# scrose/pylc

Measured on AMD Instinct MI355X. Metric: 512x512 tiles/sec fwd+bwd (DeepLabV3+/ResNet101, 9-class), higher is better.
Workload: dtype f32; 1 GPU; DeepLabV3+ ResNet101 OS16, 3-ch 512x512 tiles, 9 classes, CE+Dice+Focal, clip 0.5 + AdamW, bs=32/GPU (BASELINE.json configs[2]); global_batch=32, parallelism=dp1, conv_arithmetic=f16x3 split (fp32-grade), rccl_ranks=0, wgrad_queue=compute stream, sync_bn=True, activation_format=fp16 planes between BatchNorm and conv kernels (4 B/element)

## Files before the change

include/pylc_hip.h:

```cpp
#ifndef PYLC_HIP_H
#define PYLC_HIP_H

#include <stddef.h>
#include <stdint.h>

#ifdef __cplusplus
extern "C" {
#endif

#define PYLC_OK 0
#define PYLC_ERR_ARG 1
#define PYLC_ERR_HIP 2
#define PYLC_ERR_WORKSPACE 3
#define PYLC_ERR_UNSUPPORTED 4

const char* pylc_last_error(void);
int pylc_abi_version(void);
int pylc_experimental_build(void);
int pylc_init(void);

typedef struct PylcConvDesc {
    int B, H, W;
    int Cin, Cout;
    int R, S;
    int stride, pad, dil;
    int OH, OW;
    int x_pitch;
    int y_pitch;
    const unsigned int* x_amax;
    const unsigned int* w_amax;
    const unsigned int* dy_amax;
    const void* w_planes;
    const void* w_planes_t;
    int x_fmt;
    int dy_fmt;
    int out_fmt;
    unsigned int* out_bound;
    int w_planes_fmt;
} PylcConvDesc;

int pylc_set_conv_precision(int mode);
int pylc_get_conv_precision(void);

int pylc_amax(const float* x, long long rows, int cols, int pitch, unsigned int* out_bits, void* stream);
typedef struct PylcWPrepEntry {
    long long src_offset;
    long long fwd_offset;
    long long t_offset;
    long long tile_begin;
    int K, RS, C;
    int amax_index;
} PylcWPrepEntry;
int pylc_conv1x1_fold_input_affine(const float* w, const float* scale, const float* shift, const float* bias_in, int Cout, int Cin,
                                   float* w_out, float* bias_out, unsigned int* amax_out, void* stream);
int pylc_weight_prepare(const float* base, const PylcWPrepEntry* table, int count, long long total_tiles,
                        const unsigned int* amax, void* planes, int interleave, void* stream);
int pylc_range_product(const unsigned int* a_bits, const unsigned int* b_bits, float factor, const unsigned int* add_bits,
                       unsigned int* out_bits, void* stream);
int pylc_amax_segments(const float* base, const long long* offsets, int count, unsigned int* out_bits, void* stream);

long long pylc_planes_stride(long long M, int C, int nplanes);
int pylc_set_planes_interleave(int on);
int pylc_to_planes(const float* x, int x_pitch, void* planes, int p_pitch, long long plane_stride, long long M, int C,
                   const unsigned int* amax, int nplanes, void* stream);
int pylc_from_planes(const void* planes, int p_pitch, long long plane_stride, float* x, int x_pitch, long long M, int C,
                     const unsigned int* amax, int nplanes, void* stream);
size_t pylc_planes_colsum_workspace_floats(int C);
int pylc_upsample2_crop_concat_planes(const float* z, int z_pitch, int B, int h, int w, int C1, const float* bridge, int bridge_pitch, int HH, int WW,
                                      int C2, void* planes, long long plane_stride, int nplanes, const unsigned int* bound, void* stream);
int pylc_planes_colsum(const void* planes, int p_pitch, long long plane_stride, int nplanes, const unsigned int* amax, long long M, int C,
                       float* sums, float* workspace, void* stream);

int pylc_conv2d_fwd(const PylcConvDesc* d, const float* x, const float* w_krsc, const float* bias,
                    float* y, void* stream);
int pylc_conv2d_fwd_bnact(const PylcConvDesc* d, const float* x, const float* w_krsc, const float* bias,
                          const float* scale, const float* shift, const float* residual, int relu, float* y,
                          unsigned int* amax_out, void* stream);

typedef struct PylcFwdEp {
    const float* scale;
    const float* shift;
    const unsigned int* scale_amax;
    const unsigned int* shift_amax;
    const void* residual;
    int res_fmt;
    const unsigned int* res_scale_bound;
    const unsigned int* res_amax;
    const unsigned int* x_true_amax;
    int relu;
    unsigned int* amax_out;
} PylcFwdEp;
int pylc_conv2d_fwd_bnact_ex(const PylcConvDesc* d, const void* x, const float* w, const float* bias, const PylcFwdEp* ep, void* y, void* stream);
size_t pylc_conv2d_fwd_stats_floats(const PylcConvDesc* d);
int pylc_conv2d_fwd_stats(const PylcConvDesc* d, const float* x, const float* w_krsc, const float* bias,
                          float* y, float* stats_partial, int* stats_rows, void* stream);
int pylc_conv2d_dgrad(const PylcConvDesc* d, const float* dy, const float* w_crsk, float* dx,
                      int accumulate, void* stream);
int pylc_conv2d_dgrad_add(const PylcConvDesc* d, const float* dy, const float* w_crsk, float* dx, int accumulate,
                          const float* add_src, const void* add_mask, void* stream);
#ifdef PYLC_EXPERIMENTAL
typedef struct PylcBnBack {
    const float* y;
    const float* mean;
    const float* invstd;
    const float* scale;
    const float* shift;
    const void* relu_mask;
    int relu;
    unsigned int* g_amax;
} PylcBnBack;
size_t pylc_conv2d_dgrad_bn_floats(const PylcConvDesc* d);
int pylc_conv2d_dgrad_bn(const PylcConvDesc* d, const float* dy, const float* w_crsk, float* dx, int accumulate,
                         const float* add_src, const void* add_mask, const PylcBnBack* bn, float* sums_partial, int* sums_rows,
                         void* stream);
#endif
int pylc_relu_bwd_bits(const float* dout, const void* mask, float* g_out, long long M, int C, void* stream);
int pylc_conv2d_dgrad_needs_f32_weights(const PylcConvDesc* d);
size_t pylc_conv2d_wgrad_workspace(const PylcConvDesc* d);
int pylc_conv2d_wgrad(const PylcConvDesc* d, const float* x, const float* dy, float* dw_krsc,
                      float* dbias ,
                      void* workspace, size_t workspace_bytes, void* stream);
typedef struct PylcSlabSum {
    const float* slabs;
    float* dw;
    long long n4;
    long long slab_stride;
    int splits;
    int reserved;
} PylcSlabSum;
int pylc_conv2d_wgrad_slabs(const PylcConvDesc* d, const float* x, const float* dy, float* dw_krsc, void* workspace, size_t workspace_bytes,
                            PylcSlabSum* pending, void* stream);
int pylc_splitk_reduce_batch(const PylcSlabSum* table_dev, const long long* tile_prefix_dev, int n, long long total_tiles, void* stream);
int pylc_weight_transpose(const float* w_krsc, float* w_crsk, int K, int RS, int C, void* stream);

typedef struct PylcDwDesc {
    int B, H, W, C;
    int stride, dil;
    int OH, OW;
    int x_pitch, y_pitch;
} PylcDwDesc;
int pylc_dwconv3x3_fwd(const PylcDwDesc* d, const float* x, const float* w, float* y, void* stream);
int pylc_dwconv3x3_fwd_stats_rows(const PylcDwDesc* d);
int pylc_dwconv3x3_fwd_stats(const PylcDwDesc* d, const float* x, const float* w_c9, float* y, float* stats_partial, void* stream);
int pylc_dwconv3x3_dgrad(const PylcDwDesc* d, const float* dy, const float* w, float* dx, void* stream);
int pylc_dwconv3x3_dgrad_acc(const PylcDwDesc* d, const float* dy, const float* w_c9, float* dx, int accumulate, void* stream);
size_t pylc_dwconv3x3_wgrad_workspace(const PylcDwDesc* d);
int pylc_dwconv3x3_wgrad(const PylcDwDesc* d, const float* x, const float* dy, float* dw,
                         void* workspace, size_t workspace_bytes, void* stream);
int pylc_dwconv3x3_half_ok(const PylcDwDesc* d);
int pylc_dwconv3x3_fwd_h_stats_rows(const PylcDwDesc* d);
int pylc_dwconv3x3_fwd_h(const PylcDwDesc* d, const void* x_h, const unsigned int* x_bound, const float* w_c9, const unsigned int* w_amax,
                         void* y_h, unsigned int* y_bound_out, float* stats_partial, void* stream);
int pylc_dwconv3x3_fwd_h_eval(const PylcDwDesc* d, const void* x_h, const unsigned int* x_bound, const unsigned int* x_true_amax, const float* w,
                              const unsigned int* w_amax, void* y_h, unsigned int* y_bound_out, void* stream);
int pylc_dwconv3x3_dgrad_h(const PylcDwDesc* d, const void* dy_h, const unsigned int* dy_bound, const float* w_c9, const unsigned int* w_amax,
                           void* dx_h, unsigned int* dx_bound_out, int accumulate, const unsigned int* acc_bound, void* stream);
int pylc_dwconv3x3_dgrad_h_add_ok(const PylcDwDesc* d);
int pylc_dwconv3x3_dgrad_h_add(const PylcDwDesc* d, const void* dy_h, const unsigned int* dy_bound, const float* w_c9, const unsigned int* w_amax,
                               float* dx, const float* add_src, const unsigned char* add_mask, void* stream);
int pylc_dwconv3x3_bn_ok(const PylcDwDesc* d);
int pylc_dwconv3x3_fwd_h_bn(const PylcDwDesc* d, const void* y_in_h, const unsigned int* y_in_bound, const float* bn_scale, const float* bn_shift,
                            int relu, const unsigned int* x_bound, const float* w_c9, const unsigned int* w_amax, void* y_h,
                            unsigned int* y_bound_out, float* stats_partial, void* stream);
int pylc_dwconv3x3_wgrad_h_bn(const PylcDwDesc* d, const void* y_in_h, const unsigned int* y_in_bound, const float* bn_scale, const float* bn_shift,
                              int relu, const unsigned int* x_bound, const void* dy_h, const unsigned int* dy_bound, float* dw, void* workspace,
                              size_t workspace_bytes, void* stream);
int pylc_dwconv3x3_wgrad_h(const PylcDwDesc* d, const void* x_h, const unsigned int* x_bound, const void* dy_h, const unsigned int* dy_bound,
                           float* dw, void* workspace, size_t workspace_bytes, void* stream);

size_t pylc_bn_workspace_floats(long long M, int C);
int pylc_bn_stats(const float* y, long long M, int C, int y_pitch, float* sums ,
                  float* workspace, void* stream);
int pylc_bn_stats_from_partial(const float* partial, int n_rows, int C, float* sums , void* stream);
int pylc_bn_finalize(const float* sums, double n, int C, const float* gamma, const float* beta,
                     float eps, float momentum, int clamp_eps,
                     float* running_mean, float* running_var,
                     float* mean, float* invstd, float* scale, float* shift, void* stream);
int pylc_bn_finalize_from_partial(const float* partial, int n_rows, double n, int C, const float* gamma, const float* beta,
                                  float eps, float momentum, int clamp_eps, float* running_mean, float* running_var,
                                  float* mean, float* invstd, float* scale, float* shift, void* stream);
int pylc_bn_eval_coeffs(const float* running_mean, const float* running_var, const float* gamma,
                        const float* beta, float eps, int C, float* scale, float* shift, void* stream);
int pylc_bn_eval_coeffs_full(const float* running_mean, const float* running_var, const float* gamma, const float* beta, float eps,
                             int C, float* scale, float* shift, float* mean, float* invstd, void* stream);
int pylc_bn_apply(const float* y, int y_pitch, const float* scale, const float* shift,
                  const float* residual, int res_pitch, float* out, int out_pitch,
                  long long M, int C, int relu, unsigned int* amax_out, void* stream);
int pylc_bn_bwd_reduce(const float* dout, int dout_pitch, const float* out, int out_pitch,
                       const float* y, int y_pitch, const float* mean, const float* invstd,
                       long long M, int C, int relu, float* sums , float* workspace,
                       const float* scale, const float* shift, void* stream);
int pylc_bn_bwd_apply(const float* dout, int dout_pitch, const float* out, int out_pitch,
                      const float* y, int y_pitch, const float* mean, const float* invstd,
                      const float* gamma, const float* sums, double n,
                      long long M, int C, int relu, float* dy, int dy_pitch, float* g_out, int g_pitch,
                      unsigned int* amax_dy, const float* scale, const float* shift, void* stream);
typedef struct PylcBnExtra {
    void* out_planes;        long long out_plane_stride;  const unsigned int* out_bound;
    const void* res_planes;  long long res_plane_stride;  const unsigned int* res_amax;
    void* dy_planes;         long long dy_plane_stride;   const unsigned int* dy_bound;
    int nplanes;
    float drop_p;
    uint64_t drop_seed;
    unsigned int* g_amax;
    void* relu_mask;
    const unsigned int* y_half_bound;
    const unsigned int* dout_half_bound;
} PylcBnExtra;
int pylc_bn_finalize_ex(const float* sums, double n, int C, const float* gamma, const float* beta, float eps, float momentum,
                        int clamp_eps, float* running_mean, float* running_var, float* mean, float* invstd, float* scale,
                        float* shift, const unsigned int* bound_extra, float bound_mul, unsigned int* bound_out,
                        const float* y, int y_pitch, long long M, const float* stat_shift, void* stream);
int pylc_bn_finalize_from_partial_ex(const float* partial, int n_rows, double n, int C, const float* gamma, const float* beta,
                                     float eps, float momentum, int clamp_eps, float* running_mean, float* running_var,
                                     float* mean, float* invstd, float* scale, float* shift, const unsigned int* bound_extra,
                                     float bound_mul, unsigned int* bound_out, const float* y, int y_pitch, long long M,
                                     const float* stat_shift, void* stream);
int pylc_bn_local_moments(const float* sums, double n, int C, const float* y, int y_pitch, long long M, const float* stat_shift,
                          double* moments, void* stream);
int pylc_bn_finalize_moments(const double* moments, double n, int C, const float* gamma, const float* beta, float eps, float momentum,
                             int clamp_eps, float* running_mean, float* running_var, float* mean, float* invstd, float* scale,
                             float* shift, const unsigned int* bound_extra, float bound_mul, unsigned int* bound_out,
                             const float* stat_shift, void* stream);
int pylc_bn_apply_ex(const float* y, int y_pitch, const float* scale, const float* shift, const float* residual, int res_pitch,
                     float* out, int out_pitch, long long M, int C, int relu, unsigned int* amax_out, const PylcBnExtra* ex,
                     void* stream);
int pylc_bn_bwd_reduce_ex(const float* dout, int dout_pitch, const float* out, int out_pitch, const float* y, int y_pitch,
                          const float* mean, const float* invstd, long long M, int C, int relu, float* sums, float* workspace,
                          const float* scale, const float* shift, const float* gamma, double n, const PylcBnExtra* ex,
                          unsigned int* dy_bound_out, void* stream);
int pylc_bn_bwd_bound(const float* sums, const float* gamma, const float* invstd, double n, int C, const unsigned int* g_amax,
                      unsigned int* bound_out, void* stream);
#ifdef PYLC_EXPERIMENTAL
int pylc_bn_bwd_sums_from_partial(const float* partial, int rows, int C, float* sums, const float* gamma, const float* invstd, double n,
                                  const unsigned int* g_amax, unsigned int* dy_bound_out, void* stream);
#endif
int pylc_bn_bwd_apply_ex(const float* dout, int dout_pitch, const float* out, int out_pitch, const float* y, int y_pitch,
                         const float* mean, const float* invstd, const float* gamma, const float* sums, double n, long long M,
                         int C, int relu, float* dy, int dy_pitch, float* g_out, int g_pitch, unsigned int* amax_dy,
                         const float* scale, const float* shift, const PylcBnExtra* ex, void* stream);
int pylc_bn_frozen_bwd(const float* dout, int dout_pitch, const float* out, int out_pitch, const float* y, int y_pitch,
                       const float* mean, const float* invstd, const float* gamma, long long M, int C, int relu, float* dy,
                       int dy_pitch, float* g_out, int g_pitch, unsigned int* amax_dy, const float* scale, const float* shift,
                       float* sums , float* workspace, const PylcBnExtra* ex, void* stream);
int pylc_relu_fwd(const float* x, int x_pitch, float* out, int out_pitch, long long M, int C, void* stream);
int pylc_relu_bwd(const float* dout, int dout_pitch, const float* out, int out_pitch, float* dx, int dx_pitch,
                  long long M, int C, void* stream);

int pylc_maxpool_fwd(const float* x, float* y, unsigned char* idx, int B, int H, int W, int C, int k, int stride,
                     int pad, int OH, int OW, void* stream);
int pylc_maxpool_fwd_planes(const float* x, void* y_planes, long long plane_stride, int nplanes, const unsigned int* bound, unsigned char* idx,
                            int B, int H, int W, int C, int k, int stride, int pad, int OH, int OW, void* stream);
int pylc_maxpool_bwd(const float* dy, const unsigned char* idx, float* dx, int B, int H, int W, int C, int k,
                     int stride, int pad, int OH, int OW, void* stream);
int pylc_maxpool_bwd_add(const float* dy, const unsigned char* idx, float* dx, int B, int H, int W, int C, int k,
                         int stride, int pad, int OH, int OW, const float* add, int add_pitch, int add_h0,
                         int add_w0, int add_h, int add_w, void* stream);
int pylc_crop_copy(const float* src, int src_pitch, int H, int W, int h0, int w0, float* dst, int dst_pitch,
                   int B, int TH, int TW, int C, void* stream);
int pylc_bilinear_fwd(const float* x, int x_pitch, float* y, int y_pitch, int B, int H, int W, int C,
                      int OH, int OW, void* stream);
int pylc_bilinear_bwd(const float* dy, int dy_pitch, float* dx, int dx_pitch, int B, int H, int W, int C,
                      int OH, int OW, void* stream);
size_t pylc_bilinear_bwd_workspace(int B, int W, int C, int OH);
int pylc_bilinear_bwd_separable(const float* dy, int dy_pitch, float* dx, int dx_pitch, int B, int H, int W, int C,
                                int OH, int OW, float* workspace, unsigned int* amax_bits, void* stream);
int pylc_gap_fwd(const float* x, float* y, int B, int HW, int C, void* stream);
int pylc_gap_bwd(const float* dy, float* dx, int B, int HW, int C, void* stream);
int pylc_gap_fwd_planes(const void* planes, long long plane_stride, int nplanes, const unsigned int* amax, float* y,
                        int B, int HW, int C, void* stream);
int pylc_gap_bwd_acc(const float* dy, float* dx, int B, int HW, int C, int accumulate, void* stream);

int pylc_image_pack(const float* img_nchw, int B, int Cimg, int H, int W, const float* mean3,
                    const float* std3, float* out_nhwc4, void* stream);
int pylc_image_pack_tiles(const float* img, int Cimg, int H, int W, int tile, int stride, int first_tile, int n_tiles,
                          const float* mean3, const float* std3, float* out, void* stream);
int pylc_stitch_argmax(const float* logits, int pitch, int rows, int cols, int tile, int stride, int C,
                       unsigned char* mask, void* stream);
int pylc_colourize_resize(const unsigned char* mask, int h, int w, const unsigned char* palette_rgb,
                          unsigned char* out_rgb, int oh, int ow, void* stream);
int pylc_image_pack_tiles_reflect(const void* img, int is_u8, int Cimg, int H, int W, int tile, int out, int stride,
                                  int first_tile, int n_tiles, const float* mean3, const float* std3, float* tiles,
                                  void* stream);
int pylc_stitch_overlap_argmax(const float* logits, int pitch, int n_tiles, int H, int W, int out, int stride, int C,
                               unsigned char* mask, float* probs, void* stream);
int pylc_resize_area_u8(const unsigned char* src, int src_planar, int Cimg, int H, int W, unsigned char* dst, int oh, int ow,
                        void* stream);
int pylc_class_encode_resize(const unsigned char* rgb, int H, int W, const unsigned char* palette_rgb, int n_classes,
                             unsigned char* out, int oh, int ow, void* stream);
int pylc_class_encode_resize_ex(const unsigned char* rgb, int H, int W, const unsigned char* palette_rgb, int n_classes,
                                unsigned char* out, int oh, int ow, int unmatched_value, void* stream);
int pylc_image_pack_tiles_ex(const void* img, int is_u8, int Cimg, int H, int W, int tile, int stride, int first_tile,
                             int n_tiles, const float* mean3, const float* std3, float* out, void* stream);

int pylc_blend_accumulate(const float* logits, int pitch, int first_tile, int n_tiles, int H, int W, int out, int stride, int C,
                          int flip, float* acc, int acc_pitch, void* stream);
int pylc_blend_finalize(const float* acc, int acc_pitch, int H, int W, int out, int stride, int C, int members,
                        unsigned char* mask, float* probs, float* conf, void* stream);
int pylc_image_pack_tiles_flip(const void* img, int is_u8, int Cimg, int H, int W, int tile, int stride, int first_tile,
                               int n_tiles, const float* mean3, const float* std3, float* out, void* stream, int flip);
int pylc_image_pack_tiles_reflect_ex(const void* img, int is_u8, int Cimg, int H, int W, int tile, int out, int stride,
                                     int first_tile, int n_tiles, const float* mean3, const float* std3, float* tiles,
                                     void* stream, int flip);

int pylc_resize_bilinear_image(const void* src, int is_u8, int Cimg, int H, int W, float* dst, int oh, int ow, void* stream);
int pylc_blend_resample_accumulate(const float* acc_s, int src_pitch, int Hs, int Ws, int out, int stride, int members, float weight,
                                   int C, float* ens, int ens_pitch, int H, int W, int add, void* stream);
int pylc_ensemble_finalize(const float* ens, int pitch, int H, int W, int C, float total_weight, unsigned char* mask, float* probs,
                           float* conf, void* stream);

int pylc_extract_tiles(const unsigned char* img, int Cimg, int H, int W, const unsigned char* mask, int n_classes, int tile,
                       int stride, int first_tile, int n_tiles, int band_rows, unsigned char* img_tiles,
                       unsigned char* mask_tiles, unsigned long long* sums, unsigned long long* hist, void* stream);
int pylc_tile_stats(const unsigned char* img_tiles, long long n_tiles, int Cimg, int tile, const unsigned char* mask_tiles,
                    int n_classes, int band_rows, unsigned long long* sums, unsigned long long* hist, void* stream);
int pylc_augment_tiles(const unsigned char* img_tiles, const unsigned char* mask_tiles, long long n_src, int Cimg, int tile,
                       const int* src_index, const double* minv, const int* shift, long long m, int band_rows,
                       unsigned char* out_img, unsigned char* out_mask, int n_classes, unsigned long long* sums,
                       unsigned long long* hist, void* stream);

int pylc_confusion_matrix(const void* y_true, int true_bytes, const void* y_pred, int pred_bytes, long long n, int C,
                          int force_coverage, unsigned long long* cm, void* stream);
int pylc_confusion_matrix_ex(const void* y_true, int true_bytes, const void* y_pred, int pred_bytes, long long n, int C,
                             int force_coverage, unsigned long long* cm, int ignore_index, unsigned long long* n_skipped, void* stream);
int pylc_logits_score(const float* logits, int pitch, const void* target, int target_bytes, long long N, int C, unsigned char* mask,
                      unsigned long long* counts, void* stream);
int pylc_logits_score_ex(const float* logits, int pitch, const void* target, int target_bytes, long long N, int C, unsigned char* mask,
                         int ignore_index, unsigned long long* counts, void* stream);

int pylc_label_regions(const unsigned char* mask, int H, int W, int connectivity, int ignore_index, int* labels, void* stream);
int pylc_region_sizes(const int* labels, long long N, int* sizes, void* stream);
int pylc_sieve_regions(const unsigned char* mask, const int* labels, const int* sizes, int H, int W, int min_size, int ignore_index,
                       int fill, unsigned long long* best_ws, unsigned char* out, long long* n_changed, void* stream);

int pylc_image_pack_denom(const void* img_nchw, int is_u8, int B, int Cimg, int H, int W, const float* mean3, const float* std3,
                          float denom, float* out_nhwc4, void* stream);
int pylc_image_pack_u8(const unsigned char* img_nchw, int B, int Cimg, int H, int W, const float* mean3,
                       const float* std3, float* out_nhwc4, void* stream);

int pylc_nhwc_to_nchw(const float* x, int x_pitch, float* y, int B, int H, int W, int C, void* stream);
int pylc_nchw_to_nhwc(const float* x, float* y, int y_pitch, int B, int H, int W, int C, void* stream);

#define PYLC_MAX_CLASSES 16
size_t pylc_multiloss_workspace_floats(long long N, int C);
int pylc_multiloss_stats(const float* logits, int pitch, const int64_t* target, long long N, int C,
                         const float* class_weights, float* stats, float* workspace, void* stream);
int pylc_multiloss_finalize(const float* stats, double n_global, int C, float w_ce, float w_dice, float w_focal,
                            float* losses, void* stream);
int pylc_multiloss_bwd(const float* logits, int pitch, const int64_t* target, long long N, int C,
                       const float* class_weights, const float* stats, double n_global,
                       float w_ce, float w_dice, float w_focal, const float* grad_scale,
                       float* dlogits, int dpitch, unsigned int* amax_bits, void* stream);
int pylc_multiloss_stats_ex(const float* logits, int pitch, const void* target, int target_bytes, long long N, int C, int ignore_index,
                            const float* class_weights, float* stats, float* workspace, unsigned long long* n_bad, void* stream);
int pylc_multiloss_finalize_ex(const float* stats, int C, float w_ce, float w_dice, float w_focal, float* losses, void* stream);
int pylc_multiloss_bwd_ex(const float* logits, int pitch, const void* target, int target_bytes, long long N, int C, int ignore_index,
                          const float* class_weights, const float* stats, float w_ce, float w_dice, float w_focal,
                          const float* grad_scale, float* dlogits, int dpitch, unsigned int* amax_bits, void* stream);

size_t pylc_sqnorm_workspace_floats(long long n);
int pylc_grad_norm_clip(const float* g, long long n, float max_norm, float* out2, float* workspace, void* stream);
int pylc_adamw_step(float* p, const float* g, float* m, float* v, long long n, const float* coef,
                    float lr, float beta1, float beta2, float eps, float weight_decay, int step, void* stream);
int pylc_adamw_step_ranges(float* p, const float* g, float* m, float* v, long long n, const float* coef,
                           float lr, float beta1, float beta2, float eps, float weight_decay, int step,
                           const long long* seg_offsets, int seg_count, unsigned int* seg_amax_bits, void* stream);
int pylc_sgd_step(float* p, const float* g, float* buf, long long n, const float* coef, float lr, float momentum,
                  int step, void* stream);

int pylc_dropout(const float* x, int x_pitch, float* out, int out_pitch, long long M, int C, float p,
                 uint64_t seed, void* stream);

#ifdef PYLC_EXPERIMENTAL
int pylc_stream_create_cu_mask(int n_cus, int from_top, void** stream_out);
int pylc_stream_destroy(void* stream);
#endif

int pylc_debug_set_big_tile(int mode);
int pylc_debug_pp_flags(int flags);
int pylc_debug_stagger(int units);
int pylc_debug_dw_tiles(int on);
int pylc_debug_wgrad_m16(int on);
int pylc_debug_wgrad_dma(int on);
int pylc_debug_wgrad_acc1(int on);
int pylc_debug_wgrad_sets(int mode);
int pylc_debug_wgrad_flags(int flags);
int pylc_debug_wgrad_max_steps(int steps);
int pylc_debug_pp_stamps(unsigned long long* buf);

#define PYLC_COMM_ID_BYTES 128
int pylc_comm_available(void);
int pylc_comm_unique_id(void* id_out);
int pylc_comm_init(const void* id, int rank, int world, void** comm_out);
int pylc_comm_allreduce(void* comm, void* buf, long long count, int dtype, void* stream);
int pylc_comm_syncbn_reduce(void* comm, double* moments, int channels, void* stream);
int pylc_comm_destroy(void* comm);

#ifdef __cplusplus
}
#endif
#endif
```

pylc_amd/csrc/common.h:

```cpp
#pragma once
#include <hip/hip_runtime.h>
#include <cstdarg>
#include <cstdio>
#include <cstring>
#include "../../include/pylc_hip.h"

namespace pylc {

extern thread_local char g_err[512];

inline int fail(int code, const char* fmt, ...) {
    va_list ap;
    va_start(ap, fmt);
    vsnprintf(g_err, sizeof(g_err), fmt, ap);
    va_end(ap);
    return code;
}

#define PYLC_REQUIRE(cond, ...)                                     \
    do {                                                            \
        if (!(cond)) return ::pylc::fail(PYLC_ERR_ARG, __VA_ARGS__); \
    } while (0)

#define PYLC_HIP(expr)                                                                          \
    do {                                                                                        \
        hipError_t e__ = (expr);                                                                \
        if (e__ != hipSuccess)                                                                  \
            return ::pylc::fail(PYLC_ERR_HIP, "%s failed: %s", #expr, hipGetErrorString(e__));  \
    } while (0)

#define PYLC_LAUNCH_CHECK() PYLC_HIP(hipGetLastError())

inline hipStream_t as_stream(void* s) { return reinterpret_cast<hipStream_t>(s); }

template <typename T>
__host__ __device__ inline T cdiv(T a, T b) { return (a + b - 1) / b; }

constexpr long long kPlanesIL = 32;
__host__ __device__ inline bool planes_il(long long plane_stride) { return plane_stride == kPlanesIL; }
__host__ __device__ inline long long planes_phys(long long e, bool il) { return il ? ((e >> 5) << 6) + (e & 31) : e; }
__host__ __device__ inline long long planes_p1(long long plane_stride) { return plane_stride; }

extern int g_planes_interleave;
inline long long planes_stride_rule(long long M, int C, int pitch, int nplanes) {
    const bool il = nplanes == 2 && g_planes_interleave && pitch == C && C % 32 == 0 && M * C * 4 < (1ll << 31);
    return il ? kPlanesIL : M * pitch;
}

constexpr int kWave = 64;
constexpr int kNumCU = 256;

__device__ inline float block_sum_256(float v, float* red) {
#pragma unroll
    for (int o = 32; o > 0; o >>= 1) v += __shfl_down(v, o, 64);
    const int lane = threadIdx.x & 63, wv = threadIdx.x >> 6;
    __syncthreads();
    if (lane == 0) red[wv] = v;
    __syncthreads();
    return red[0] + red[1] + red[2] + red[3];
}

__device__ inline void amax_commit(float m, unsigned* out) {
#pragma unroll
    for (int o = 32; o > 0; o >>= 1) m = fmaxf(m, __shfl_xor(m, o, 64));
    if ((threadIdx.x & 63) == 0) {
        const unsigned bits = __float_as_uint(m);
        if (bits > __atomic_load_n(out, __ATOMIC_RELAXED)) atomicMax(out, bits);
    }
}

__global__ __launch_bounds__(256) static void column_sum_kernel(const float* __restrict__ partial, int nrows, int ncols,
                                                                 float* __restrict__ out) {
    __shared__ double red[32][9];
    const int tx = threadIdx.x & 7, ty = threadIdx.x >> 3;
    const int c = blockIdx.x * 8 + tx;
    double acc = 0.0;
    if (c < ncols) {
        for (int r = ty; r < nrows; r += 16 * 32) {
            float v[16];
#pragma unroll
            for (int u = 0; u < 16; ++u) v[u] = partial[(size_t)(r + u * 32 < nrows ? r + u * 32 : 0) * ncols + c];
#pragma unroll
            for (int u = 0; u < 16; ++u) acc += r + u * 32 < nrows ? (double)v[u] : 0.0;
        }
    }
    red[ty][tx] = acc;
    __syncthreads();
    if (ty == 0 && c < ncols) {
        double s = 0.0;
#pragma unroll
        for (int k = 0; k < 32; ++k) s += red[k][tx];
        out[c] = (float)s;
    }
}

}
```

pylc_amd/csrc/loss.hip:

```cpp
#include "common.h"

namespace pylc {

constexpr int MAXC = PYLC_MAX_CLASSES;
constexpr float kFlAlpha = 0.25f;
constexpr float kFlEps = 1e-8f;
constexpr float kDiceSmooth = 1.f;
constexpr int kLossBlocks = 1024;

template <int C>
__device__ __forceinline__ void softmax_px(const float* __restrict__ z, float (&p)[C], float& lse) {
    float zmax = z[0];
#pragma unroll
    for (int c = 1; c < C; ++c) zmax = fmaxf(zmax, z[c]);
    float sum = 0.f;
#pragma unroll
    for (int c = 0; c < C; ++c) { p[c] = expf(z[c] - zmax); sum += p[c]; }
    const float inv = 1.f / sum;
#pragma unroll
    for (int c = 0; c < C; ++c) p[c] *= inv;
    lse = zmax + logf(sum);
}

template <int C, typename TT, bool IGN>
__global__ __launch_bounds__(256) void multiloss_stats_kernel(const float* __restrict__ logits, int pitch, const TT* __restrict__ target,
                                                              long long N, const float* __restrict__ cw, float* __restrict__ partial,
                                                              long long ignore, unsigned long long* __restrict__ n_bad) {
    __shared__ float red[4];
    float acc[3 + 3 * C];
#pragma unroll
    for (int k = 0; k < 3 + 3 * C; ++k) acc[k] = 0.f;
    unsigned int bad = 0;
    for (long long n = (long long)blockIdx.x * blockDim.x + threadIdx.x; n < N; n += (long long)gridDim.x * blockDim.x) {
        const long long tl = (long long)target[n];
        if constexpr (IGN) {
            if (tl == ignore) continue;
            if ((unsigned long long)tl >= (unsigned long long)C) { ++bad; continue; }
        }
        float z[C], p[C], lse;
        const float* src = logits + n * pitch;
#pragma unroll
        for (int c = 0; c < C; ++c) z[c] = src[c];
        softmax_px<C>(z, p, lse);
        const int t = (int)tl;
        float zt = 0.f, pt = 0.f;
#pragma unroll
        for (int c = 0; c < C; ++c) {
            const bool is = (c == t);
            zt = is ? z[c] : zt;
            pt = is ? p[c] : pt;
            acc[3 + c] += is ? p[c] : 0.f;
            acc[3 + C + c] += p[c];
            acc[3 + 2 * C + c] += is ? 1.f : 0.f;
        }
        const float w = cw != nullptr ? cw[t] : 1.f;
        acc[0] += w * (lse - zt);
        acc[1] += w;
        const float q = pt + kFlEps;
        const float omq = 1.f - q;
        acc[2] += -kFlAlpha * omq * omq * logf(q);
    }
    float* dst = partial + (size_t)blockIdx.x * (3 + 3 * C);
#pragma unroll
    for (int k = 0; k < 3 + 3 * C; ++k) {
        const float s = block_sum_256(acc[k], red);
        if (threadIdx.x == 0) dst[k] = s;
    }
    if constexpr (IGN) {
        if (n_bad != nullptr) {
            unsigned long long wave_bad = 0;
            for (int l = 0; l < 64; ++l) wave_bad += (unsigned)__shfl((int)bad, l, 64);
            if ((threadIdx.x & 63) == 0 && wave_bad != 0) atomicAdd(n_bad, wave_bad);
        }
    }
}

__device__ __forceinline__ double stats_n_valid(const float* __restrict__ stats, int C) {
    double n = 0.0;
    for (int c = 0; c < C; ++c) n += (double)stats[3 + 2 * C + c];
    return n;
}

template <bool FROM_STATS>
__global__ void multiloss_finalize_kernel(const float* __restrict__ stats, double n, int C, float w_ce, float w_d, float w_f,
                                          float* __restrict__ losses) {
    if (threadIdx.x != 0 || blockIdx.x != 0) return;
    double ce, fl;
    if constexpr (FROM_STATS) {
        n = stats_n_valid(stats, C);
        ce = stats[1] > 0.f ? (double)stats[0] / (double)stats[1] : 0.0;
        fl = n > 0.0 ? (double)stats[2] / n : 0.0;
    } else {
        ce = (double)stats[0] / (double)stats[1];
        fl = (double)stats[2] / n;
    }
    double dsc = 0.0;
    for (int c = 0; c < C; ++c) {
        const double I = stats[3 + c], K = (double)stats[3 + C + c] + (double)stats[3 + 2 * C + c];
        dsc += 1.0 - (2.0 * I + kDiceSmooth) / (K + kDiceSmooth);
    }
    dsc /= C;
    losses[0] = (float)(w_ce * ce + w_d * dsc + w_f * fl);
    losses[1] = (float)ce;
    losses[2] = (float)dsc;
    losses[3] = (float)fl;
}

typedef float loss_f4 __attribute__((ext_vector_type(4)));

template <int C, typename TT, bool IGN>
__global__ __launch_bounds__(256) void multiloss_bwd_kernel(const float* __restrict__ logits, int pitch, const TT* __restrict__ target,
                                                            long long N, const float* __restrict__ cw, const float* __restrict__ stats,
                                                            float inv_n, float w_ce, float w_d, float w_f,
                                                            const float* __restrict__ grad_scale, float* __restrict__ dlogits, int dpitch,
                                                            int Cstore, unsigned* __restrict__ amax_out, long long ignore, int zero16) {
    float dA[C], dB[C];
#pragma unroll
    for (int c = 0; c < C; ++c) {
        const float I = stats[3 + c], K = stats[3 + C + c] + stats[3 + 2 * C + c];
        const float den = K + kDiceSmooth;
        dA[c] = -2.f / den / (float)C;
        dB[c] = (2.f * I + kDiceSmooth) / (den * den) / (float)C;
    }
    const float gs = grad_scale != nullptr ? grad_scale[0] : 1.f;
    float ce_norm;
    if constexpr (IGN) {
        const double nv = stats_n_valid(stats, C);
        inv_n = nv > 0.0 ? (float)(1.0 / nv) : 0.f;
        ce_norm = stats[1] > 0.f ? w_ce / stats[1] : 0.f;
    } else {
        ce_norm = w_ce / stats[1];
    }
    float gmax = 0.f;
    for (long long n = (long long)blockIdx.x * blockDim.x + threadIdx.x; n < N; n += (long long)gridDim.x * blockDim.x) {
        const long long tl = (long long)target[n];
        if constexpr (IGN) {
            if (tl == ignore || (unsigned long long)tl >= (unsigned long long)C) {
                float* zrow = dlogits + n * dpitch;
                if (zero16) {
                    for (int c = 0; c < Cstore; c += 4) *reinterpret_cast<loss_f4*>(zrow + c) = loss_f4{0.f, 0.f, 0.f, 0.f};
                } else {
                    for (int c = 0; c < Cstore; ++c) zrow[c] = 0.f;
                }
                continue;
            }
        }
        float z[C], p[C], lse;
        const float* src = logits + n * pitch;
#pragma unroll
        for (int c = 0; c < C; ++c) z[c] = src[c];
        softmax_px<C>(z, p, lse);
        const int t = (int)tl;
        float pt = 0.f;
#pragma unroll
        for (int c = 0; c < C; ++c) pt = (c == t) ? p[c] : pt;
        const float w = cw != nullptr ? cw[t] : 1.f;
        const float q = pt + kFlEps, omq = 1.f - q;
        const float fprime = kFlAlpha * 2.f * omq * logf(q) - kFlAlpha * omq * omq / q;
        const float fcoef = w_f * inv_n * fprime * pt;
        float gdot = 0.f;
#pragma unroll
        for (int c = 0; c < C; ++c) gdot += ((c == t ? dA[c] : 0.f) + dB[c]) * p[c];
        float* dst = dlogits + n * dpitch;
#pragma unroll
        for (int c = 0; c < C; ++c) {
            const float o = (c == t) ? 1.f : 0.f;
            const float gc = (c == t ? dA[c] : 0.f) + dB[c];
            const float d = ce_norm * w * (p[c] - o) + w_d * p[c] * (gc - gdot) + fcoef * (o - p[c]);
            dst[c] = gs * d;
            gmax = fmaxf(gmax, fabsf(gs * d));
        }
        for (int c = C; c < Cstore; ++c) dst[c] = 0.f;
    }
    if (amax_out != nullptr) amax_commit(gmax, amax_out);
}

#define PYLC_FOR_C(MACRO)                                                                                              \
    switch (C) {                                                                                                       \
        case 2: MACRO(2); break; case 3: MACRO(3); break; case 4: MACRO(4); break; case 5: MACRO(5); break;           \
        case 6: MACRO(6); break; case 7: MACRO(7); break; case 8: MACRO(8); break; case 9: MACRO(9); break;           \
        case 10: MACRO(10); break; case 11: MACRO(11); break; case 12: MACRO(12); break; case 13: MACRO(13); break;   \
        case 14: MACRO(14); break; case 15: MACRO(15); break; case 16: MACRO(16); break;                              \
        default: return fail(PYLC_ERR_ARG, "multiloss: n_classes=%d unsupported (2..%d)", C, MAXC);                   \
    }

}

using namespace pylc;

extern "C" size_t pylc_multiloss_workspace_floats(long long N, int C) {
    (void)N;
    return (size_t)kLossBlocks * (3 + 3 * (size_t)C);
}

static int multiloss_stats_impl(const float* logits, int pitch, const void* target, int target_bytes, bool ign, long long N, int C, long long ignore,
                                const float* cw, float* stats, float* workspace, unsigned long long* n_bad, void* stream) {
    hipStream_t st = as_stream(stream);
    const int blocks = (int)(cdiv<long long>(N, 256) < kLossBlocks ? cdiv<long long>(N, 256) : kLossBlocks);
#define LAUNCH_STATS_T(CC, TT, IGN)                                                                                                          \
    hipLaunchKernelGGL((multiloss_stats_kernel<CC, TT, IGN>), dim3(blocks), dim3(256), 0, st, logits, pitch, static_cast<const TT*>(target), N, cw, \
                       workspace, ignore, n_bad)
    if (!ign) {
#define LAUNCH_STATS(CC) LAUNCH_STATS_T(CC, long long, false)
        PYLC_FOR_C(LAUNCH_STATS)
#undef LAUNCH_STATS
    } else if (target_bytes == 8) {
#define LAUNCH_STATS(CC) LAUNCH_STATS_T(CC, long long, true)
        PYLC_FOR_C(LAUNCH_STATS)
#undef LAUNCH_STATS
    } else {
#define LAUNCH_STATS(CC) LAUNCH_STATS_T(CC, unsigned char, true)
        PYLC_FOR_C(LAUNCH_STATS)
#undef LAUNCH_STATS
    }
#undef LAUNCH_STATS_T
    PYLC_LAUNCH_CHECK();
    const int K = 3 + 3 * C;
    hipLaunchKernelGGL(column_sum_kernel, dim3(cdiv(K, 8)), dim3(256), 0, st, workspace, blocks, K, stats);
    PYLC_LAUNCH_CHECK();
    return PYLC_OK;
}

extern "C" int pylc_multiloss_stats(const float* logits, int pitch, const int64_t* target, long long N, int C, const float* cw, float* stats,
                                    float* workspace, void* stream) {
    PYLC_REQUIRE(C >= 2 && C <= MAXC, "multiloss_stats: n_classes=%d unsupported (2..%d)", C, MAXC);
    PYLC_REQUIRE(logits && target && stats && workspace && N > 0 && pitch >= C, "multiloss_stats: bad arguments");
    return multiloss_stats_impl(logits, pitch, target, 8, false, N, C, 0, cw, stats, workspace, nullptr, stream);
}

extern "C" int pylc_multiloss_stats_ex(const float* logits, int pitch, const void* target, int target_bytes, long long N, int C, int ignore_index,
                                       const float* cw, float* stats, float* workspace, unsigned long long* n_bad, void* stream) {
    PYLC_REQUIRE(C >= 2 && C <= MAXC, "multiloss_stats_ex: n_classes=%d unsupported (2..%d)", C, MAXC);
    PYLC_REQUIRE(target_bytes == 1 || target_bytes == 8, "multiloss_stats_ex: target_bytes=%d (1: uint8, 8: int64)", target_bytes);
    PYLC_REQUIRE(target, "multiloss_stats_ex: target is NULL");
    PYLC_REQUIRE(pitch >= C, "multiloss_stats_ex: pitch=%d below n_classes=%d", pitch, C);
    PYLC_REQUIRE(N > 0, "multiloss_stats_ex: N=%lld is not positive", N);
    PYLC_REQUIRE(logits && stats && workspace, "multiloss_stats_ex: logits, stats or workspace is NULL");
    PYLC_REQUIRE((target_bytes != 8 || (reinterpret_cast<uintptr_t>(target) & 7) == 0) && (reinterpret_cast<uintptr_t>(n_bad) & 7) == 0,
                 "multiloss_stats_ex: a buffer is not aligned to its element");
    return multiloss_stats_impl(logits, pitch, target, target_bytes, true, N, C, (long long)ignore_index, cw, stats, workspace, n_bad, stream);
}

extern "C" int pylc_multiloss_finalize(const float* stats, double n_global, int C, float w_ce, float w_dice, float w_focal, float* losses,
                                       void* stream) {
    PYLC_REQUIRE(stats && losses && n_global > 0 && C >= 2 && C <= MAXC, "multiloss_finalize: bad arguments");
    hipLaunchKernelGGL(multiloss_finalize_kernel<false>, dim3(1), dim3(64), 0, as_stream(stream), stats, n_global, C, w_ce, w_dice, w_focal, losses);
    PYLC_LAUNCH_CHECK();
    return PYLC_OK;
}

extern "C" int pylc_multiloss_finalize_ex(const float* stats, int C, float w_ce, float w_dice, float w_focal, float* losses, void* stream) {
    PYLC_REQUIRE(C >= 2 && C <= MAXC, "multiloss_finalize_ex: n_classes=%d unsupported (2..%d)", C, MAXC);
    PYLC_REQUIRE(stats && losses, "multiloss_finalize_ex: stats or losses is NULL");
    hipLaunchKernelGGL(multiloss_finalize_kernel<true>, dim3(1), dim3(64), 0, as_stream(stream), stats, 0.0, C, w_ce, w_dice, w_focal, losses);
    PYLC_LAUNCH_CHECK();
    return PYLC_OK;
}

static int multiloss_bwd_impl(const float* logits, int pitch, const void* target, int target_bytes, bool ign, long long N, int C, long long ignore,
                              const float* cw, const float* stats, double n_global, float w_ce, float w_dice, float w_focal,
                              const float* grad_scale, float* dlogits, int dpitch, unsigned int* amax_bits, void* stream) {
    hipStream_t st = as_stream(stream);
    if (amax_bits != nullptr) PYLC_HIP(hipMemsetAsync(amax_bits, 0, sizeof(unsigned), st));
    const int blocks = (int)(cdiv<long long>(N, 256) < 4096 ? cdiv<long long>(N, 256) : 4096);
    const int Cstore = ((C + 3) & ~3) <= dpitch ? ((C + 3) & ~3) : C;
    const float inv_n = ign ? 0.f : (float)(1.0 / n_global);
    const int zero16 = dpitch % 4 == 0 && (reinterpret_cast<uintptr_t>(dlogits) & 15) == 0;
#define LAUNCH_BWD_T(CC, TT, IGN)                                                                                                              \
    hipLaunchKernelGGL((multiloss_bwd_kernel<CC, TT, IGN>), dim3(blocks), dim3(256), 0, st, logits, pitch, static_cast<const TT*>(target), N, cw, \
                       stats, inv_n, w_ce, w_dice, w_focal, grad_scale, dlogits, dpitch, Cstore, amax_bits, ignore, zero16)
    if (!ign) {
#define LAUNCH_BWD(CC) LAUNCH_BWD_T(CC, long long, false)
        PYLC_FOR_C(LAUNCH_BWD)
#undef LAUNCH_BWD
    } else if (target_bytes == 8) {
#define LAUNCH_BWD(CC) LAUNCH_BWD_T(CC, long long, true)
        PYLC_FOR_C(LAUNCH_BWD)
#undef LAUNCH_BWD
    } else {
#define LAUNCH_BWD(CC) LAUNCH_BWD_T(CC, unsigned char, true)
        PYLC_FOR_C(LAUNCH_BWD)
#undef LAUNCH_BWD
    }
#undef LAUNCH_BWD_T
    PYLC_LAUNCH_CHECK();
    return PYLC_OK;
}

extern "C" int pylc_multiloss_bwd(const float* logits, int pitch, const int64_t* target, long long N, int C, const float* cw,
                                  const float* stats, double n_global, float w_ce, float w_dice, float w_focal, const float* grad_scale,
                                  float* dlogits, int dpitch, unsigned int* amax_bits, void* stream) {
    PYLC_REQUIRE(C >= 2 && C <= MAXC, "multiloss_bwd: n_classes=%d unsupported (2..%d)", C, MAXC);
    PYLC_REQUIRE(logits && target && stats && dlogits && N > 0 && pitch >= C && dpitch >= C && n_global > 0, "multiloss_bwd: bad arguments");
    return multiloss_bwd_impl(logits, pitch, target, 8, false, N, C, 0, cw, stats, n_global, w_ce, w_dice, w_focal, grad_scale, dlogits, dpitch,
                              amax_bits, stream);
}

extern "C" int pylc_multiloss_bwd_ex(const float* logits, int pitch, const void* target, int target_bytes, long long N, int C, int ignore_index,
                                     const float* cw, const float* stats, float w_ce, float w_dice, float w_focal, const float* grad_scale,
                                     float* dlogits, int dpitch, unsigned int* amax_bits, void* stream) {
    PYLC_REQUIRE(C >= 2 && C <= MAXC, "multiloss_bwd_ex: n_classes=%d unsupported (2..%d)", C, MAXC);
    PYLC_REQUIRE(target_bytes == 1 || target_bytes == 8, "multiloss_bwd_ex: target_bytes=%d (1: uint8, 8: int64)", target_bytes);
    PYLC_REQUIRE(target, "multiloss_bwd_ex: target is NULL");
    PYLC_REQUIRE(pitch >= C && dpitch >= C, "multiloss_bwd_ex: pitch=%d or dpitch=%d below n_classes=%d", pitch, dpitch, C);
    PYLC_REQUIRE(N > 0, "multiloss_bwd_ex: N=%lld is not positive", N);
    PYLC_REQUIRE(logits && stats && dlogits, "multiloss_bwd_ex: logits, stats or dlogits is NULL");
    PYLC_REQUIRE(target_bytes != 8 || (reinterpret_cast<uintptr_t>(target) & 7) == 0, "multiloss_bwd_ex: an int64 target is not 8-byte aligned");
    return multiloss_bwd_impl(logits, pitch, target, target_bytes, true, N, C, (long long)ignore_index, cw, stats, 1.0, w_ce, w_dice, w_focal,
                              grad_scale, dlogits, dpitch, amax_bits, stream);
}
```

pylc_amd/csrc/planes.hip:

```cpp
#include "conv_common.h"

namespace pylc {

typedef _Float16 f16;

__device__ __forceinline__ void psplit(float x, float s, f16& h0, f16& h1) {
    const float xs = x * s;
    h0 = (f16)xs;
    h1 = (f16)((xs - (float)h0) * 2048.f);
}

template <int NPL>
__global__ __launch_bounds__(256) void to_planes_kernel(const float* __restrict__ x, int x_pitch, f16* __restrict__ planes, int p_pitch,
                                                        long long plane_stride, long long M, int C8, const unsigned* __restrict__ amax) {
    const float s = pow2_scale_for(*amax);
    const long long total = M * C8;
    for (long long i = (long long)blockIdx.x * 256 + threadIdx.x; i < total; i += (long long)gridDim.x * 256) {
        const long long r = i / C8;
        const int c = (int)(i - r * C8) * 8;
        const f32x4 lo = *reinterpret_cast<const f32x4*>(x + r * x_pitch + c);
        const f32x4 hi = *reinterpret_cast<const f32x4*>(x + r * x_pitch + c + 4);
        f16x8 h0, h1;
#pragma unroll
        for (int e = 0; e < 4; ++e) {
            f16 a0, a1, b0, b1;
            psplit(lo[e], s, a0, a1);
            psplit(hi[e], s, b0, b1);
            h0[e] = a0; h1[e] = a1; h0[4 + e] = b0; h1[4 + e] = b1;
        }
        const long long e = planes_phys(r * p_pitch + c, NPL == 2 && planes_il(plane_stride));
        *reinterpret_cast<f16x8*>(planes + e) = h0;
        if constexpr (NPL == 2) *reinterpret_cast<f16x8*>(planes + plane_stride + e) = h1;
    }
}

template <int NPL>
__global__ __launch_bounds__(256) void from_planes_kernel(const f16* __restrict__ planes, int p_pitch, long long plane_stride,
                                                          float* __restrict__ x, int x_pitch, long long M, int C8,
                                                          const unsigned* __restrict__ amax) {
    const float inv = 1.f / pow2_scale_for(*amax);
    const long long total = M * C8;
    for (long long i = (long long)blockIdx.x * 256 + threadIdx.x; i < total; i += (long long)gridDim.x * 256) {
        const long long r = i / C8;
        const int c = (int)(i - r * C8) * 8;
        const long long e = planes_phys(r * p_pitch + c, NPL == 2 && planes_il(plane_stride));
        const f16x8 h0 = *reinterpret_cast<const f16x8*>(planes + e);
        f16x8 h1 = {};
        if constexpr (NPL == 2) h1 = *reinterpret_cast<const f16x8*>(planes + plane_stride + e);
        f32x4 lo, hi;
#pragma unroll
        for (int e = 0; e < 4; ++e) {
            lo[e] = ((float)h0[e] + (float)h1[e] * (1.f / 2048.f)) * inv;
            hi[e] = ((float)h0[4 + e] + (float)h1[4 + e] * (1.f / 2048.f)) * inv;
        }
        *reinterpret_cast<f32x4*>(x + r * x_pitch + c) = lo;
        *reinterpret_cast<f32x4*>(x + r * x_pitch + c + 4) = hi;
    }
}

struct UpLerp { int i0, i1; float w0, w1; };
__device__ __forceinline__ UpLerp up_lerp(int dst, float scale, int in_size) {
    const float src = scale * (float)dst;
    UpLerp l;
    l.i0 = (int)src;
    if (l.i0 > in_size - 1) l.i0 = in_size - 1;
    l.i1 = l.i0 + (l.i0 < in_size - 1 ? 1 : 0);
    l.w1 = src - (float)l.i0;
    l.w0 = 1.f - l.w1;
    return l;
}

template <int NPL>
__global__ __launch_bounds__(256) void upcat_planes_kernel(const float* __restrict__ z, int z_pitch, int h, int w, const float* __restrict__ bridge,
                                                           int b_pitch, int HH, int WW, int h0, int w0, f16* __restrict__ planes,
                                                           long long plane_stride, int OH, int OW, int C1, int C2, float sh, float sw,
                                                           const unsigned* __restrict__ bound) {
    const int C8 = (C1 + C2) / 8;
    const unsigned i = blockIdx.x * 256u + threadIdx.x;
    if (i >= (unsigned)(OW * C8)) return;
    const int c = (int)(i % (unsigned)C8) * 8, ow = (int)(i / (unsigned)C8);
    const int oh = blockIdx.y, b = blockIdx.z;
    const float s = pow2_scale_for(*bound);
    f32x4 lo, hi;
    if (c < C1) {
        const UpLerp lh = up_lerp(oh, sh, h), lw = up_lerp(ow, sw, w);
        const float* base = z + (size_t)b * h * w * z_pitch + c;
        const float* p00 = base + ((size_t)lh.i0 * w + lw.i0) * z_pitch;
        const float* p01 = base + ((size_t)lh.i0 * w + lw.i1) * z_pitch;
        const float* p10 = base + ((size_t)lh.i1 * w + lw.i0) * z_pitch;
        const float* p11 = base + ((size_t)lh.i1 * w + lw.i1) * z_pitch;
        lo = lh.w0 * (lw.w0 * *reinterpret_cast<const f32x4*>(p00) + lw.w1 * *reinterpret_cast<const f32x4*>(p01)) +
             lh.w1 * (lw.w0 * *reinterpret_cast<const f32x4*>(p10) + lw.w1 * *reinterpret_cast<const f32x4*>(p11));
        hi = lh.w0 * (lw.w0 * *reinterpret_cast<const f32x4*>(p00 + 4) + lw.w1 * *reinterpret_cast<const f32x4*>(p01 + 4)) +
             lh.w1 * (lw.w0 * *reinterpret_cast<const f32x4*>(p10 + 4) + lw.w1 * *reinterpret_cast<const f32x4*>(p11 + 4));
    } else {
        const float* src = bridge + ((size_t)(b * HH + h0 + oh) * WW + w0 + ow) * b_pitch + (c - C1);
        lo = *reinterpret_cast<const f32x4*>(src);
        hi = *reinterpret_cast<const f32x4*>(src + 4);
    }
    f16x8 q0, q1;
#pragma unroll
    for (int e = 0; e < 4; ++e) {
        f16 a0, a1, b0, b1;
        psplit(lo[e], s, a0, a1);
        psplit(hi[e], s, b0, b1);
        q0[e] = a0; q1[e] = a1; q0[4 + e] = b0; q1[4 + e] = b1;
    }
    f16* dst = planes + planes_phys((long long)((size_t)(b * OH + oh) * OW + ow) * (C1 + C2) + c, NPL == 2 && planes_il(plane_stride));
    *reinterpret_cast<f16x8*>(dst) = q0;
    if constexpr (NPL == 2) *reinterpret_cast<f16x8*>(dst + plane_stride) = q1;
}

constexpr int kColsumSlabs = 768;
template <int NPL>
__global__ __launch_bounds__(256) void planes_colsum_kernel(const f16* __restrict__ planes, int p_pitch, long long plane_stride, long long M, int C8,
                                                            int cols, int RL, long long rows_per_slab, const unsigned* __restrict__ amax,
                                                            float* __restrict__ partial) {
    __shared__ float red[256][9];
    const float inv = 1.f / pow2_scale_for(*amax);
    const int tx = threadIdx.x % cols, ty = threadIdx.x / cols;
    const long long r_begin = (long long)blockIdx.x * rows_per_slab;
    long long r_end = r_begin + rows_per_slab;
    if (r_end > M) r_end = M;
    for (int cb = 0; cb < C8; cb += cols) {
        const int c8 = cb + tx;
        const bool active = ty < RL && c8 < C8;
        float acc[8] = {0.f, 0.f, 0.f, 0.f, 0.f, 0.f, 0.f, 0.f};
        if (active) {
            for (long long r = r_begin + ty; r < r_end; r += RL) {
                const long long e = planes_phys(r * p_pitch + 8 * c8, NPL == 2 && planes_il(plane_stride));
                const f16x8 h0 = *reinterpret_cast<const f16x8*>(planes + e);
                f16x8 h1 = {};
                if constexpr (NPL == 2) h1 = *reinterpret_cast<const f16x8*>(planes + plane_stride + e);
#pragma unroll
                for (int e = 0; e < 8; ++e) acc[e] += ((float)h0[e] + (float)h1[e] * (1.f / 2048.f)) * inv;
            }
        }
#pragma unroll
        for (int e = 0; e < 8; ++e) red[threadIdx.x][e] = acc[e];
        __syncthreads();
        if (ty == 0 && c8 < C8) {
#pragma unroll
            for (int e = 0; e < 8; ++e) {
                float sum = acc[e];
                for (int q = 1; q < RL; ++q) sum += red[q * cols + tx][e];
                partial[(size_t)blockIdx.x * (8 * C8) + 8 * c8 + e] = sum;
            }
        }
        __syncthreads();
    }
}

static int check_planes(const void* planes, int p_pitch, long long plane_stride, long long M, int C, int nplanes, const char* what) {
    PYLC_REQUIRE(planes && M > 0 && C > 0 && C % 8 == 0, "%s: need M > 0 and C %% 8 == 0 (M=%lld C=%d)", what, M, C);
    PYLC_REQUIRE(p_pitch >= C && p_pitch % 8 == 0, "%s: plane pitch %d invalid for C=%d (multiple of 8)", what, p_pitch, C);
    PYLC_REQUIRE(nplanes == 1 || nplanes == 2, "%s: nplanes must be 1 or 2", what);
    PYLC_REQUIRE(nplanes == 1 || (plane_stride >= M * p_pitch - (p_pitch - C) && plane_stride % 8 == 0) ||
                     (planes_il(plane_stride) && p_pitch == C && C % 32 == 0),
                 "%s: bad plane stride (32 = chunk-interleaved needs a dense pitch and C %% 32 == 0)", what);
    PYLC_REQUIRE((reinterpret_cast<uintptr_t>(planes) & 15) == 0, "%s: planes must be 16-byte aligned", what);
    return PYLC_OK;
}

}

using namespace pylc;

int pylc::g_planes_interleave = 1;
extern "C" int pylc_set_planes_interleave(int on) { pylc::g_planes_interleave = on ? 1 : 0; return PYLC_OK; }
extern "C" long long pylc_planes_stride(long long M, int C, int nplanes) { return pylc::planes_stride_rule(M, C, C, nplanes); }

extern "C" int pylc_to_planes(const float* x, int x_pitch, void* planes, int p_pitch, long long plane_stride, long long M, int C,
                              const unsigned int* amax, int nplanes, void* stream) {
    if (int rc = check_planes(planes, p_pitch, plane_stride, M, C, nplanes, "to_planes")) return rc;
    PYLC_REQUIRE(x && amax && x_pitch >= C && x_pitch % 4 == 0 && (reinterpret_cast<uintptr_t>(x) & 15) == 0, "to_planes: bad fp32 source");
    const long long total = M * (C / 8);
    const int blocks = (int)(cdiv<long long>(total, 256 * 4) < 4096 ? cdiv<long long>(total, 256 * 4) : 4096);
    const dim3 g(blocks > 0 ? blocks : 1), b(256);
    if (nplanes == 2) hipLaunchKernelGGL((to_planes_kernel<2>), g, b, 0, as_stream(stream), x, x_pitch, static_cast<f16*>(planes), p_pitch, plane_stride, M, C / 8, amax);
    else hipLaunchKernelGGL((to_planes_kernel<1>), g, b, 0, as_stream(stream), x, x_pitch, static_cast<f16*>(planes), p_pitch, plane_stride, M, C / 8, amax);
    PYLC_LAUNCH_CHECK();
    return PYLC_OK;
}

extern "C" int pylc_from_planes(const void* planes, int p_pitch, long long plane_stride, float* x, int x_pitch, long long M, int C,
                                const unsigned int* amax, int nplanes, void* stream) {
    if (int rc = check_planes(planes, p_pitch, plane_stride, M, C, nplanes, "from_planes")) return rc;
    PYLC_REQUIRE(x && amax && x_pitch >= C && x_pitch % 4 == 0 && (reinterpret_cast<uintptr_t>(x) & 15) == 0, "from_planes: bad fp32 destination");
    const long long total = M * (C / 8);
    const int blocks = (int)(cdiv<long long>(total, 256 * 4) < 4096 ? cdiv<long long>(total, 256 * 4) : 4096);
    const dim3 g(blocks > 0 ? blocks : 1), b(256);
    if (nplanes == 2) hipLaunchKernelGGL((from_planes_kernel<2>), g, b, 0, as_stream(stream), static_cast<const f16*>(planes), p_pitch, plane_stride, x, x_pitch, M, C / 8, amax);
    else hipLaunchKernelGGL((from_planes_kernel<1>), g, b, 0, as_stream(stream), static_cast<const f16*>(planes), p_pitch, plane_stride, x, x_pitch, M, C / 8, amax);
    PYLC_LAUNCH_CHECK();
    return PYLC_OK;
}

extern "C" size_t pylc_planes_colsum_workspace_floats(int C) { return (size_t)kColsumSlabs * (size_t)C; }

extern "C" int pylc_planes_colsum(const void* planes, int p_pitch, long long plane_stride, int nplanes, const unsigned int* amax, long long M, int C,
                                  float* sums, float* workspace, void* stream) {
    if (int rc = check_planes(planes, p_pitch, plane_stride, M, C, nplanes, "planes_colsum")) return rc;
    PYLC_REQUIRE(amax && sums && workspace, "planes_colsum: null pointer");
    const int C8 = C / 8;
    const int cols = C8 < 256 ? C8 : 256;
    const int RL = 256 / cols;
    long long rps = cdiv<long long>(M, kColsumSlabs);
    if (rps < (long long)RL * 8) rps = (long long)RL * 8;
    rps = cdiv<long long>(rps, RL) * RL;
    const int nslab = (int)cdiv<long long>(M, rps);
    hipStream_t st = as_stream(stream);
    const f16* p = static_cast<const f16*>(planes);
    if (nplanes == 2)
        hipLaunchKernelGGL(planes_colsum_kernel<2>, dim3(nslab), dim3(256), 0, st, p, p_pitch, plane_stride, M, C8, cols, RL, rps, amax, workspace);
    else
        hipLaunchKernelGGL(planes_colsum_kernel<1>, dim3(nslab), dim3(256), 0, st, p, p_pitch, plane_stride, M, C8, cols, RL, rps, amax, workspace);
    PYLC_LAUNCH_CHECK();
    hipLaunchKernelGGL(column_sum_kernel, dim3(cdiv(C, 8)), dim3(256), 0, st, workspace, nslab, C, sums);
    PYLC_LAUNCH_CHECK();
    return PYLC_OK;
}

extern "C" int pylc_upsample2_crop_concat_planes(const float* z, int z_pitch, int B, int h, int w, int C1, const float* bridge, int bridge_pitch, int HH,
                                                 int WW, int C2, void* planes, long long plane_stride, int nplanes, const unsigned int* bound,
                                                 void* stream) {
    const int OH = 2 * h, OW = 2 * w;
    PYLC_REQUIRE(z && bridge && planes && bound && B > 0 && h > 0 && w > 0 && C1 > 0 && C2 > 0 && C1 % 8 == 0 && C2 % 8 == 0 && (nplanes == 1 || nplanes == 2),
                 "upsample2_crop_concat_planes: bad arguments (channel counts must be multiples of 8)");
    PYLC_REQUIRE(z_pitch >= C1 && bridge_pitch >= C2 && z_pitch % 4 == 0 && bridge_pitch % 4 == 0 && HH >= OH && WW >= OW && B <= 65535 && OH <= 65535 &&
                     (reinterpret_cast<uintptr_t>(planes) & 15) == 0 && plane_stride % 8 == 0,
                 "upsample2_crop_concat_planes: bad pitch / the bridge is smaller than the up-sampled tensor / unaligned planes");
    const int h0 = (HH - OH) / 2, w0 = (WW - OW) / 2;
    const float sh = OH > 1 ? (float)(h - 1) / (float)(OH - 1) : 0.f, sw = OW > 1 ? (float)(w - 1) / (float)(OW - 1) : 0.f;
    const dim3 grid(cdiv(OW * ((C1 + C2) / 8), 256), OH, B);
    if (nplanes == 2)
        hipLaunchKernelGGL(upcat_planes_kernel<2>, grid, dim3(256), 0, as_stream(stream), z, z_pitch, h, w, bridge, bridge_pitch, HH, WW, h0, w0,
                           static_cast<f16*>(planes), plane_stride, OH, OW, C1, C2, sh, sw, bound);
    else
        hipLaunchKernelGGL(upcat_planes_kernel<1>, grid, dim3(256), 0, as_stream(stream), z, z_pitch, h, w, bridge, bridge_pitch, HH, WW, h0, w0,
                           static_cast<f16*>(planes), plane_stride, OH, OW, C1, C2, sh, sw, bound);
    PYLC_LAUNCH_CHECK();
    return PYLC_OK;
}
```

pylc_amd/csrc/pool_resize.hip:

```cpp
#include "common.h"

namespace pylc {

typedef float f32x4 __attribute__((ext_vector_type(4)));
__device__ __forceinline__ f32x4 ld4(const float* p) { return *reinterpret_cast<const f32x4*>(p); }
__device__ __forceinline__ void st4(float* p, f32x4 v) { *reinterpret_cast<f32x4*>(p) = v; }

static inline int grid_for(long long n, int cap = 8192) {
    long long b = cdiv<long long>(n, 256);
    return (int)(b < cap ? (b < 1 ? 1 : b) : cap);
}

struct PoolPlanes { _Float16* planes; long long plane_stride; const unsigned* bound; int nplanes; };
__device__ __forceinline__ float pool_pow2_scale(unsigned bits) {
    int e = (int)((bits >> 23) & 0xFFu);
    int se = 127 + 14 - (e - 127);
    se = se < 1 ? 1 : (se > 242 ? 242 : se);
    return __uint_as_float((unsigned)se << 23);
}

__global__ void maxpool_fwd_kernel(const float* __restrict__ x, float* __restrict__ y, unsigned char* __restrict__ idx, int B, int H, int W,
                                   int C, int k, int s, int pad, int OH, int OW, PoolPlanes pp) {
    const int CV = C / 4;
    const long long total = (long long)B * OH * OW * CV;
    for (long long i = (long long)blockIdx.x * blockDim.x + threadIdx.x; i < total; i += (long long)gridDim.x * blockDim.x) {
        const int cv = (int)(i % CV);
        long long t = i / CV;
        const int ow = (int)(t % OW); t /= OW;
        const int oh = (int)(t % OH);
        const int b = (int)(t / OH);
        f32x4 best = {-INFINITY, -INFINITY, -INFINITY, -INFINITY};
        int bi[4] = {0, 0, 0, 0};
        bool first = true;
        for (int kh = 0; kh < k; ++kh) {
            const int h = oh * s - pad + kh;
            if ((unsigned)h >= (unsigned)H) continue;
            for (int kw = 0; kw < k; ++kw) {
                const int w = ow * s - pad + kw;
                if ((unsigned)w >= (unsigned)W) continue;
                const f32x4 v = ld4(x + ((size_t)(b * H + h) * W + w) * C + 4 * cv);
                const int code = kh * k + kw;
                if (first || v.x > best.x) { best.x = v.x; bi[0] = code; }
                if (first || v.y > best.y) { best.y = v.y; bi[1] = code; }
                if (first || v.z > best.z) { best.z = v.z; bi[2] = code; }
                if (first || v.w > best.w) { best.w = v.w; bi[3] = code; }
                first = false;
            }
        }
        if (pp.planes != nullptr) {
            typedef _Float16 f16x4_ __attribute__((ext_vector_type(4)));
            const float sc = pool_pow2_scale(*pp.bound);
            const f32x4 xs = best * sc;
            const f16x4_ h0 = {(_Float16)xs.x, (_Float16)xs.y, (_Float16)xs.z, (_Float16)xs.w};
            const long long pe = planes_phys(4 * i, pp.nplanes == 2 && planes_il(pp.plane_stride));
            *reinterpret_cast<uint2*>(pp.planes + pe) = __builtin_bit_cast(uint2, h0);
            if (pp.nplanes == 2) {
                const f32x4 r = {(xs.x - (float)h0.x) * 2048.f, (xs.y - (float)h0.y) * 2048.f, (xs.z - (float)h0.z) * 2048.f, (xs.w - (float)h0.w) * 2048.f};
                const f16x4_ h1 = {(_Float16)r.x, (_Float16)r.y, (_Float16)r.z, (_Float16)r.w};
                *reinterpret_cast<uint2*>(pp.planes + pp.plane_stride + pe) = __builtin_bit_cast(uint2, h1);
            }
        } else {
            st4(y + 4 * i, best);
        }
        if (idx != nullptr) {
            uchar4 c4 = make_uchar4((unsigned char)bi[0], (unsigned char)bi[1], (unsigned char)bi[2], (unsigned char)bi[3]);
            *reinterpret_cast<uchar4*>(idx + 4 * i) = c4;
        }
    }
}

struct PoolAdd { const float* p; int pitch, h0, w0, AH, AW; };

__global__ void maxpool_bwd_kernel(const float* __restrict__ dy, const unsigned char* __restrict__ idx, float* __restrict__ dx, int B, int H,
                                   int W, int C, int k, int s, int pad, int OH, int OW, PoolAdd add) {
    const int CV = C / 4;
    const long long total = (long long)B * H * W * CV;
    for (long long i = (long long)blockIdx.x * blockDim.x + threadIdx.x; i < total; i += (long long)gridDim.x * blockDim.x) {
        const int cv = (int)(i % CV);
        long long t = i / CV;
        const int w = (int)(t % W); t /= W;
        const int h = (int)(t % H);
        const int b = (int)(t / H);
        f32x4 acc = {0.f, 0.f, 0.f, 0.f};
        int oh_lo = (h + pad - k + 1 + s - 1); oh_lo = oh_lo < 0 ? 0 : oh_lo / s;
        int oh_hi = (h + pad) / s; if (oh_hi > OH - 1) oh_hi = OH - 1;
        int ow_lo = (w + pad - k + 1 + s - 1); ow_lo = ow_lo < 0 ? 0 : ow_lo / s;
        int ow_hi = (w + pad) / s; if (ow_hi > OW - 1) ow_hi = OW - 1;
        for (int oh = oh_lo; oh <= oh_hi; ++oh) {
            const int kh = h - (oh * s - pad);
            for (int ow = ow_lo; ow <= ow_hi; ++ow) {
                const int code = kh * k + (w - (ow * s - pad));
                const size_t o = ((size_t)(b * OH + oh) * OW + ow) * C + 4 * cv;
                const uchar4 c4 = *reinterpret_cast<const uchar4*>(idx + o);
                const f32x4 g = ld4(dy + o);
                if (c4.x == code) acc.x += g.x;
                if (c4.y == code) acc.y += g.y;
                if (c4.z == code) acc.z += g.z;
                if (c4.w == code) acc.w += g.w;
            }
        }
        if (add.p != nullptr && (unsigned)(h - add.h0) < (unsigned)add.AH && (unsigned)(w - add.w0) < (unsigned)add.AW)
            acc += ld4(add.p + ((size_t)(b * add.AH + (h - add.h0)) * add.AW + (w - add.w0)) * add.pitch + 4 * cv);
        st4(dx + 4 * i, acc);
    }
}

__global__ __launch_bounds__(256) void maxpool2_bwd_kernel(const float* __restrict__ dy, const unsigned char* __restrict__ idx, float* __restrict__ dx,
                                                          int H, int W, int C, int OH, int OW, int PW, PoolAdd add) {
    const int CV = C / 4;
    const unsigned i = blockIdx.x * 256u + threadIdx.x;
    if (i >= (unsigned)(PW * CV)) return;
    const int cv = (int)(i % (unsigned)CV), pw = (int)(i / (unsigned)CV);
    const int ph = blockIdx.y, b = blockIdx.z;
    f32x4 g = {0.f, 0.f, 0.f, 0.f};
    uchar4 c4 = make_uchar4(255, 255, 255, 255);
    if (ph < OH && pw < OW) {
        const size_t o = ((size_t)(b * OH + ph) * OW + pw) * C + 4 * cv;
        g = ld4(dy + o);
        c4 = *reinterpret_cast<const uchar4*>(idx + o);
    }
#pragma unroll
    for (int kh = 0; kh < 2; ++kh)
#pragma unroll
        for (int kw = 0; kw < 2; ++kw) {
            const int h = 2 * ph + kh, w = 2 * pw + kw;
            if (h >= H || w >= W) continue;
            const int code = kh * 2 + kw;
            f32x4 acc = {c4.x == code ? g.x : 0.f, c4.y == code ? g.y : 0.f, c4.z == code ? g.z : 0.f, c4.w == code ? g.w : 0.f};
            if (add.p != nullptr && (unsigned)(h - add.h0) < (unsigned)add.AH && (unsigned)(w - add.w0) < (unsigned)add.AW)
                acc += ld4(add.p + ((size_t)(b * add.AH + (h - add.h0)) * add.AW + (w - add.w0)) * add.pitch + 4 * cv);
            st4(dx + ((size_t)(b * H + h) * W + w) * C + 4 * cv, acc);
        }
}

static bool launch_maxpool2_bwd(const float* dy, const unsigned char* idx, float* dx, int B, int H, int W, int C, int k, int stride, int pad, int OH,
                                int OW, PoolAdd add, hipStream_t st) {
    if (!(k == 2 && stride == 2 && pad == 0 && OH == (H - 2) / 2 + 1 && OW == (W - 2) / 2 + 1 && B <= 65535 && (H + 1) / 2 <= 65535)) return false;
    const int PH = (H + 1) / 2, PW = (W + 1) / 2;
    hipLaunchKernelGGL(maxpool2_bwd_kernel, dim3(cdiv(PW * (C / 4), 256), PH, B), dim3(256), 0, st, dy, idx, dx, H, W, C, OH, OW, PW, add);
    return true;
}

__global__ void crop_copy_kernel(const float* __restrict__ src, int src_pitch, int H, int W, int h0, int w0, float* __restrict__ dst,
                                 int dst_pitch, int B, int TH, int TW, int C) {
    const int CV = C / 4;
    const long long total = (long long)B * TH * TW * CV;
    for (long long i = (long long)blockIdx.x * blockDim.x + threadIdx.x; i < total; i += (long long)gridDim.x * blockDim.x) {
        const int cv = (int)(i % CV);
        long long t = i / CV;
        const int x = (int)(t % TW); t /= TW;
        const int y = (int)(t % TH);
        const int b = (int)(t / TH);
        st4(dst + ((size_t)(b * TH + y) * TW + x) * dst_pitch + 4 * cv,
            ld4(src + ((size_t)(b * H + h0 + y) * W + w0 + x) * src_pitch + 4 * cv));
    }
}

struct Lerp { int i0, i1; float w0, w1; };
__device__ __forceinline__ Lerp lerp_of(int dst, float scale, int in_size) {
    const float src = scale * (float)dst;
    Lerp l;
    l.i0 = (int)src;
    if (l.i0 > in_size - 1) l.i0 = in_size - 1;
    l.i1 = l.i0 + (l.i0 < in_size - 1 ? 1 : 0);
    l.w1 = src - (float)l.i0;
    l.w0 = 1.f - l.w1;
    return l;
}

__global__ void bilinear_fwd_kernel(const float* __restrict__ x, int x_pitch, float* __restrict__ y, int y_pitch, int B, int H, int W, int C,
                                    int OH, int OW, float sh, float sw) {
    const int CV = C / 4;
    const long long total = (long long)B * OH * OW * CV;
    for (long long i = (long long)blockIdx.x * blockDim.x + threadIdx.x; i < total; i += (long long)gridDim.x * blockDim.x) {
        const int cv = (int)(i % CV);
        long long t = i / CV;
        const int ow = (int)(t % OW); t /= OW;
        const int oh = (int)(t % OH);
        const int b = (int)(t / OH);
        const Lerp lh = lerp_of(oh, sh, H), lw = lerp_of(ow, sw, W);
        const float* base = x + (size_t)b * H * W * x_pitch + 4 * cv;
        const f32x4 v00 = ld4(base + ((size_t)lh.i0 * W + lw.i0) * x_pitch), v01 = ld4(base + ((size_t)lh.i0 * W + lw.i1) * x_pitch);
        const f32x4 v10 = ld4(base + ((size_t)lh.i1 * W + lw.i0) * x_pitch), v11 = ld4(base + ((size_t)lh.i1 * W + lw.i1) * x_pitch);
        const f32x4 r = lh.w0 * (lw.w0 * v00 + lw.w1 * v01) + lh.w1 * (lw.w0 * v10 + lw.w1 * v11);
        st4(y + ((size_t)(b * OH + oh) * OW + ow) * y_pitch + 4 * cv, r);
    }
}

__global__ __launch_bounds__(256) void bilinear_fwd_rows_kernel(const float* __restrict__ x, int x_pitch, float* __restrict__ y, int y_pitch, int H, int W,
                                                                  int C, int OH, int OW, float sh, float sw) {
    const unsigned CV = (unsigned)C / 4;
    const unsigned idx = blockIdx.x * 256u + threadIdx.x;
    if (idx >= (unsigned)OW * CV) return;
    const unsigned ow = idx / CV, cv = idx - ow * CV;
    const int oh = blockIdx.y, b = blockIdx.z;
    const Lerp lh = lerp_of(oh, sh, H), lw = lerp_of((int)ow, sw, W);
    const float* base = x + (size_t)b * H * W * x_pitch + 4 * cv;
    const f32x4 v00 = ld4(base + ((size_t)lh.i0 * W + lw.i0) * x_pitch), v01 = ld4(base + ((size_t)lh.i0 * W + lw.i1) * x_pitch);
    const f32x4 v10 = ld4(base + ((size_t)lh.i1 * W + lw.i0) * x_pitch), v11 = ld4(base + ((size_t)lh.i1 * W + lw.i1) * x_pitch);
    const f32x4 r = lh.w0 * (lw.w0 * v00 + lw.w1 * v01) + lh.w1 * (lw.w0 * v10 + lw.w1 * v11);
    st4(y + ((size_t)(b * OH + oh) * OW + ow) * y_pitch + 4 * cv, r);
}

__device__ __forceinline__ void cand_range(int i, float scale, int out_size, int& lo, int& hi) {
    if (scale <= 0.f) { lo = 0; hi = out_size - 1; return; }
    lo = (int)floorf((float)(i - 1) / scale) - 1;
    hi = (int)ceilf((float)(i + 1) / scale) + 1;
    if (lo < 0) lo = 0;
    if (hi > out_size - 1) hi = out_size - 1;
}

__global__ void bilinear_bwd_kernel(const float* __restrict__ dy, int dy_pitch, float* __restrict__ dx, int dx_pitch, int B, int H, int W,
                                    int C, int OH, int OW, float sh, float sw) {
    const int CV = C / 4;
    const long long total = (long long)B * H * W * CV;
    for (long long i = (long long)blockIdx.x * blockDim.x + threadIdx.x; i < total; i += (long long)gridDim.x * blockDim.x) {
        const int cv = (int)(i % CV);
        long long t = i / CV;
        const int w = (int)(t % W); t /= W;
        const int h = (int)(t % H);
        const int b = (int)(t / H);
        int oh_lo, oh_hi, ow_lo, ow_hi;
        cand_range(h, sh, OH, oh_lo, oh_hi);
        cand_range(w, sw, OW, ow_lo, ow_hi);
        f32x4 acc = {0.f, 0.f, 0.f, 0.f};
        for (int oh = oh_lo; oh <= oh_hi; ++oh) {
            const Lerp lh = lerp_of(oh, sh, H);
            float wh = 0.f;
            if (lh.i0 == h) wh += lh.w0;
            if (lh.i1 == h) wh += lh.w1;
            if (lh.i0 != h && lh.i1 != h) continue;
            const float* row = dy + (size_t)(b * OH + oh) * OW * dy_pitch + 4 * cv;
            for (int ow = ow_lo; ow <= ow_hi; ++ow) {
                const Lerp lw = lerp_of(ow, sw, W);
                if (lw.i0 != w && lw.i1 != w) continue;
                float ww = 0.f;
                if (lw.i0 == w) ww += lw.w0;
                if (lw.i1 == w) ww += lw.w1;
                acc += (wh * ww) * ld4(row + (size_t)ow * dy_pitch);
            }
        }
        st4(dx + ((size_t)(b * H + h) * W + w) * dx_pitch + 4 * cv, acc);
    }
}

template <int AXIS>
__global__ void bilinear_bwd_axis_kernel(const float* __restrict__ src, int src_pitch, float* __restrict__ dst, int dst_pitch, int rows, int n_in,
                                         int n_out, int inner, int C, float scale, unsigned* __restrict__ amax_out) {
    const int CV = C / 4;
    const long long total = (long long)rows * n_in * inner * CV;
    float m = 0.f;
    for (long long idx = (long long)blockIdx.x * blockDim.x + threadIdx.x; idx < total; idx += (long long)gridDim.x * blockDim.x) {
        const int cv = (int)(idx % CV);
        long long t = idx / CV;
        const int w = (int)(t % inner); t /= inner;
        const int i = (int)(t % n_in);
        const int row = (int)(t / n_in);
        int lo, hi;
        cand_range(i, scale, n_out, lo, hi);
        f32x4 acc = {0.f, 0.f, 0.f, 0.f};
        const float* base = src + ((size_t)row * n_out * inner + w) * src_pitch + 4 * cv;
        for (int o = lo; o <= hi; ++o) {
            const Lerp l = lerp_of(o, scale, n_in);
            if (l.i0 != i && l.i1 != i) continue;
            float wt = 0.f;
            if (l.i0 == i) wt += l.w0;
            if (l.i1 == i) wt += l.w1;
            acc += wt * ld4(base + (size_t)o * inner * src_pitch);
        }
        st4(dst + (((size_t)row * n_in + i) * inner + w) * dst_pitch + 4 * cv, acc);
        m = fmaxf(fmaxf(m, fmaxf(fabsf(acc.x), fabsf(acc.y))), fmaxf(fabsf(acc.z), fabsf(acc.w)));
    }
    if (amax_out != nullptr) amax_commit(m, amax_out);
}

__global__ __launch_bounds__(256) void gap_fwd_kernel(const float* __restrict__ x, float* __restrict__ y, int HW, int C) {
    __shared__ f32x4 red[256];
    const int CV = C / 4;
    const int b = blockIdx.y;
    const int tx = threadIdx.x & 15, ty = threadIdx.x >> 4;
    const int cv = blockIdx.x * 16 + tx;
    f32x4 s = {0.f, 0.f, 0.f, 0.f};
    if (cv < CV) {
        const float* base = x + (size_t)b * HW * C + 4 * cv;
        for (int r = ty; r < HW; r += 16 * 8) {
            f32x4 v[8];
#pragma unroll
            for (int u = 0; u < 8; ++u) {
                const int rr = r + 16 * u;
                v[u] = ld4(base + (size_t)(rr < HW ? rr : r) * C);
            }
#pragma unroll
            for (int u = 0; u < 8; ++u)
                if (r + 16 * u < HW) s += v[u];
        }
    }
    red[threadIdx.x] = s;
    __syncthreads();
    if (ty == 0 && cv < CV) {
        for (int k = 1; k < 16; ++k) s += red[16 * k + tx];
        st4(y + (size_t)b * C + 4 * cv, s * (1.f / (float)HW));
    }
}

typedef _Float16 f16x4p __attribute__((ext_vector_type(4)));
template <int NPL>
__global__ __launch_bounds__(256) void gap_fwd_planes_kernel(const _Float16* __restrict__ planes, long long plane_stride, const unsigned* __restrict__ amax,
                                                             float* __restrict__ y, int HW, int C) {
    __shared__ f32x4 red[256];
    const int CV = C / 4;
    const int b = blockIdx.y;
    const int tx = threadIdx.x & 15, ty = threadIdx.x >> 4;
    const int cv = blockIdx.x * 16 + tx;
    int e = (int)((*amax >> 23) & 0xFFu);
    int se = 127 + 14 - (e - 127);
    se = se < 1 ? 1 : (se > 242 ? 242 : se);
    const float inv = 1.f / __uint_as_float((unsigned)se << 23);
    f32x4 s = {0.f, 0.f, 0.f, 0.f};
    if (cv < CV) {
        const bool il = NPL == 2 && planes_il(plane_stride);
        const long long e0 = (long long)b * HW * C + 4 * cv;
        for (int r = ty; r < HW; r += 16 * 8) {
            f16x4p h0[8], h1[8];
#pragma unroll
            for (int u = 0; u < 8; ++u) {
                const int rr = r + 16 * u;
                const long long off = planes_phys(e0 + (long long)(rr < HW ? rr : r) * C, il);
                h0[u] = *reinterpret_cast<const f16x4p*>(planes + off);
                if constexpr (NPL == 2) h1[u] = *reinterpret_cast<const f16x4p*>(planes + plane_stride + off);
            }
#pragma unroll
            for (int u = 0; u < 8; ++u)
                if (r + 16 * u < HW) {
                    f32x4 v;
#pragma unroll
                    for (int k = 0; k < 4; ++k) v[k] = ((float)h0[u][k] + (NPL == 2 ? (float)h1[u][k] : 0.f) * (1.f / 2048.f)) * inv;
                    s += v;
                }
        }
    }
    red[threadIdx.x] = s;
    __syncthreads();
    if (ty == 0 && cv < CV) {
        for (int k = 1; k < 16; ++k) s += red[16 * k + tx];
        st4(y + (size_t)b * C + 4 * cv, s * (1.f / (float)HW));
    }
}

template <bool ACC>
__global__ void gap_bwd_kernel(const float* __restrict__ dy, float* __restrict__ dx, int B, int HW, int C) {
    const int CV = C / 4;
    const long long total = (long long)B * HW * CV;
    const float inv = 1.f / (float)HW;
    for (long long i = (long long)blockIdx.x * blockDim.x + threadIdx.x; i < total; i += (long long)gridDim.x * blockDim.x) {
        const int cv = (int)(i % CV);
        const int b = (int)(i / ((long long)HW * CV));
        f32x4 v = ld4(dy + (size_t)b * C + 4 * cv) * inv;
        if (ACC) v = v + ld4(dx + 4 * i);
        st4(dx + 4 * i, v);
    }
}

__global__ void image_pack_kernel(const float* __restrict__ img, int B, int Cimg, int HW, f32x4 mean, f32x4 istd, float* __restrict__ out,
                                  float denom) {
    const long long total = (long long)B * HW;
    for (long long i = (long long)blockIdx.x * blockDim.x + threadIdx.x; i < total; i += (long long)gridDim.x * blockDim.x) {
        const long long b = i / HW, p = i % HW;
        const float* src = img + b * Cimg * HW + p;
        f32x4 v;
        v.x = src[0];
        v.y = Cimg == 3 ? src[HW] : v.x;
        v.z = Cimg == 3 ? src[2 * (long long)HW] : v.x;
        v.w = 0.f;
        f32x4 r;
        r.x = ((v.x - mean.x) / istd.x) / denom;
        r.y = ((v.y - mean.y) / istd.y) / denom;
        r.z = ((v.z - mean.z) / istd.z) / denom;
        r.w = 0.f;
        st4(out + 4 * i, r);
    }
}

__global__ void image_pack_u8_kernel(const unsigned char* __restrict__ img, int B, int Cimg, int HW, f32x4 mean, f32x4 sd,
                                     float* __restrict__ out, float denom) {
    const long long total = (long long)B * HW;
    for (long long i = (long long)blockIdx.x * blockDim.x + threadIdx.x; i < total; i += (long long)gridDim.x * blockDim.x) {
        const long long b = i / HW, p = i % HW;
        const unsigned char* src = img + b * Cimg * HW + p;
        const float x = (float)src[0];
        const float y = Cimg == 3 ? (float)src[HW] : x;
        const float z = Cimg == 3 ? (float)src[2 * (long long)HW] : x;
        f32x4 r;
        r.x = ((x - mean.x) / sd.x) / denom;
        r.y = ((y - mean.y) / sd.y) / denom;
        r.z = ((z - mean.z) / sd.z) / denom;
        r.w = 0.f;
        st4(out + 4 * i, r);
    }
}

__global__ void nhwc_to_nchw_kernel(const float* __restrict__ x, int x_pitch, float* __restrict__ y, int B, int HW, int C) {
    const long long total = (long long)B * C * HW;
    for (long long i = (long long)blockIdx.x * blockDim.x + threadIdx.x; i < total; i += (long long)gridDim.x * blockDim.x) {
        const long long p = i % HW;
        const long long t = i / HW;
        const int c = (int)(t % C);
        const long long b = t / C;
        y[i] = x[(b * HW + p) * x_pitch + c];
    }
}

__global__ void nchw_to_nhwc_kernel(const float* __restrict__ x, float* __restrict__ y, int y_pitch, int B, int HW, int C) {
    const long long total = (long long)B * HW * C;
    for (long long i = (long long)blockIdx.x * blockDim.x + threadIdx.x; i < total; i += (long long)gridDim.x * blockDim.x) {
        const int c = (int)(i % C);
        const long long t = i / C;
        const long long p = t % HW, b = t / HW;
        y[(b * HW + p) * y_pitch + c] = x[(b * C + c) * HW + p];
    }
}

}

using namespace pylc;

extern "C" int pylc_maxpool_fwd(const float* x, float* y, unsigned char* idx, int B, int H, int W, int C, int k, int stride, int pad, int OH,
                                int OW, void* stream) {
    PYLC_REQUIRE(x && y && B > 0 && C > 0 && C % 4 == 0 && k >= 1 && k <= 15 && stride >= 1 && pad >= 0 && pad <= k / 2, "maxpool_fwd: bad arguments");
    PYLC_REQUIRE(OH == (H + 2 * pad - k) / stride + 1 && OW == (W + 2 * pad - k) / stride + 1 && OH > 0 && OW > 0, "maxpool_fwd: bad output size");
    const long long total = (long long)B * OH * OW * (C / 4);
    hipLaunchKernelGGL(maxpool_fwd_kernel, dim3(grid_for(total)), dim3(256), 0, as_stream(stream), x, y, idx, B, H, W, C, k, stride, pad, OH, OW,
                       PoolPlanes{nullptr, 0, nullptr, 0});
    PYLC_LAUNCH_CHECK();
    return PYLC_OK;
}

extern "C" int pylc_maxpool_fwd_planes(const float* x, void* y_planes, long long plane_stride, int nplanes, const unsigned int* bound, unsigned char* idx,
                                       int B, int H, int W, int C, int k, int stride, int pad, int OH, int OW, void* stream) {
    PYLC_REQUIRE(x && y_planes && bound && B > 0 && C > 0 && C % 8 == 0 && k >= 1 && k <= 15 && stride >= 1 && pad >= 0 && pad <= k / 2 &&
                     (nplanes == 1 || nplanes == 2) && plane_stride % 4 == 0, "maxpool_fwd_planes: bad arguments (C must be a multiple of 8)");
    PYLC_REQUIRE(OH == (H + 2 * pad - k) / stride + 1 && OW == (W + 2 * pad - k) / stride + 1 && OH > 0 && OW > 0, "maxpool_fwd_planes: bad output size");
    const long long total = (long long)B * OH * OW * (C / 4);
    hipLaunchKernelGGL(maxpool_fwd_kernel, dim3(grid_for(total)), dim3(256), 0, as_stream(stream), x, nullptr, idx, B, H, W, C, k, stride, pad, OH, OW,
                       PoolPlanes{static_cast<_Float16*>(y_planes), plane_stride, bound, nplanes});
    PYLC_LAUNCH_CHECK();
    return PYLC_OK;
}

extern "C" int pylc_maxpool_bwd(const float* dy, const unsigned char* idx, float* dx, int B, int H, int W, int C, int k, int stride, int pad,
                                int OH, int OW, void* stream) {
    PYLC_REQUIRE(dy && idx && dx && B > 0 && C > 0 && C % 4 == 0 && k >= 1 && k <= 15 && stride >= 1, "maxpool_bwd: bad arguments");
    const long long total = (long long)B * H * W * (C / 4);
    if (!launch_maxpool2_bwd(dy, idx, dx, B, H, W, C, k, stride, pad, OH, OW, PoolAdd{nullptr, 0, 0, 0, 0, 0}, as_stream(stream)))
        hipLaunchKernelGGL(maxpool_bwd_kernel, dim3(grid_for(total)), dim3(256), 0, as_stream(stream), dy, idx, dx, B, H, W, C, k, stride, pad, OH, OW,
                           PoolAdd{nullptr, 0, 0, 0, 0, 0});
    PYLC_LAUNCH_CHECK();
    return PYLC_OK;
}

extern "C" int pylc_maxpool_bwd_add(const float* dy, const unsigned char* idx, float* dx, int B, int H, int W, int C, int k, int stride, int pad,
                                    int OH, int OW, const float* add, int add_pitch, int add_h0, int add_w0, int add_h, int add_w, void* stream) {
    PYLC_REQUIRE(dy && idx && dx && add && B > 0 && C > 0 && C % 4 == 0 && k >= 1 && k <= 15 && stride >= 1, "maxpool_bwd_add: bad arguments");
    PYLC_REQUIRE(add_pitch >= C && add_pitch % 4 == 0 && add_h0 >= 0 && add_w0 >= 0 && add_h > 0 && add_w > 0 && add_h0 + add_h <= H &&
                     add_w0 + add_w <= W, "maxpool_bwd_add: the added window must lie inside the %dx%d input", H, W);
    const long long total = (long long)B * H * W * (C / 4);
    if (!launch_maxpool2_bwd(dy, idx, dx, B, H, W, C, k, stride, pad, OH, OW, PoolAdd{add, add_pitch, add_h0, add_w0, add_h, add_w}, as_stream(stream)))
        hipLaunchKernelGGL(maxpool_bwd_kernel, dim3(grid_for(total)), dim3(256), 0, as_stream(stream), dy, idx, dx, B, H, W, C, k, stride, pad, OH, OW,
                           PoolAdd{add, add_pitch, add_h0, add_w0, add_h, add_w});
    PYLC_LAUNCH_CHECK();
    return PYLC_OK;
}

extern "C" int pylc_crop_copy(const float* src, int src_pitch, int H, int W, int h0, int w0, float* dst, int dst_pitch, int B, int TH, int TW,
                              int C, void* stream) {
    PYLC_REQUIRE(src && dst && B > 0 && C > 0 && C % 4 == 0 && TH > 0 && TW > 0, "crop_copy: bad arguments");
    PYLC_REQUIRE(src_pitch >= C && dst_pitch >= C && src_pitch % 4 == 0 && dst_pitch % 4 == 0, "crop_copy: bad pitch");
    PYLC_REQUIRE(h0 >= 0 && w0 >= 0 && h0 + TH <= H && w0 + TW <= W, "crop_copy: window outside the %dx%d source", H, W);
    const long long total = (long long)B * TH * TW * (C / 4);
    hipLaunchKernelGGL(crop_copy_kernel, dim3(grid_for(total)), dim3(256), 0, as_stream(stream), src, src_pitch, H, W, h0, w0, dst, dst_pitch, B, TH,
                       TW, C);
    PYLC_LAUNCH_CHECK();
    return PYLC_OK;
}

static inline float ac_scale(int in, int out) { return out > 1 ? (float)(in - 1) / (float)(out - 1) : 0.f; }

extern "C" int pylc_bilinear_fwd(const float* x, int x_pitch, float* y, int y_pitch, int B, int H, int W, int C, int OH, int OW, void* stream) {
    PYLC_REQUIRE(x && y && B > 0 && H > 0 && W > 0 && OH > 0 && OW > 0 && C > 0 && C % 4 == 0, "bilinear_fwd: bad arguments");
    PYLC_REQUIRE(x_pitch >= C && y_pitch >= C && x_pitch % 4 == 0 && y_pitch % 4 == 0, "bilinear_fwd: bad pitch");
    const long long total = (long long)B * OH * OW * (C / 4);
    if (B <= 65535 && OH <= 65535 && (long long)OW * (C / 4) < (1ll << 31))
        hipLaunchKernelGGL(bilinear_fwd_rows_kernel, dim3(cdiv(OW * (C / 4), 256), OH, B), dim3(256), 0, as_stream(stream), x, x_pitch, y, y_pitch, H, W, C, OH, OW,
                           ac_scale(H, OH), ac_scale(W, OW));
    else
    hipLaunchKernelGGL(bilinear_fwd_kernel, dim3(grid_for(total)), dim3(256), 0, as_stream(stream), x, x_pitch, y, y_pitch, B, H, W, C, OH, OW,
                       ac_scale(H, OH), ac_scale(W, OW));
    PYLC_LAUNCH_CHECK();
    return PYLC_OK;
}

extern "C" int pylc_bilinear_bwd(const float* dy, int dy_pitch, float* dx, int dx_pitch, int B, int H, int W, int C, int OH, int OW, void* stream) {
    PYLC_REQUIRE(dy && dx && B > 0 && H > 0 && W > 0 && OH > 0 && OW > 0 && C > 0 && C % 4 == 0, "bilinear_bwd: bad arguments");
    PYLC_REQUIRE(dy_pitch >= C && dx_pitch >= C && dy_pitch % 4 == 0 && dx_pitch % 4 == 0, "bilinear_bwd: bad pitch");
    const long long total = (long long)B * H * W * (C / 4);
    hipLaunchKernelGGL(bilinear_bwd_kernel, dim3(grid_for(total)), dim3(256), 0, as_stream(stream), dy, dy_pitch, dx, dx_pitch, B, H, W, C, OH, OW,
                       ac_scale(H, OH), ac_scale(W, OW));
    PYLC_LAUNCH_CHECK();
    return PYLC_OK;
}

extern "C" size_t pylc_bilinear_bwd_workspace(int B, int W, int C, int OH) { return (size_t)B * OH * W * C * sizeof(float); }

extern "C" int pylc_bilinear_bwd_separable(const float* dy, int dy_pitch, float* dx, int dx_pitch, int B, int H, int W, int C, int OH, int OW,
                                           float* workspace, unsigned int* amax_bits, void* stream) {
    PYLC_REQUIRE(dy && dx && workspace && B > 0 && H > 0 && W > 0 && OH > 0 && OW > 0 && C > 0 && C % 4 == 0, "bilinear_bwd_separable: bad arguments");
    PYLC_REQUIRE(dy_pitch >= C && dx_pitch >= C && dy_pitch % 4 == 0 && dx_pitch % 4 == 0, "bilinear_bwd_separable: bad pitch");
    const long long t0 = (long long)B * OH * W * (C / 4), t1 = (long long)B * H * W * (C / 4);
    if (amax_bits != nullptr) PYLC_HIP(hipMemsetAsync(amax_bits, 0, sizeof(unsigned), as_stream(stream)));
    hipLaunchKernelGGL(bilinear_bwd_axis_kernel<0>, dim3(grid_for(t0)), dim3(256), 0, as_stream(stream), dy, dy_pitch, workspace, C, B * OH, W, OW, 1, C,
                       ac_scale(W, OW), static_cast<unsigned*>(nullptr));
    PYLC_LAUNCH_CHECK();
    hipLaunchKernelGGL(bilinear_bwd_axis_kernel<1>, dim3(grid_for(t1)), dim3(256), 0, as_stream(stream), workspace, C, dx, dx_pitch, B, H, OH, W, C,
                       ac_scale(H, OH), amax_bits);
    PYLC_LAUNCH_CHECK();
    return PYLC_OK;
}

extern "C" int pylc_gap_fwd(const float* x, float* y, int B, int HW, int C, void* stream) {
    PYLC_REQUIRE(x && y && B > 0 && HW > 0 && C > 0 && C % 4 == 0, "gap_fwd: bad arguments");
    hipLaunchKernelGGL(gap_fwd_kernel, dim3(cdiv(C / 4, 16), B), dim3(256), 0, as_stream(stream), x, y, HW, C);
    PYLC_LAUNCH_CHECK();
    return PYLC_OK;
}

extern "C" int pylc_gap_fwd_planes(const void* planes, long long plane_stride, int nplanes, const unsigned int* amax, float* y, int B, int HW, int C,
                                   void* stream) {
    PYLC_REQUIRE(planes && amax && y && B > 0 && HW > 0 && C > 0 && C % 8 == 0 && (nplanes == 1 || nplanes == 2) &&
                 (nplanes == 1 || plane_stride >= (long long)B * HW * C || (planes_il(plane_stride) && C % 32 == 0)), "gap_fwd_planes: bad arguments");
    const _Float16* p = static_cast<const _Float16*>(planes);
    if (nplanes == 2)
        hipLaunchKernelGGL(gap_fwd_planes_kernel<2>, dim3(cdiv(C / 4, 16), B), dim3(256), 0, as_stream(stream), p, plane_stride, amax, y, HW, C);
    else
        hipLaunchKernelGGL(gap_fwd_planes_kernel<1>, dim3(cdiv(C / 4, 16), B), dim3(256), 0, as_stream(stream), p, plane_stride, amax, y, HW, C);
    PYLC_LAUNCH_CHECK();
    return PYLC_OK;
}

extern "C" int pylc_gap_bwd_acc(const float* dy, float* dx, int B, int HW, int C, int accumulate, void* stream) {
    PYLC_REQUIRE(dy && dx && B > 0 && HW > 0 && C > 0 && C % 4 == 0, "gap_bwd: bad arguments");
    const dim3 grid(grid_for((long long)B * HW * (C / 4)));
    if (accumulate)
        hipLaunchKernelGGL(gap_bwd_kernel<true>, grid, dim3(256), 0, as_stream(stream), dy, dx, B, HW, C);
    else
        hipLaunchKernelGGL(gap_bwd_kernel<false>, grid, dim3(256), 0, as_stream(stream), dy, dx, B, HW, C);
    PYLC_LAUNCH_CHECK();
    return PYLC_OK;
}

extern "C" int pylc_gap_bwd(const float* dy, float* dx, int B, int HW, int C, void* stream) {
    return pylc_gap_bwd_acc(dy, dx, B, HW, C, 0, stream);
}

extern "C" int pylc_image_pack_denom(const void* img, int is_u8, int B, int Cimg, int H, int W, const float* mean3, const float* std3,
                                     float denom, float* out, void* stream) {
    PYLC_REQUIRE(img && out && mean3 && std3 && B > 0 && H > 0 && W > 0 && (Cimg == 1 || Cimg == 3) && denom > 0.f, "image_pack: bad arguments");
    f32x4 mean = {mean3[0], mean3[1], mean3[2], 0.f}, sd = {std3[0], std3[1], std3[2], 1.f};
    if (is_u8)
        hipLaunchKernelGGL(image_pack_u8_kernel, dim3(grid_for((long long)B * H * W)), dim3(256), 0, as_stream(stream),
                           static_cast<const unsigned char*>(img), B, Cimg, H * W, mean, sd, out, denom);
    else
        hipLaunchKernelGGL(image_pack_kernel, dim3(grid_for((long long)B * H * W)), dim3(256), 0, as_stream(stream),
                           static_cast<const float*>(img), B, Cimg, H * W, mean, sd, out, denom);
    PYLC_LAUNCH_CHECK();
    return PYLC_OK;
}

extern "C" int pylc_image_pack(const float* img, int B, int Cimg, int H, int W, const float* mean3, const float* std3, float* out, void* stream) {
    return pylc_image_pack_denom(img, 0, B, Cimg, H, W, mean3, std3, 255.f, out, stream);
}

extern "C" int pylc_image_pack_u8(const unsigned char* img, int B, int Cimg, int H, int W, const float* mean3, const float* std3, float* out,
                                  void* stream) {
    return pylc_image_pack_denom(img, 1, B, Cimg, H, W, mean3, std3, 255.f, out, stream);
}

extern "C" int pylc_nhwc_to_nchw(const float* x, int x_pitch, float* y, int B, int H, int W, int C, void* stream) {
    PYLC_REQUIRE(x && y && B > 0 && H > 0 && W > 0 && C > 0 && x_pitch >= C, "nhwc_to_nchw: bad arguments");
    hipLaunchKernelGGL(nhwc_to_nchw_kernel, dim3(grid_for((long long)B * H * W * C)), dim3(256), 0, as_stream(stream), x, x_pitch, y, B, H * W, C);
    PYLC_LAUNCH_CHECK();
    return PYLC_OK;
}

extern "C" int pylc_nchw_to_nhwc(const float* x, float* y, int y_pitch, int B, int H, int W, int C, void* stream) {
    PYLC_REQUIRE(x && y && B > 0 && H > 0 && W > 0 && C > 0 && y_pitch >= C, "nchw_to_nhwc: bad arguments");
    hipLaunchKernelGGL(nchw_to_nhwc_kernel, dim3(grid_for((long long)B * H * W * C)), dim3(256), 0, as_stream(stream), x, y, y_pitch, B, H * W, C);
    PYLC_LAUNCH_CHECK();
    return PYLC_OK;
}
```

pylc_amd/lib.py:

```python
import ctypes as C
import os

import torch

_HERE = os.path.dirname(os.path.abspath(__file__))
LIB_PATH = os.environ.get('PYLC_LIB') or os.path.join(_HERE, 'libpylc_hip.so')

ABI_VERSION = 15


class PylcError(RuntimeError):
    pass


class ConvDesc(C.Structure):
    _fields_ = [(n, C.c_int) for n in ('B', 'H', 'W', 'Cin', 'Cout', 'R', 'S', 'stride', 'pad', 'dil',
                                       'OH', 'OW', 'x_pitch', 'y_pitch')] + \
               [(n, C.c_void_p) for n in ('x_amax', 'w_amax', 'dy_amax',
                                          'w_planes', 'w_planes_t')] + \
               [(n, C.c_int) for n in ('x_fmt', 'dy_fmt', 'out_fmt')] + [('out_bound', C.c_void_p)] + \
               [('w_planes_fmt', C.c_int)]


class WPrepEntry(C.Structure):
    _fields_ = [('src_offset', C.c_longlong), ('fwd_offset', C.c_longlong), ('t_offset', C.c_longlong),
                ('tile_begin', C.c_longlong), ('K', C.c_int), ('RS', C.c_int), ('C', C.c_int), ('amax_index', C.c_int)]


class SlabSum(C.Structure):
    _fields_ = [('slabs', C.c_void_p), ('dw', C.c_void_p), ('n4', C.c_longlong), ('slab_stride', C.c_longlong), ('splits', C.c_int), ('reserved', C.c_int)]


class BnExtra(C.Structure):
    _fields_ = [('out_planes', C.c_void_p), ('out_plane_stride', C.c_longlong), ('out_bound', C.c_void_p),
                ('res_planes', C.c_void_p), ('res_plane_stride', C.c_longlong), ('res_amax', C.c_void_p),
                ('dy_planes', C.c_void_p), ('dy_plane_stride', C.c_longlong), ('dy_bound', C.c_void_p),
                ('nplanes', C.c_int), ('drop_p', C.c_float), ('drop_seed', C.c_uint64), ('g_amax', C.c_void_p), ('relu_mask', C.c_void_p), ('y_half_bound', C.c_void_p), ('dout_half_bound', C.c_void_p)]


class BnBack(C.Structure):
    _fields_ = [('y', C.c_void_p), ('mean', C.c_void_p), ('invstd', C.c_void_p), ('scale', C.c_void_p), ('shift', C.c_void_p),
                ('relu_mask', C.c_void_p), ('relu', C.c_int), ('g_amax', C.c_void_p)]


class FwdEp(C.Structure):
    _fields_ = [('scale', C.c_void_p), ('shift', C.c_void_p), ('scale_amax', C.c_void_p), ('shift_amax', C.c_void_p), ('residual', C.c_void_p),
                ('res_fmt', C.c_int), ('res_scale_bound', C.c_void_p), ('res_amax', C.c_void_p), ('x_true_amax', C.c_void_p), ('relu', C.c_int),
                ('amax_out', C.c_void_p)]


class DwDesc(C.Structure):
    _fields_ = [(n, C.c_int) for n in ('B', 'H', 'W', 'C', 'stride', 'dil', 'OH', 'OW', 'x_pitch', 'y_pitch')]


_P = C.c_void_p
_I = C.c_int
_LL = C.c_longlong
_F = C.c_float
_D = C.c_double
_SZ = C.c_size_t

SIGNATURES = {
    'pylc_last_error': (C.c_char_p, []),
    'pylc_abi_version': (_I, []),
    'pylc_planes_stride': (_LL, [_LL, _I, _I]),
    'pylc_set_planes_interleave': (_I, [_I]),
    'pylc_experimental_build': (_I, []),
    'pylc_init': (_I, []),
    'pylc_set_conv_precision': (_I, [_I]),
    'pylc_get_conv_precision': (_I, []),
    'pylc_debug_set_big_tile': (_I, [_I]),
    'pylc_debug_pp_flags': (_I, [_I]),
    'pylc_debug_stagger': (_I, [_I]),
    'pylc_debug_wgrad_flags': (_I, [_I]),
    'pylc_debug_wgrad_max_steps': (_I, [_I]),
    'pylc_comm_available': (_I, []),
    'pylc_comm_unique_id': (_I, [_P]),
    'pylc_comm_init': (_I, [_P, _I, _I, C.POINTER(C.c_void_p)]),
    'pylc_comm_allreduce': (_I, [_P, _P, _LL, _I, _P]),
    'pylc_comm_syncbn_reduce': (_I, [_P, _P, _I, _P]),
    'pylc_comm_destroy': (_I, [_P]),
    'pylc_debug_dw_tiles': (_I, [_I]),
    'pylc_range_product': (_I, [_P, _P, _F, _P, _P, _P]),
    'pylc_maxpool_fwd_planes': (_I, [_P, _P, _LL, _I, _P, _P, _I, _I, _I, _I, _I, _I, _I, _I, _I, _P]),
    'pylc_upsample2_crop_concat_planes': (_I, [_P, _I, _I, _I, _I, _I, _P, _I, _I, _I, _I, _P, _LL, _I, _P, _P]),
    'pylc_conv1x1_fold_input_affine': (_I, [_P, _P, _P, _P, _I, _I, _P, _P, _P, _P]),
    'pylc_debug_wgrad_acc1': (_I, [_I]),
    'pylc_debug_wgrad_sets': (_I, [_I]),
    'pylc_debug_wgrad_m16': (_I, [_I]),
    'pylc_debug_wgrad_dma': (_I, [_I]),
    'pylc_debug_pp_stamps': (_I, [_P]),
    'pylc_amax': (_I, [_P, _LL, _I, _I, _P, _P]),
    'pylc_amax_segments': (_I, [_P, _P, _I, _P, _P]),
    'pylc_to_planes': (_I, [_P, _I, _P, _I, _LL, _LL, _I, _P, _I, _P]),
    'pylc_from_planes': (_I, [_P, _I, _LL, _P, _I, _LL, _I, _P, _I, _P]),
    'pylc_planes_colsum_workspace_floats': (C.c_size_t, [_I]),
    'pylc_planes_colsum': (_I, [_P, _I, _LL, _I, _P, _LL, _I, _P, _P, _P]),
    'pylc_weight_prepare': (_I, [_P, _P, _I, _LL, _P, _P, _I, _P]),
    'pylc_conv2d_dgrad_needs_f32_weights': (_I, [C.POINTER(ConvDesc)]),
    'pylc_conv2d_fwd': (_I, [C.POINTER(ConvDesc), _P, _P, _P, _P, _P]),
    'pylc_conv2d_fwd_bnact': (_I, [C.POINTER(ConvDesc), _P, _P, _P, _P, _P, _P, _I, _P, _P, _P]),
    'pylc_conv2d_fwd_bnact_ex': (_I, [C.POINTER(ConvDesc), _P, _P, _P, C.POINTER(FwdEp), _P, _P]),
    'pylc_conv2d_fwd_stats_floats': (_SZ, [C.POINTER(ConvDesc)]),
    'pylc_conv2d_fwd_stats': (_I, [C.POINTER(ConvDesc), _P, _P, _P, _P, _P, C.POINTER(_I), _P]),
    'pylc_conv2d_dgrad': (_I, [C.POINTER(ConvDesc), _P, _P, _P, _I, _P]),
    'pylc_conv2d_dgrad_add': (_I, [C.POINTER(ConvDesc), _P, _P, _P, _I, _P, _P, _P]),
    'pylc_relu_bwd_bits': (_I, [_P, _P, _P, _LL, _I, _P]),
    'pylc_conv2d_dgrad_bn_floats': (_SZ, [C.POINTER(ConvDesc)]),
    'pylc_conv2d_dgrad_bn': (_I, [C.POINTER(ConvDesc), _P, _P, _P, _I, _P, _P, C.POINTER(BnBack), _P, C.POINTER(_I), _P]),
    'pylc_bn_bwd_sums_from_partial': (_I, [_P, _I, _I, _P, _P, _P, _D, _P, _P, _P]),
    'pylc_conv2d_wgrad_workspace': (_SZ, [C.POINTER(ConvDesc)]),
    'pylc_conv2d_wgrad': (_I, [C.POINTER(ConvDesc), _P, _P, _P, _P, _P, _SZ, _P]),
    'pylc_conv2d_wgrad_slabs': (_I, [C.POINTER(ConvDesc), _P, _P, _P, _P, _SZ, C.POINTER(SlabSum), _P]),
    'pylc_splitk_reduce_batch': (_I, [_P, _P, _I, C.c_longlong, _P]),
    'pylc_weight_transpose': (_I, [_P, _P, _I, _I, _I, _P]),
    'pylc_dwconv3x3_fwd': (_I, [C.POINTER(DwDesc), _P, _P, _P, _P]),
    'pylc_dwconv3x3_fwd_stats_rows': (_I, [C.POINTER(DwDesc)]),
    'pylc_dwconv3x3_fwd_stats': (_I, [C.POINTER(DwDesc), _P, _P, _P, _P, _P]),
    'pylc_dwconv3x3_dgrad': (_I, [C.POINTER(DwDesc), _P, _P, _P, _P]),
    'pylc_dwconv3x3_dgrad_acc': (_I, [C.POINTER(DwDesc), _P, _P, _P, _I, _P]),
    'pylc_dwconv3x3_wgrad_workspace': (_SZ, [C.POINTER(DwDesc)]),
    'pylc_dwconv3x3_wgrad': (_I, [C.POINTER(DwDesc), _P, _P, _P, _P, _SZ, _P]),
    'pylc_dwconv3x3_half_ok': (_I, [C.POINTER(DwDesc)]),
    'pylc_dwconv3x3_fwd_h_stats_rows': (_I, [C.POINTER(DwDesc)]),
    'pylc_dwconv3x3_bn_ok': (_I, [C.POINTER(DwDesc)]),
    'pylc_dwconv3x3_fwd_h_bn': (_I, [C.POINTER(DwDesc), _P, _P, _P, _P, _I, _P, _P, _P, _P, _P, _P, _P]),
    'pylc_dwconv3x3_wgrad_h_bn': (_I, [C.POINTER(DwDesc), _P, _P, _P, _P, _I, _P, _P, _P, _P, _P, _SZ, _P]),
    'pylc_dwconv3x3_dgrad_h_add_ok': (_I, [C.POINTER(DwDesc)]),
    'pylc_dwconv3x3_dgrad_h_add': (_I, [C.POINTER(DwDesc), _P, _P, _P, _P, _P, _P, _P, _P]),
    'pylc_dwconv3x3_fwd_h': (_I, [C.POINTER(DwDesc), _P, _P, _P, _P, _P, _P, _P, _P]),
    'pylc_dwconv3x3_fwd_h_eval': (_I, [C.POINTER(DwDesc), _P, _P, _P, _P, _P, _P, _P, _P]),
    'pylc_dwconv3x3_dgrad_h': (_I, [C.POINTER(DwDesc), _P, _P, _P, _P, _P, _P, _I, _P, _P]),
    'pylc_dwconv3x3_wgrad_h': (_I, [C.POINTER(DwDesc), _P, _P, _P, _P, _P, _P, _SZ, _P]),
    'pylc_bn_workspace_floats': (_SZ, [_LL, _I]),
    'pylc_bn_stats': (_I, [_P, _LL, _I, _I, _P, _P, _P]),
    'pylc_bn_stats_from_partial': (_I, [_P, _I, _I, _P, _P]),
    'pylc_bn_finalize': (_I, [_P, _D, _I, _P, _P, _F, _F, _I, _P, _P, _P, _P, _P, _P, _P]),
    'pylc_bn_eval_coeffs': (_I, [_P, _P, _P, _P, _F, _I, _P, _P, _P]),
    'pylc_bn_eval_coeffs_full': (_I, [_P, _P, _P, _P, _F, _I, _P, _P, _P, _P, _P]),
    'pylc_bn_finalize_from_partial': (_I, [_P, _I, _D, _I, _P, _P, _F, _F, _I, _P, _P, _P, _P, _P, _P, _P]),
    'pylc_bn_finalize_ex': (_I, [_P, _D, _I, _P, _P, _F, _F, _I, _P, _P, _P, _P, _P, _P, _P, _F, _P, _P, _I, _LL, _P, _P]),
    'pylc_bn_local_moments': (_I, [_P, _D, _I, _P, _I, _LL, _P, _P, _P]),
    'pylc_bn_finalize_moments': (_I, [_P, _D, _I, _P, _P, _F, _F, _I, _P, _P, _P, _P, _P, _P, _P, _F, _P, _P, _P]),
    'pylc_bn_finalize_from_partial_ex': (_I, [_P, _I, _D, _I, _P, _P, _F, _F, _I, _P, _P, _P, _P, _P, _P, _P, _F, _P, _P, _I, _LL, _P, _P]),
    'pylc_bn_apply_ex': (_I, [_P, _I, _P, _P, _P, _I, _P, _I, _LL, _I, _I, _P, C.POINTER(BnExtra), _P]),
    'pylc_bn_bwd_reduce_ex': (_I, [_P, _I, _P, _I, _P, _I, _P, _P, _LL, _I, _I, _P, _P, _P, _P, _P, _D, C.POINTER(BnExtra), _P, _P]),
    'pylc_bn_bwd_bound': (_I, [_P, _P, _P, _D, _I, _P, _P, _P]),
    'pylc_bn_bwd_apply_ex': (_I, [_P, _I, _P, _I, _P, _I, _P, _P, _P, _P, _D, _LL, _I, _I, _P, _I, _P, _I, _P, _P, _P,
                                  C.POINTER(BnExtra), _P]),
    'pylc_bn_apply': (_I, [_P, _I, _P, _P, _P, _I, _P, _I, _LL, _I, _I, _P, _P]),
    'pylc_bn_bwd_reduce': (_I, [_P, _I, _P, _I, _P, _I, _P, _P, _LL, _I, _I, _P, _P, _P, _P, _P]),
    'pylc_bn_bwd_apply': (_I, [_P, _I, _P, _I, _P, _I, _P, _P, _P, _P, _D, _LL, _I, _I, _P, _I, _P, _I, _P, _P, _P, _P]),
    'pylc_bn_frozen_bwd': (_I, [_P, _I, _P, _I, _P, _I, _P, _P, _P, _LL, _I, _I, _P, _I, _P, _I, _P, _P, _P, _P, _P, C.POINTER(BnExtra), _P]),
    'pylc_relu_fwd': (_I, [_P, _I, _P, _I, _LL, _I, _P]),
    'pylc_relu_bwd': (_I, [_P, _I, _P, _I, _P, _I, _LL, _I, _P]),
    'pylc_maxpool_fwd': (_I, [_P, _P, _P, _I, _I, _I, _I, _I, _I, _I, _I, _I, _P]),
    'pylc_maxpool_bwd': (_I, [_P, _P, _P, _I, _I, _I, _I, _I, _I, _I, _I, _I, _P]),
    'pylc_maxpool_bwd_add': (_I, [_P, _P, _P, _I, _I, _I, _I, _I, _I, _I, _I, _I, _P, _I, _I, _I, _I, _I, _P]),
    'pylc_crop_copy': (_I, [_P, _I, _I, _I, _I, _I, _P, _I, _I, _I, _I, _I, _P]),
    'pylc_bilinear_fwd': (_I, [_P, _I, _P, _I, _I, _I, _I, _I, _I, _I, _P]),
    'pylc_bilinear_bwd': (_I, [_P, _I, _P, _I, _I, _I, _I, _I, _I, _I, _P]),
    'pylc_bilinear_bwd_workspace': (C.c_size_t, [_I, _I, _I, _I]),
    'pylc_bilinear_bwd_separable': (_I, [_P, _I, _P, _I, _I, _I, _I, _I, _I, _I, _P, _P, _P]),
    'pylc_gap_fwd': (_I, [_P, _P, _I, _I, _I, _P]),
    'pylc_gap_fwd_planes': (_I, [_P, _LL, _I, _P, _P, _I, _I, _I, _P]),
    'pylc_gap_bwd': (_I, [_P, _P, _I, _I, _I, _P]),
    'pylc_gap_bwd_acc': (_I, [_P, _P, _I, _I, _I, _I, _P]),
    'pylc_image_pack': (_I, [_P, _I, _I, _I, _I, C.POINTER(_F), C.POINTER(_F), _P, _P]),
    'pylc_image_pack_tiles': (_I, [_P, _I, _I, _I, _I, _I, _I, _I, C.POINTER(_F), C.POINTER(_F), _P, _P]),
    'pylc_stitch_argmax': (_I, [_P, _I, _I, _I, _I, _I, _I, _P, _P]),
    'pylc_colourize_resize': (_I, [_P, _I, _I, _P, _P, _I, _I, _P]),
    'pylc_image_pack_tiles_reflect': (_I, [_P, _I, _I, _I, _I, _I, _I, _I, _I, _I, C.POINTER(_F), C.POINTER(_F), _P, _P]),
    'pylc_stitch_overlap_argmax': (_I, [_P, _I, _I, _I, _I, _I, _I, _I, _P, _P, _P]),
    'pylc_resize_area_u8': (_I, [_P, _I, _I, _I, _I, _P, _I, _I, _P]),
    'pylc_class_encode_resize': (_I, [_P, _I, _I, _P, _I, _P, _I, _I, _P]),
    'pylc_class_encode_resize_ex': (_I, [_P, _I, _I, _P, _I, _P, _I, _I, _I, _P]),
    'pylc_image_pack_tiles_ex': (_I, [_P, _I, _I, _I, _I, _I, _I, _I, _I, C.POINTER(_F), C.POINTER(_F), _P, _P]),
    'pylc_image_pack_tiles_flip': (_I, [_P, _I, _I, _I, _I, _I, _I, _I, _I, C.POINTER(_F), C.POINTER(_F), _P, _P, _I]),
    'pylc_image_pack_tiles_reflect_ex': (_I, [_P, _I, _I, _I, _I, _I, _I, _I, _I, _I, C.POINTER(_F), C.POINTER(_F), _P, _P, _I]),
    'pylc_blend_accumulate': (_I, [_P, _I, _I, _I, _I, _I, _I, _I, _I, _I, _P, _I, _P]),
    'pylc_blend_finalize': (_I, [_P, _I, _I, _I, _I, _I, _I, _I, _P, _P, _P, _P]),
    'pylc_resize_bilinear_image': (_I, [_P, _I, _I, _I, _I, _P, _I, _I, _P]),
    'pylc_blend_resample_accumulate': (_I, [_P, _I, _I, _I, _I, _I, _I, _F, _I, _P, _I, _I, _I, _I, _P]),
    'pylc_ensemble_finalize': (_I, [_P, _I, _I, _I, _I, _F, _P, _P, _P, _P]),
    'pylc_image_pack_denom': (_I, [_P, _I, _I, _I, _I, _I, C.POINTER(_F), C.POINTER(_F), _F, _P, _P]),
    'pylc_image_pack_u8': (_I, [_P, _I, _I, _I, _I, C.POINTER(_F), C.POINTER(_F), _P, _P]),
    'pylc_extract_tiles': (_I, [_P, _I, _I, _I, _P, _I, _I, _I, _I, _I, _I, _P, _P, _P, _P, _P]),
    'pylc_tile_stats': (_I, [_P, _LL, _I, _I, _P, _I, _I, _P, _P, _P]),
    'pylc_augment_tiles': (_I, [_P, _P, _LL, _I, _I, _P, _P, _P, _LL, _I, _P, _P, _I, _P, _P, _P]),
    'pylc_confusion_matrix': (_I, [_P, _I, _P, _I, _LL, _I, _I, _P, _P]),
    'pylc_confusion_matrix_ex': (_I, [_P, _I, _P, _I, _LL, _I, _I, _P, _I, _P, _P]),
    'pylc_logits_score': (_I, [_P, _I, _P, _I, _LL, _I, _P, _P, _P]),
    'pylc_logits_score_ex': (_I, [_P, _I, _P, _I, _LL, _I, _P, _I, _P, _P]),
    'pylc_label_regions': (_I, [_P, _I, _I, _I, _I, _P, _P]),
    'pylc_region_sizes': (_I, [_P, _LL, _P, _P]),
    'pylc_sieve_regions': (_I, [_P, _P, _P, _I, _I, _I, _I, _I, _P, _P, _P, _P]),
    'pylc_nhwc_to_nchw': (_I, [_P, _I, _P, _I, _I, _I, _I, _P]),
    'pylc_nchw_to_nhwc': (_I, [_P, _P, _I, _I, _I, _I, _I, _P]),
    'pylc_multiloss_workspace_floats': (_SZ, [_LL, _I]),
    'pylc_multiloss_stats': (_I, [_P, _I, _P, _LL, _I, _P, _P, _P, _P]),
    'pylc_multiloss_finalize': (_I, [_P, _D, _I, _F, _F, _F, _P, _P]),
    'pylc_multiloss_bwd': (_I, [_P, _I, _P, _LL, _I, _P, _P, _D, _F, _F, _F, _P, _P, _I, _P, _P]),
    'pylc_multiloss_stats_ex': (_I, [_P, _I, _P, _I, _LL, _I, _I, _P, _P, _P, _P, _P]),
    'pylc_multiloss_finalize_ex': (_I, [_P, _I, _F, _F, _F, _P, _P]),
    'pylc_multiloss_bwd_ex': (_I, [_P, _I, _P, _I, _LL, _I, _I, _P, _P, _F, _F, _F, _P, _P, _I, _P, _P]),
    'pylc_sqnorm_workspace_floats': (_SZ, [_LL]),
    'pylc_grad_norm_clip': (_I, [_P, _LL, _F, _P, _P, _P]),
    'pylc_adamw_step': (_I, [_P, _P, _P, _P, _LL, _P, _F, _F, _F, _F, _F, _I, _P]),
    'pylc_adamw_step_ranges': (_I, [_P, _P, _P, _P, _LL, _P, _F, _F, _F, _F, _F, _I, _P, _I, _P, _P]),
    'pylc_sgd_step': (_I, [_P, _P, _P, _LL, _P, _F, _F, _I, _P]),
    'pylc_dropout': (_I, [_P, _I, _P, _I, _LL, _I, _F, C.c_uint64, _P]),
    'pylc_stream_create_cu_mask': (_I, [_I, _I, C.POINTER(_P)]),
    'pylc_stream_destroy': (_I, [_P]),
}


EXPERIMENTAL = ('pylc_conv2d_dgrad_bn_floats', 'pylc_conv2d_dgrad_bn', 'pylc_bn_bwd_sums_from_partial',
                'pylc_stream_create_cu_mask', 'pylc_stream_destroy')
HAS_EXPERIMENTAL = False


def _load():
    global HAS_EXPERIMENTAL
    if not os.path.exists(LIB_PATH):
        raise PylcError(
            'libpylc_hip.so is not built (%s). Build it with `python __graft_entry__.py` or '
            '`make -C pylc_amd/csrc`; there is no CPU fallback.' % LIB_PATH)
    lib = C.CDLL(LIB_PATH)
    HAS_EXPERIMENTAL = hasattr(lib, 'pylc_experimental_build') and lib.pylc_experimental_build() == 1
    for name, (res, args) in SIGNATURES.items():
        if name in EXPERIMENTAL and not HAS_EXPERIMENTAL:
            continue
        fn = getattr(lib, name)
        fn.restype = res
        fn.argtypes = args
    if lib.pylc_abi_version() != ABI_VERSION:
        raise PylcError('libpylc_hip.so ABI %d != binding ABI %d' % (lib.pylc_abi_version(), ABI_VERSION))
    return lib


lib = _load()
_initialised = False


def check(rc):
    if rc != 0:
        raise PylcError('libpylc_hip: %s (code %d)' % (lib.pylc_last_error().decode(), rc))


def _need_experimental(what):
    if not HAS_EXPERIMENTAL:
        raise PylcError('%s needs a library built with `make -C pylc_amd/csrc EXPERIMENTAL=1` (this one holds the product kernels only)' % what)


def init():
    global _initialised
    if not _initialised:
        check(lib.pylc_init())
        mode = os.environ.get('PYLC_CONV_PRECISION')
        if mode is not None:
            check(lib.pylc_set_conv_precision(int(mode)))
        flags = os.environ.get('PYLC_DEBUG_FLAGS')
        if flags is not None:
            lib.pylc_debug_pp_flags(int(flags))
        if os.environ.get('PYLC_NO_PLANE_INTERLEAVE'):
            lib.pylc_set_planes_interleave(0)
        for item in filter(None, (t.strip() for t in os.environ.get('PYLC_DEBUG_KNOBS', '').split(','))):
            name, _, val = item.partition('=')
            fn = getattr(lib, 'pylc_debug_' + name, None)
            if fn is None or name in ('pp_stamps',):
                raise PylcError('PYLC_DEBUG_KNOBS: no knob %r' % name)
            fn(int(val))
        _initialised = True


def stream():
    return torch.cuda.current_stream().cuda_stream


def ptr(t):
    if t is None:
        return None
    if not t.is_cuda:
        raise PylcError('pylc_amd ops need HIP device tensors (got %s); there is no CPU fallback' % t.device)
    return t.data_ptr()
```

pylc_amd/loss.py:

```python
import numpy as np
import torch
from torch import nn

from . import ops
from .runtime import runtime


class MultiLoss(nn.Module):

    def __init__(self, loss_weights, schema, ignore_index=None):
        super().__init__()
        self.ignore_index = None if ignore_index is None else int(ignore_index)
        self.bad_targets = None
        self.n_classes = schema['n_classes']
        self.codes = schema.get('class_codes')
        self.categories = schema.get('class_labels')
        self.weighted = bool(loss_weights['weighted'])
        w = loss_weights.get('weights')
        w = np.ones(self.n_classes, np.float32) if w is None else np.asarray(w, np.float32)
        if w.shape != (self.n_classes,):
            raise ValueError('class weights must have length n_classes=%d' % self.n_classes)
        self.register_buffer('weights', torch.from_numpy(w.copy()))
        self.dsc_weight = float(loss_weights['dice'])
        self.ce_weight = float(loss_weights['ce'])
        self.fl_weight = float(loss_weights['focal'])
        self.eps = 1e-8
        self.ce = self.dsc = self.fl = 0.

    def _check(self, pred, target):
        if not torch.is_tensor(pred):
            raise TypeError('Input type is not a torch.Tensor. Got {}'.format(type(pred)))
        if pred.dim() != 4 or pred.size(1) != self.n_classes:
            raise ValueError('Invalid input shape, we expect Bx{}xHxW. Got: {}'.format(self.n_classes, tuple(pred.shape)))
        if pred.size(0) != target.size(0) or pred.size(2) != target.size(1) or pred.size(3) != target.size(2):
            raise ValueError('Expected prediction {} to match target {}.'.format(tuple(pred.shape), tuple(target.shape)))
        if pred.device != target.device:
            raise ValueError('input and target must be in the same device. Got: {} and {}'.format(pred.device, target.device))

    def _all(self, pred, target, w_ce, w_d, w_f):
        self._check(pred, target)
        cw = self.weights if self.weighted else None
        if self.ignore_index is None:
            return ops.multiloss(pred, target, cw, w_ce, w_d, w_f, runtime.sync_group)
        if self.bad_targets is None or self.bad_targets.device != pred.device:
            self.bad_targets = torch.zeros(1, dtype=torch.int64, device=pred.device)
        return ops.multiloss(pred, target, cw, w_ce, w_d, w_f, runtime.sync_group, self.ignore_index, self.bad_targets)

    def forward(self, pred, target):
        losses = self._all(pred, target, self.ce_weight, self.dsc_weight, self.fl_weight)
        self.ce, self.dsc, self.fl = losses[1].detach(), losses[2].detach(), losses[3].detach()
        return losses[0]

    def ce_loss(self, pred, target):
        return self._all(pred, target, 1.0, 0.0, 0.0)[0]

    def dice_loss(self, pred, target):
        return self._all(pred, target, 0.0, 1.0, 0.0)[0]

    def focal_loss(self, pred, target):
        return self._all(pred, target, 0.0, 0.0, 1.0)[0]

    def all_losses(self, pred, target):
        return self._all(pred, target, self.ce_weight, self.dsc_weight, self.fl_weight)

    def print_settings(self):
        hline = '_' * 40
        print('{:30s}{:<10s}'.format('Loss', 'Weight'))
        print(hline)
        print('{:30s}{:<10f}'.format('Cross-entropy', self.ce_weight))
        print('\tCE losses {}weighted by class.'.format('' if self.weighted else 'not '))
        print('{:30s}{:<10f}'.format('Dice Coefficient', self.dsc_weight))
        print('{:30s}{:<10f}'.format('Focal Loss', self.fl_weight))
        if self.codes and self.categories:
            print('\n{:8s}{:22s}{:<10s}'.format('Class', 'Label', 'Weight'))
            print(hline)
            for i, w in enumerate(self.weights.tolist()):
                print('{:8s}{:22s}{:<10f}'.format(str(self.codes[i]), str(self.categories[i]), w))
```

pylc_amd/model.py:

```python
import numpy as np
import torch

from . import ops
from .loss import MultiLoss
from .nets import DeepLab, UNet
from .optim import FlatArena, FlatAdamW, FlatSGD, StepLR
from .runtime import runtime


class Meta:

    def __init__(self, **kw):
        self.arch = 'deeplab'
        self.backbone = 'resnet'
        self.ch = 3
        self.n_classes = 9
        self.class_codes = None
        self.class_labels = None
        self.px_mean = [132.47, 144.47, 149.45]
        self.px_std = [24.85, 22.04, 18.77]
        self.px_grayscale_mean = 142.01
        self.px_grayscale_std = 23.66
        self.normalize_default = False
        self.weights = None
        self.weighted = False
        self.dice_weight = 0.5
        self.ce_weight = 0.5
        self.focal_weight = 0.5
        self.lr = 1e-4
        self.weight_decay = 5e-5
        self.momentum = 0.9
        self.gamma = 0.9
        self.optim_type = 'adam'
        self.clip_norm = 0.5
        self.dropout = 0.5
        self.up_mode = 'upsample'
        self.pad_size = 94
        self.report = 20
        self.pretrained = False
        self.freeze_bn = False
        self.ignore_index = None
        for k, v in kw.items():
            if not hasattr(self, k):
                raise AttributeError('unknown Meta field %r' % k)
            setattr(self, k, v)

    def update(self, other):
        src = other if isinstance(other, dict) else vars(other)
        for k, v in src.items():
            if hasattr(self, k):
                setattr(self, k, v)
        return self


class LossLog:

    def __init__(self):
        self._pending = []
        self.intv = []
        self.train, self.valid, self.test, self.lr = [], [], [], []
        self.avg_dice, self.best_dice, self.is_best = 1.0, 1.0, False

    def save(self, path):
        self.flush()
        tmp = path + '.tmp'
        torch.save({'train': list(self.train), 'valid': list(self.valid), 'test': list(self.test), 'best_dice': float(self.best_dice),
                    'lr': list(self.lr)}, tmp)
        import os
        os.replace(tmp, path)

    def load(self, path, resume=True):
        import os
        import pickle
        if not os.path.exists(path):
            return False
        if not resume:
            os.remove(path)
            return False
        from .checkpoint import load_losses_file
        try:
            res = load_losses_file(path)
            rows = {k: [(int(row[0]),) + tuple(float(v) for v in row[1:]) for row in res.get(k, [])] for k in ('train', 'valid', 'test')}
            best = float(res['best_dice'])
        except (pickle.UnpicklingError, EOFError, ValueError, KeyError, TypeError, IndexError, RuntimeError) as e:
            if os.environ.get('PYLC_RESTART_LOSS_LOG') != '1':
                raise RuntimeError('losses.pth at %s is unreadable (%s: %s); fix or remove it, or set PYLC_RESTART_LOSS_LOG=1 to restart the '
                                   'loss log (best-Dice tracking restarts with it)' % (path, type(e).__name__, e)) from e
            import warnings
            warnings.warn('losses.pth at %s is unreadable (%s: %s); the loss log restarts (PYLC_RESTART_LOSS_LOG=1)' % (path, type(e).__name__, e))
            return False
        self.train, self.valid, self.test = rows['train'], rows['valid'], rows['test']
        self.best_dice = best
        return True

    def push(self, triple):
        self._pending.append(triple)

    def flush(self):
        if self._pending:
            vals = torch.stack(self._pending).cpu().tolist()
            self.intv += [tuple(v) for v in vals]
            self._pending = []
        return self.intv

    def log(self, it, training):
        self.flush()
        if self.intv:
            avg = tuple(np.mean(np.asarray(self.intv, np.float64), axis=0).tolist())
            if training:
                self.train.append((it,) + avg)
            else:
                self.valid.append((it,) + avg)
                self.avg_dice = avg[1]
                self.is_best = self.avg_dice < self.best_dice
                if self.is_best:
                    self.best_dice = self.avg_dice
        self.intv = []


class Model:
    def __init__(self, meta=None, device=None):
        self.meta = meta if meta is not None else Meta()
        self.device = torch.device(device if device is not None else 'cuda:0')
        self.net = self.crit = self.optim = self.sched = self.arena = None
        self.loss = LossLog()
        self.iter = 0
        self.epoch = 0
        self._bucketer = None
        self.scores = None
        self._best_by = 'dice'
        self._ranges_checked = False

    @property
    def best_by(self):
        return self._best_by

    @best_by.setter
    def best_by(self, rule):
        if rule not in ('dice', 'iou'):
            raise ValueError("best_by is 'dice' or 'iou', got %r" % (rule,))
        if rule == 'iou' and self.scores is None:
            raise ValueError("best_by='iou' needs Model.scores (a metrics.ScoreLog)")
        self._best_by = rule

    def update_meta(self, params):
        self.meta.update(params)
        return self

    def build(self):
        m = self.meta
        if m.arch == 'unet':
            if m.freeze_bn:
                raise ValueError('freeze_bn is not available for arch=unet: frozen BatchNorm is implemented for the DeepLab networks only '
                                 '(the U-Net keeps batch statistics in its training kernels)')
            self.net = UNet(in_channels=m.ch, n_classes=m.n_classes, up_mode=m.up_mode, dropout=m.dropout)
        elif m.arch == 'deeplab':
            self.net = DeepLab(backbone=m.backbone, n_classes=m.n_classes, in_channels=m.ch, freeze_bn=bool(m.freeze_bn), pretrained=False)
        else:
            raise ValueError('Model {} not available.'.format(m.arch))
        self.net = self.net.to(self.device)
        self.crit = MultiLoss(
            loss_weights={'weighted': m.weighted, 'weights': m.weights, 'ce': m.ce_weight, 'dice': m.dice_weight,
                          'focal': m.focal_weight},
            schema={'n_classes': m.n_classes, 'class_codes': m.class_codes, 'class_labels': m.class_labels},
            ignore_index=m.ignore_index).to(self.device)
        ign = None if m.ignore_index is None else int(m.ignore_index)
        if self.scores is not None and self.scores.ignore_index != ign:
            self.scores.ignore_index, self.scores.counts = ign, None
        self.init_optim()
        return self

    def init_optim(self):
        m = self.meta
        self.arena = FlatArena(self.net)
        if m.optim_type == 'adam':
            self.optim = FlatAdamW(self.arena, lr=m.lr, weight_decay=m.weight_decay, clip=m.clip_norm)
        elif m.optim_type == 'sgd':
            self.optim = FlatSGD(self.arena, lr=m.lr, momentum=m.momentum, clip=m.clip_norm)
        else:
            raise ValueError('Optimizer is not defined.')
        self.sched = StepLR(self.optim, m.gamma)

    def _stats(self, default=False):
        m = self.meta
        if m.ch == 1:
            if default:
                return [float(m.px_grayscale_mean)] * 3, [float(m.px_grayscale_std)] * 3, 1.0
            mean = float(np.mean(np.asarray(m.px_mean, np.float32)))
            std = float(np.mean(np.asarray(m.px_std, np.float32)))
            return [mean] * 3, [std] * 3, 255.0
        if default:
            return [132.47, 144.47, 149.45], [24.85, 22.04, 18.77], 255.0
        return list(m.px_mean), list(m.px_std), 255.0

    def pack_input(self, x, default=False):
        if x.dim() != 4 or x.shape[1] != self.meta.ch:
            raise ValueError('expected [B,%d,H,W] tiles, got %s' % (self.meta.ch, tuple(x.shape)))
        if x.dtype != torch.uint8:
            x = x.to(dtype=torch.float32)
        x = x.to(self.device, non_blocking=True)
        mean, std, denom = self._stats(default)
        return ops.image_pack(x, mean, std, denom)

    def _target(self, y):
        y = y.to(self.device, non_blocking=True)
        if self.meta.ignore_index is None or y.dtype != torch.uint8:
            y = y.long()
        return self.crop_target(y)

    def crop_target(self, y):
        if self.meta.arch == 'unet':
            p = self.meta.pad_size
            y = y[:, p:y.shape[1] - p, p:y.shape[2] - p]
        return y.contiguous()

    def train(self, x, y):
        self.net.train()
        if getattr(self.net, 'freeze_bn', False) and ops.nplanes() == 1:
            raise ValueError('freeze_bn is not available in conv precision mode 3: its half activations are scaled with range bounds '
                             'taken from batch statistics, which a frozen BatchNorm does not compute')
        self._ranges_checked = False
        x4 = self.pack_input(x)
        y = self._target(y)
        y_hat = self.net(x4)
        loss = self.crit(y_hat, y)
        self.loss.push(torch.stack((self.crit.ce, self.crit.dsc, self.crit.fl)))
        self.optim.zero_grad()
        if runtime.sync_group is not None:
            from .parallel import GradBucketer, assert_equal_shards
            if getattr(self, '_dp_batch', None) is None:
                assert_equal_shards(x.shape[0], runtime.sync_group)
                self._dp_batch = x.shape[0]
            if self._bucketer is None:
                self._bucketer = GradBucketer(self.arena, runtime.grad_group)
            self._bucketer.reset()
            runtime.grad_ready = self._bucketer.ready
        ops.reset_slab_sums()
        loss.backward()
        ops.sync_side_streams()
        self.arena.clear_undelivered()
        if runtime.sync_group is not None:
            runtime.grad_ready = None
            self._bucketer.finish()
        self.optim.step()
        if self.iter % self.meta.report == 0:
            self.log()
        self.loss.lr += [(self.iter, self.optim.lr)]
        self.iter += 1
        return loss.detach()

    def eval(self, x, y):
        self.net.eval()
        self._refresh_for_inference()
        x4 = self.pack_input(x)
        y = self._target(y)
        with torch.no_grad():
            y_hat = self.net(x4)
            self.loss.push(self.crit.all_losses(y_hat, y)[1:4])
            if self.scores is not None:
                if self.scores.ignore_index != self.meta.ignore_index:
                    raise ValueError('Model.scores has ignore_index=%r, Meta has %r' % (self.scores.ignore_index, self.meta.ignore_index))
                self.scores.add(y_hat, y)
        return [y_hat]

    def test(self, x):
        self._refresh_for_inference()
        x4 = self.pack_input(x, default=self.meta.normalize_default)
        with torch.no_grad():
            return [self.net(x4)]

    def predict(self, x):
        from . import metrics
        return metrics.logits_confusion(self.test(x)[0], return_mask=True)[1]

    def _refresh_for_inference(self):
        self.arena.refresh_if_changed(force=not self._ranges_checked)
        self._ranges_checked = True

    def log(self):
        if runtime.sync_group is not None:
            ops.check_equal_shards()
        training = self.net.training
        self.loss.log(self.iter, training)
        bad = getattr(self.crit, 'bad_targets', None)
        if bad is not None:
            n_bad = int(bad.item())
            if n_bad:
                bad.zero_()
                raise ValueError('%d targets since the last report lie outside 0..%d and are not ignore_index=%d'
                                 % (n_bad, self.meta.n_classes - 1, self.meta.ignore_index))
        if self._best_by == 'iou' and self.scores is None:
            raise ValueError("best_by='iou' needs Model.scores (a metrics.ScoreLog)")
        if not training and self.scores is not None:
            self.scores.close(self.iter, self.epoch, runtime.sync_group)
            if self._best_by == 'iou':
                self.loss.is_best = self.scores.is_best

    def get_lr(self):
        return self.optim.lr

    def model_id(self):
        return 'pylc_%s_ch%d_schema_%s' % (self.meta.arch, self.meta.ch, 'a' if self.meta.n_classes == 9 else 'b')

    def save(self, save_dir):
        import os
        from . import checkpoint, parallel
        rank0 = runtime.sync_group is None or parallel.rank() == 0
        if rank0:
            d = os.path.join(save_dir, self.model_id())
            os.makedirs(d, exist_ok=True)
            targets = [(os.path.join(d, 'checkpoint.pth'), False)]
            if self.loss.is_best:
                targets.append((os.path.join(d, self.model_id() + '.pth'), True))
            for path, best in targets:
                tmp = path + '.tmp.%d' % os.getpid()
                checkpoint.save(self, tmp, best=best)
                os.replace(tmp, path)
            self.loss.save(os.path.join(d, 'losses.pth'))
            if self.scores is not None:
                self.scores.save(os.path.join(d, 'scores.json'))
        if runtime.sync_group is not None:
            parallel.barrier(runtime.sync_group)
```

pylc_amd/nets/deeplabv3p.py:

```python
import torch
from torch import nn

from .. import ops
from ..layers import Conv2d, BatchNorm2d, Dropout, Named, conv_bn, bn_group
from ..runtime import runtime
from .encoder_resnet import ResNet101
from .encoder_xception import AlignedXception


class _ASPPBranch(nn.Module):
    def __init__(self, cin, cout, k, dilation):
        super().__init__()
        self.atrous_conv = Conv2d(cin, cout, k, 1, 0 if k == 1 else dilation, dilation, init='kaiming', bn=True)
        self.bn = BatchNorm2d(cout)

    def forward(self, x, link=None, into=None):
        return conv_bn(self.atrous_conv, self.bn, x, relu=True, conv_link=link, into=into)


class ASPP(nn.Module):
    def __init__(self, output_stride=16, inplanes=2048):
        super().__init__()
        dil = (1, 6, 12, 18) if output_stride == 16 else (1, 12, 24, 36)
        self.aspp1 = _ASPPBranch(inplanes, 256, 1, dil[0])
        self.aspp2 = _ASPPBranch(inplanes, 256, 3, dil[1])
        self.aspp3 = _ASPPBranch(inplanes, 256, 3, dil[2])
        self.aspp4 = _ASPPBranch(inplanes, 256, 3, dil[3])
        self.global_avg_pool = Named(_1=Conv2d(inplanes, 256, 1, init='kaiming', bn=True), _2=BatchNorm2d(256))
        self.conv1 = Conv2d(1280, 256, 1, init='kaiming', bn=True)
        self.bn1 = BatchNorm2d(256)
        self.dropout = Dropout(0.5)

    def forward(self, x):
        h, w = x.shape[2:]
        link = ops.grad_link(x)
        g = ops.global_avg_pool(x, link)
        buf = [ops.empty_nhwc(x.shape[0], 1280, h, w, x.device)]
        if (self.training and torch.is_grad_enabled() and runtime.sync_group is not None and runtime.sync_bn and runtime.coalesce_sync_bn
                and not self.bn1.frozen):
            pool_conv, pool_bn = self.global_avg_pool.child(1), self.global_avg_pool.child(2)
            brs = (self.aspp1, self.aspp2, self.aspp3, self.aspp4)
            ys = [br.atrous_conv(x, res_link=link) for br in brs]
            outs = bn_group([(br.bn, y, dict(relu=True, into=(buf, 256 * i))) for i, (br, y) in enumerate(zip(brs, ys))] +
                            [(pool_bn, pool_conv(g), dict(relu=True))])
            branches = outs[:4] + [ops.bilinear(outs[4], h, w, into=(buf, 1024))]
        else:
            g = conv_bn(self.global_avg_pool.child(1), self.global_avg_pool.child(2), g, relu=True)
            branches = [self.aspp1(x, link, (buf, 0)), self.aspp2(x, link, (buf, 256)), self.aspp3(x, link, (buf, 512)),
                        self.aspp4(x, link, (buf, 768)), ops.bilinear(g, h, w, into=(buf, 1024))]
        y = ops.concat_slices(buf, branches)
        return conv_bn(self.conv1, self.bn1, y, relu=True, drop=self.dropout)


class Decoder(nn.Module):
    def __init__(self, n_classes, low_level_inplanes):
        super().__init__()
        self.conv1 = Conv2d(low_level_inplanes, 48, 1, init='kaiming', bn=True)
        self.bn1 = BatchNorm2d(48)
        self.last_conv = Named(_0=Conv2d(304, 256, 3, 1, 1, init='kaiming', bn=True), _1=BatchNorm2d(256),
                               _4=Conv2d(256, 256, 3, 1, 1, init='kaiming', bn=True), _5=BatchNorm2d(256),
                               _8=Conv2d(256, n_classes, 1, bias=True, init='kaiming'))
        self.drop3, self.drop7 = Dropout(0.5), Dropout(0.1)
        import os
        self.last_conv.child(0).weight._pylc_wgrad_hold = int(runtime.decoder_hold[0])
        self.last_conv.child(4).weight._pylc_wgrad_hold = int(runtime.decoder_hold[1])

    def forward(self, x, low):
        b, _, lh, lw = low.shape
        cx, cl = x.shape[1], self.conv1.cout
        buf = [ops.empty_nhwc(b, cx + cl, lh, lw, x.device)]
        up = ops.bilinear(x, lh, lw, into=(buf, 0))
        low = conv_bn(self.conv1, self.bn1, low, relu=True, conv_link=ops.grad_link(low), into=(buf, cx))
        x = ops.concat_slices(buf, (up, low))
        lc = self.last_conv
        x = conv_bn(lc.child(0), lc.child(1), x, relu=True, out_planes=lc.child(4).takes_planes(), drop=self.drop3, sole=True)
        x = conv_bn(lc.child(4), lc.child(5), x, relu=True, drop=self.drop7)
        return lc.child(8)(x)


class DeepLab(nn.Module):

    def __init__(self, activ_func=None, normalizer=None, backbone='resnet', output_stride=16, n_classes=9, in_channels=3,
                 freeze_bn=False, pretrained=False):
        super().__init__()
        if backbone == 'resnet':
            self.backbone = ResNet101(output_stride)
            low_c = 256
        elif backbone == 'xception':
            self.backbone = AlignedXception(output_stride)
            low_c = 128
        else:
            raise ValueError('backbone %r not available (resnet | xception)' % backbone)
        self.aspp = ASPP(output_stride)
        self.decoder = Decoder(n_classes, low_c)
        self.in_channels = in_channels
        self.n_classes = n_classes
        self.freeze_bn = False
        if freeze_bn:
            self.set_bn_frozen(True)
        if pretrained:
            self.load_pretrained_backbone()

    def set_bn_frozen(self, on=True):
        from ..layers import DepthwiseConv3x3
        on = bool(on)
        for m in self.modules():
            if isinstance(m, BatchNorm2d):
                m.frozen = on
            elif isinstance(m, (Conv2d, DepthwiseConv3x3)):
                m.bn_frozen = on
        self.freeze_bn = on
        return self

    PRETRAINED_PATH = './data/models/resnet101-5d3b4d8f.pth'

    def load_pretrained_backbone(self, path=None):
        import torch
        if not isinstance(self.backbone, ResNet101):
            raise ValueError('pretrained weights exist for the resnet backbone only')
        path = path or self.PRETRAINED_PATH
        pretrain = torch.load(path, map_location='cpu', weights_only=True)
        own = self.backbone.state_dict()
        picked = {k: v for k, v in pretrain.items() if k in own}
        own.update(picked)
        self.backbone.load_state_dict(own)
        return sorted(picked)

    def forward(self, x):
        h, w = x.shape[2:]
        x4 = x if x.shape[1] == 4 else ops.pack_nchw(x, 4)
        f, low = self.backbone(x4, keep_planes=True)
        y = self.decoder(self.aspp(f), low)
        return ops.bilinear(y, h, w)
```

pylc_amd/ops/misc.py:

```python
from . import _core
from ._core import *


class ReluFn(torch.autograd.Function):
    @staticmethod
    def forward(ctx, x):
        L.init()
        x = as_nhwc(x)
        b, c, h, w = x.shape
        out = empty_nhwc(b, c, h, w, x.device)
        check(lib.pylc_relu_fwd(ptr(x), pitch_of(x), ptr(out), c, b * h * w, c, stream()))
        ctx.save_for_backward(out)
        return out

    @staticmethod
    def backward(ctx, dout):
        (out,) = ctx.saved_tensors
        dout = as_nhwc(dout)
        b, c, h, w = out.shape
        dx = empty_nhwc(b, c, h, w, out.device)
        check(lib.pylc_relu_bwd(ptr(dout), pitch_of(dout), ptr(out), c, ptr(dx), c, b * h * w, c, stream()))
        return dx


def relu(x):
    return ReluFn.apply(x)


class DropoutFn(torch.autograd.Function):
    @staticmethod
    def forward(ctx, x, p, seed):
        L.init()
        x = as_nhwc(x)
        b, c, h, w = x.shape
        out = empty_nhwc(b, c, h, w, x.device)
        check(lib.pylc_dropout(ptr(x), pitch_of(x), ptr(out), c, b * h * w, c, p, seed, stream()))
        ctx.cfg = (p, seed)
        return out

    @staticmethod
    def backward(ctx, dout):
        p, seed = ctx.cfg
        dout = as_nhwc(dout)
        b, c, h, w = dout.shape
        dx = empty_nhwc(b, c, h, w, dout.device)
        check(lib.pylc_dropout(ptr(dout), pitch_of(dout), ptr(dx), c, b * h * w, c, p, seed, stream()))
        return dx, None, None


def dropout(x, p, seed):
    out = DropoutFn.apply(x, p, seed)
    if ranges_needed() and 0.0 <= p < 1.0:
        binades = 0
        while (1 << binades) * (1.0 - p) < 1.0:
            binades += 1
        inherit_amax(out, x, binades)
    return out


class MaxPoolFn(torch.autograd.Function):
    @staticmethod
    def forward(ctx, x, k, stride, pad, link=None, planes_bound=None):
        L.init()
        x = as_nhwc(x)
        if pitch_of(x) != x.shape[1]:
            x = x.contiguous(memory_format=torch.channels_last)
        b, c, h, w = x.shape
        oh, ow = (h + 2 * pad - k) // stride + 1, (w + 2 * pad - k) // stride + 1
        y = empty_nhwc(b, c, oh, ow, x.device)
        need_idx = ctx.needs_input_grad[0]
        idx = torch.empty((b, oh, ow, c), device=x.device, dtype=torch.uint8) if need_idx else None
        if planes_bound is not None:
            check(lib.pylc_maxpool_fwd_planes(ptr(x), ptr(y), pstride(b * oh * ow, c), nplanes(), ptr(planes_bound), ptr(idx), b, h, w, c, k, stride, pad,
                                              oh, ow, stream()))
        else:
            check(lib.pylc_maxpool_fwd(ptr(x), ptr(y), ptr(idx), b, h, w, c, k, stride, pad, oh, ow, stream()))
        ctx.save_for_backward(idx)
        ctx.cfg = (b, c, h, w, k, stride, pad, oh, ow)
        ctx.link = link if need_idx else None
        if ctx.link is not None:
            link.pool_armed = True
        return y

    @staticmethod
    def backward(ctx, dy):
        (idx,) = ctx.saved_tensors
        b, c, h, w, k, stride, pad, oh, ow = ctx.cfg
        dy = as_nhwc(dy)
        if pitch_of(dy) != c:
            dy = dy.contiguous(memory_format=torch.channels_last)
        dx = empty_nhwc(b, c, h, w, dy.device)
        link = ctx.link
        crop = None
        if link is not None:
            link.pool_armed = False
            crop, link.crop = link.crop, None
        if crop is not None:
            g, c0, h0, w0 = crop
            check(lib.pylc_maxpool_bwd_add(ptr(dy), ptr(idx), ptr(dx), b, h, w, c, k, stride, pad, oh, ow, g.data_ptr() + 4 * c0, pitch_of(g),
                                           h0, w0, g.shape[2], g.shape[3], stream()))
        else:
            check(lib.pylc_maxpool_bwd(ptr(dy), ptr(idx), ptr(dx), b, h, w, c, k, stride, pad, oh, ow, stream()))
        return dx, None, None, None, None, None


def maxpool(x, k, stride, pad=0, link=None, out_planes=False):
    b, c, h, w = x.shape
    oh, ow = (h + 2 * pad - k) // stride + 1, (w + 2 * pad - k) // stride + 1
    if (out_planes and (torch.is_grad_enabled() or _runtime.eval_planes) and ranges_needed() and not _runtime.no_planes and not is_planes(x) and c % 8 == 0
            and planes_ok(c, b * oh * ow) and b * oh * ow >= _core.PLANES_MIN_PIXELS and _runtime.pool_planes):
        bound = amax_of(x)
        return mark_planes(MaxPoolFn.apply(x, k, stride, pad, link, bound), bound)
    y = MaxPoolFn.apply(x, k, stride, pad, link)
    return inherit_amax(y, x) if ranges_needed() else y


class CropConcatFn(torch.autograd.Function):

    @staticmethod
    def forward(ctx, up, bridge, holder, link):
        L.init()
        buf = holder[0]
        bridge = as_nhwc(bridge)
        b, cu, th, tw = up.shape
        cb, hh, ww = bridge.shape[1:]
        if (tuple(buf.shape) != (b, cu + cb, th, tw) or pitch_of(buf) != cu + cb or up.data_ptr() != buf.data_ptr() or cu % 4 or cb % 4
                or th > hh or tw > ww):
            raise L.PylcError('crop_concat: `up` must be the leading channels of the [B, C_up + C_bridge, h, w] buffer')
        h0, w0 = (hh - th) // 2, (ww - tw) // 2
        check(lib.pylc_crop_copy(ptr(bridge), pitch_of(bridge), hh, ww, h0, w0, buf.data_ptr() + 4 * cu, cu + cb, b, th, tw, cb, stream()))
        ctx.geom = (cu, cb, hh, ww, h0, w0)
        ctx.link = link if ctx.needs_input_grad[1] else None
        return buf

    @staticmethod
    def backward(ctx, dy):
        cu, cb, hh, ww, h0, w0 = ctx.geom
        dy = as_nhwc(dy)
        d_up = dy[:, :cu] if ctx.needs_input_grad[0] else None
        d_bridge = None
        if ctx.needs_input_grad[1]:
            link = ctx.link
            if link is not None and link.pool_armed and link.crop is None:
                link.crop = (dy, cu, h0, w0)
            else:
                d_bridge = zeros_nhwc(dy.shape[0], cb, hh, ww, dy.device)
                d_bridge[:, :, h0:h0 + dy.shape[2], w0:w0 + dy.shape[3]] = dy[:, cu:]
        return d_up, d_bridge, None, None


def crop_concat(up, bridge, holder, link=None):
    return CropConcatFn.apply(up, bridge, holder, link)


class UpCatPlanesFn(torch.autograd.Function):

    @staticmethod
    def forward(ctx, z, bridge, bound, link):
        L.init()
        z, bridge = as_nhwc(z), as_nhwc(bridge)
        b, c1, h, w = z.shape
        c2, hh, ww = bridge.shape[1:]
        oh, ow = 2 * h, 2 * w
        out = empty_nhwc(b, c1 + c2, oh, ow, z.device)
        check(lib.pylc_upsample2_crop_concat_planes(ptr(z), pitch_of(z), b, h, w, c1, ptr(bridge), pitch_of(bridge), hh, ww, c2, ptr(out),
                                                    pstride(b * oh * ow, c1 + c2), nplanes(), ptr(bound), stream()))
        ctx.geom = (b, c1, h, w, c2, hh, ww, (hh - oh) // 2, (ww - ow) // 2)
        ctx.link = link if ctx.needs_input_grad[1] else None
        return out

    @staticmethod
    def backward(ctx, dy):
        b, c1, h, w, c2, hh, ww, h0, w0 = ctx.geom
        dy = as_nhwc(dy)
        oh, ow = 2 * h, 2 * w
        dz = d_bridge = None
        if ctx.needs_input_grad[0]:
            dz = empty_nhwc(b, c1, h, w, dy.device)
            tmp = torch.empty(lib.pylc_bilinear_bwd_workspace(b, w, c1, oh) // 4, device=dy.device, dtype=torch.float32)
            amax = torch.empty(1, dtype=torch.int32, device=dy.device) if ranges_needed() and _runtime.fused_grad_ranges else None
            check(lib.pylc_bilinear_bwd_separable(ptr(dy), pitch_of(dy), ptr(dz), c1, b, h, w, c1, oh, ow, ptr(tmp), ptr(amax), stream()))
            if amax is not None:
                tag_amax(dz, amax)
        if ctx.needs_input_grad[1]:
            link = ctx.link
            if link is not None and link.pool_armed and link.crop is None:
                link.crop = (dy, c1, h0, w0)
            else:
                d_bridge = zeros_nhwc(b, c2, hh, ww, dy.device)
                d_bridge[:, :, h0:h0 + oh, w0:w0 + ow] = dy[:, c1:]
        return dz, d_bridge, None, None


def upsample2_crop_concat(z, bridge, link=None):
    c1, c2 = z.shape[1], bridge.shape[1]
    pixels = z.shape[0] * 4 * z.shape[2] * z.shape[3]
    if not ((torch.is_grad_enabled() or _runtime.eval_planes) and ranges_needed() and not _runtime.no_planes and c1 % 8 == 0 and c2 % 8 == 0 and planes_ok(c1 + c2, pixels)
            and pixels >= _core.PLANES_MIN_PIXELS and not is_planes(z) and _runtime.upcat_planes):
        return None
    bound = torch.maximum(amax_of(z), amax_of(bridge))
    out = UpCatPlanesFn.apply(z, bridge, bound, link)
    return mark_planes(out, bound)


class ConcatSlicesFn(torch.autograd.Function):

    @staticmethod
    def forward(ctx, holder, *parts):
        buf = holder[0]
        c0 = 0
        offs = []
        for p in parts:
            if p.data_ptr() != buf.data_ptr() + 4 * c0 or tuple(p.shape[2:]) != tuple(buf.shape[2:]) or pitch_of(p) != pitch_of(buf):
                raise L.PylcError('concat_slices: part at channel %d is not that slice of the buffer' % c0)
            offs.append((c0, p.shape[1]))
            c0 += p.shape[1]
        if c0 != buf.shape[1]:
            raise L.PylcError('concat_slices: the parts cover %d of %d channels' % (c0, buf.shape[1]))
        ctx.offs = offs
        return buf

    @staticmethod
    def backward(ctx, dy):
        dy = as_nhwc(dy)
        return (None,) + tuple(dy[:, c0:c0 + c] for c0, c in ctx.offs)


def concat_slices(holder, parts):
    out = ConcatSlicesFn.apply(holder, *parts)
    if ranges_needed():
        tags = [getattr(t, '_pylc_amax', None) for t in parts]
        if all(tg is not None and tg[1] == t._version for tg, t in zip(tags, parts)):
            a = tags[0][0]
            for tg in tags[1:]:
                a = torch.maximum(a, tg[0])
            tag_amax(out, a)
    return out


class BilinearFn(torch.autograd.Function):

    @staticmethod
    def forward(ctx, x, oh, ow, into=None):
        L.init()
        x = as_nhwc(x)
        b, c, h, w = x.shape
        cp = pitch_of(x)
        cc = _r4(c)
        if cc > cp:
            raise L.PylcError('bilinear: channel count %d needs a pitch >= %d' % (c, cc))
        if into is not None:
            buf, c0 = into[0][0], into[1]
            if tuple(buf.shape[2:]) != (oh, ow) or buf.shape[0] != b or c0 % 4 or c % 4 or c0 + c > buf.shape[1]:
                raise L.PylcError('bilinear into=: slice [%d, %d) does not fit the %s buffer' % (c0, c0 + c, tuple(buf.shape)))
            y, yp = buf[:, c0:c0 + c], pitch_of(buf)
        else:
            y, yp = empty_nhwc(b, c, oh, ow, x.device, cc), cc
        check(lib.pylc_bilinear_fwd(ptr(x), cp, ptr(y), yp, b, h, w, cc, oh, ow, stream()))
        ctx.cfg = (b, c, h, w, oh, ow)
        return y

    @staticmethod
    def backward(ctx, dy):
        b, c, h, w, oh, ow = ctx.cfg
        dy = as_nhwc(dy)
        cc = _r4(c)
        if pitch_of(dy) < cc:
            t = zeros_nhwc(b, c, oh, ow, dy.device, cc)
            t.copy_(dy)
            dy = t
        dx = empty_nhwc(b, c, h, w, dy.device, cc)
        if oh >= 2 * h and ow >= 2 * w:
            tmp = torch.empty(lib.pylc_bilinear_bwd_workspace(b, w, cc, oh) // 4, device=dy.device, dtype=torch.float32)
            amax = torch.empty(1, dtype=torch.int32, device=dy.device) if ranges_needed() and _runtime.fused_grad_ranges else None
            check(lib.pylc_bilinear_bwd_separable(ptr(dy), pitch_of(dy), ptr(dx), cc, b, h, w, cc, oh, ow, ptr(tmp), ptr(amax), stream()))
            if amax is not None:
                tag_amax(dx, amax)
        else:
            check(lib.pylc_bilinear_bwd(ptr(dy), pitch_of(dy), ptr(dx), cc, b, h, w, cc, oh, ow, stream()))
        return dx, None, None, None


def bilinear(x, oh, ow, into=None):
    y = BilinearFn.apply(x, oh, ow, into)
    return inherit_amax(y, x) if ranges_needed() else y


class GapFn(torch.autograd.Function):
    @staticmethod
    def forward(ctx, x, res_link=None):
        L.init()
        b, c, h, w = x.shape
        y = empty_nhwc(b, c, 1, 1, x.device)
        if is_planes(x) and c % 8 == 0 and _runtime.gap_planes:
            check(lib.pylc_gap_fwd_planes(ptr(x), pstride(b * h * w, c), nplanes(), ptr(planes_amax(x)), ptr(y), b, h * w, c, stream()))
        else:
            x = as_nhwc(x)
            if pitch_of(x) != x.shape[1]:
                x = x.contiguous(memory_format=torch.channels_last)
            check(lib.pylc_gap_fwd(ptr(x), ptr(y), b, h * w, c, stream()))
        ctx.cfg = (b, c, h, w)
        ctx.res_link = res_link if (res_link is not None and ctx.needs_input_grad[0]) else None
        if ctx.res_link is not None:
            res_link.pending += 1
        return y

    @staticmethod
    def backward(ctx, dy):
        b, c, h, w = ctx.cfg
        dy = dy.reshape(b, c).contiguous()
        link = ctx.res_link
        sink = _link_sink(link)
        dx = sink if sink is not None else empty_nhwc(b, c, h, w, dy.device)
        check(lib.pylc_gap_bwd_acc(ptr(dy), ptr(dx), b, h * w, c, 1 if sink is not None else 0, stream()))
        if link is not None:
            link.pending -= 1
            if link.pending > 0:
                link.buf, dx = dx, None
            else:
                link.buf = None
        return dx, None


def global_avg_pool(x, res_link=None):
    return GapFn.apply(x, res_link)


def image_pack(img, mean3, std3, denom=255.0):
    L.init()
    b, c, h, w = img.shape
    img = img.contiguous()
    out = empty_nhwc(b, 4, h, w, img.device)
    m = (C.c_float * 3)(*[float(v) for v in mean3])
    s = (C.c_float * 3)(*[float(v) for v in std3])
    u8 = img.dtype == torch.uint8
    src = img if u8 else img.float()
    check(lib.pylc_image_pack_denom(ptr(src), int(u8), b, c, h, w, m, s, float(denom), ptr(out), stream()))
    return out


def pack_nchw(x, pitch):
    L.init()
    b, c, h, w = x.shape
    x = x.contiguous()
    out = zeros_nhwc(b, pitch, h, w, x.device)
    check(lib.pylc_nchw_to_nhwc(ptr(x), ptr(out), pitch, b, h, w, c, stream()))
    return out


_shard_pairs = {}


def _shard_pair(b, dev):
    key = (int(b), str(dev))
    if key not in _shard_pairs:
        _shard_pairs[key] = torch.tensor([float(b), float(b) * float(b)], device=dev)
    return _shard_pairs[key]


SHARD_PAIRS_MAX = 64


def note_shard_pair(pair, world):
    pend = _runtime.shard_check
    if pend is None:
        pend = _runtime.shard_check = {'pairs': [], 'world': world, 'worst': None}
    pend['pairs'].append(pair)
    pend['world'] = world
    if len(pend['pairs']) >= SHARD_PAIRS_MAX:
        _fold_shard_pairs(pend)


def _shard_violation(pairs, world):
    p = torch.stack([q.double() for q in pairs])
    viol = (p[:, 1] * world - p[:, 0] * p[:, 0]).abs()
    k = torch.argmax(viol)
    return torch.stack([viol[k], p[k, 0], p[k, 1]])


def _fold_shard_pairs(pend):
    v = _shard_violation(pend['pairs'], pend['world'])
    pend['pairs'] = []
    pend['worst'] = v if pend['worst'] is None else torch.where(v[0] > pend['worst'][0], v, pend['worst'])


def check_equal_shards():
    pend, _runtime.shard_check = _runtime.shard_check, None
    if pend is None:
        return
    if isinstance(pend, tuple):
        pend = {'pairs': [pend[0]], 'world': pend[1], 'worst': None}
    world = pend['world']
    cands = [] if pend['worst'] is None else [pend['worst']]
    if pend['pairs']:
        cands.append(_shard_violation(pend['pairs'], world))
    if not cands:
        return
    viol, sb, sb2 = max((tuple(float(x) for x in c.cpu().tolist()) for c in cands), key=lambda t: t[0])
    if viol > 0.5:
        raise RuntimeError('data-parallel ranks hold different batch sizes (sum b = %g, sum b^2 = %g over %d ranks in one of the steps since the '
                           'last check): SyncBN and the loss head need equal shards -- use a drop_last loader' % (sb, sb2, world))


class MultiLossFn(torch.autograd.Function):

    @staticmethod
    def forward(ctx, logits, target, class_weights, w_ce, w_dice, w_focal, group, ignore_index=None, bad=None):
        L.init()
        logits = as_nhwc(logits)
        b, c, h, w = logits.shape
        n = b * h * w
        target = target.contiguous()
        ctx.ignore = ignore_index
        if ignore_index is not None:
            return MultiLossFn._forward_ignore(ctx, logits, target, class_weights, w_ce, w_dice, w_focal, group, int(ignore_index), bad)
        if target.dtype != torch.int64 or tuple(target.shape) != (b, h, w):
            raise L.PylcError('target must be int64 [B,H,W] matching the logits')
        dev = logits.device
        st = stream()
        k = 3 + 3 * c
        stats = torch.empty(k + (2 if group is not None else 0), device=dev)
        ws = torch.empty(lib.pylc_multiloss_workspace_floats(n, c), device=dev)
        check(lib.pylc_multiloss_stats(ptr(logits), pitch_of(logits), ptr(target), n, c, ptr(class_weights), ptr(stats), ptr(ws), st))
        n_global = float(n)
        if group is not None:
            stats[k:].copy_(_shard_pair(b, dev), non_blocking=True)
            _runtime.sync_all_reduce(stats, group)
            n_global = float(n) * dist.get_world_size(group)
            note_shard_pair(stats[k:], dist.get_world_size(group))
        losses = torch.empty(4, device=dev)
        check(lib.pylc_multiloss_finalize(ptr(stats), n_global, c, w_ce, w_dice, w_focal, ptr(losses), st))
        ctx.save_for_backward(logits, target, stats, class_weights)
        ctx.cfg = (n_global, w_ce, w_dice, w_focal, group)
        return losses

    @staticmethod
    def _forward_ignore(ctx, logits, target, class_weights, w_ce, w_dice, w_focal, group, ignore_index, bad):
        b, c, h, w = logits.shape
        n = b * h * w
        if target.dtype not in (torch.uint8, torch.int64) or tuple(target.shape) != (b, h, w):
            raise L.PylcError('target must be uint8 or int64 [B,H,W] matching the logits')
        if bad is not None and (bad.dtype != torch.int64 or bad.numel() != 1 or bad.device != logits.device):
            raise L.PylcError('bad must be an int64 [1] tensor on the device of the logits')
        dev = logits.device
        st = stream()
        k = 3 + 3 * c
        stats = torch.empty(k + (2 if group is not None else 0), device=dev)
        ws = torch.empty(lib.pylc_multiloss_workspace_floats(n, c), device=dev)
        check(lib.pylc_multiloss_stats_ex(ptr(logits), pitch_of(logits), ptr(target), target.element_size(), n, c, ignore_index,
                                          ptr(class_weights), ptr(stats), ptr(ws), ptr(bad), st))
        if group is not None:
            stats[k:].copy_(_shard_pair(b, dev), non_blocking=True)
            _runtime.sync_all_reduce(stats, group)
            note_shard_pair(stats[k:], dist.get_world_size(group))
        losses = torch.empty(4, device=dev)
        check(lib.pylc_multiloss_finalize_ex(ptr(stats), c, w_ce, w_dice, w_focal, ptr(losses), st))
        ctx.save_for_backward(logits, target, stats, class_weights)
        ctx.cfg = (None, w_ce, w_dice, w_focal, group)
        return losses

    @staticmethod
    def backward(ctx, dlosses):
        logits, target, stats, cw = ctx.saved_tensors
        n_global, w_ce, w_dice, w_focal, group = ctx.cfg
        b, c, h, w = logits.shape
        n = b * h * w
        gs = dlosses[0:1].contiguous().float()
        cp = _r4(c)
        dl = empty_nhwc(b, c, h, w, logits.device, cp)
        amax = torch.empty(1, dtype=torch.int32, device=logits.device) if ranges_needed() and _runtime.fused_grad_ranges else None
        ignore = getattr(ctx, 'ignore', None)
        if ignore is None:
            check(lib.pylc_multiloss_bwd(ptr(logits), pitch_of(logits), ptr(target), n, c, ptr(cw), ptr(stats), n_global,
                                         w_ce, w_dice, w_focal, ptr(gs), ptr(dl), cp, ptr(amax), stream()))
        else:
            check(lib.pylc_multiloss_bwd_ex(ptr(logits), pitch_of(logits), ptr(target), target.element_size(), n, c, int(ignore), ptr(cw),
                                            ptr(stats), w_ce, w_dice, w_focal, ptr(gs), ptr(dl), cp, ptr(amax), stream()))
        if amax is not None:
            tag_amax(dl, amax)
        return dl, None, None, None, None, None, None, None, None


def multiloss(logits, target, class_weights, w_ce, w_dice, w_focal, group=None, ignore_index=None, bad=None):
    return MultiLossFn.apply(logits, target, class_weights, w_ce, w_dice, w_focal, group, ignore_index, bad)


__all__ = [n for n in dir() if not n.startswith('__')]
```

pylc_amd/runtime.py:

```python
import itertools
import os


class _Runtime:
    def side_stream_on(self):
        if self.wgrad_side_stream is None:
            from .lib import lib
            return lib.pylc_get_conv_precision() == 3
        return bool(self.wgrad_side_stream)

    def __init__(self):
        self.sync_group = None
        self.sync_bn = os.environ.get('PYLC_SYNC_BN', '1') != '0'
        self.coalesce_sync_bn = True
        self.bn_refine = True
        self.defer_wgrad_1x1 = False
        self.wgrad_hold = True
        self.grad_group = None
        self.grad_ready = None
        self.wgrad_side_stream = False if os.environ.get('PYLC_NO_SIDE_STREAM') else (True if os.environ.get('PYLC_SIDE_STREAM') else None)
        self.wgrad_cus = 0
        self.no_relu_bits = False
        self.fuse_res_grad = True
        self.skip_zero_bias_grad = True
        self.defer_bn_apply = True
        self.upcat_planes = True
        self.fused_grad_ranges = True
        self.gap_planes = True
        self.batch_slab_sums = True
        self.fuse_bn_sums = False
        self.half_acts = True
        self.half_dw = True
        self.eval_planes = True
        self.fuse_eval_bn = True
        self.bn_clamp_eps = False
        self.dropout_enabled = True
        self.no_planes = False
        self.planes_dy = True
        self.pool_planes = True
        self.fold_planes = True
        self.dw_wgrad_side = True
        self.adamw_ranges = True
        self.grad_overlap = True
        self.decoder_hold = (0, 0)
        self.debug_planes = False
        self.debug_streams = False
        self.planes_only = ''
        self.planes_fwd_only = False
        self.comm = None
        self.grad_comm = None
        self.shard_check = None
        self.collectives = 0
        self.seed = 0x5EED
        self._counter = itertools.count(1)
        self._apply_overrides(os.environ.get('PYLC_RUNTIME', ''))

    def _apply_overrides(self, spec):
        for item in filter(None, (t.strip() for t in spec.split(','))):
            name, _, val = item.partition('=')
            if not hasattr(self, name) or name.startswith('_'):
                raise ValueError('PYLC_RUNTIME: no runtime attribute %r' % name)
            low = val.strip().lower()
            if low in ('true', 'false'):
                v = low == 'true'
            else:
                try:
                    v = int(val)
                except ValueError:
                    try:
                        v = float(val)
                    except ValueError:
                        v = val
            if isinstance(getattr(self, name), bool) and isinstance(v, int):
                v = bool(v)
            setattr(self, name, v)

    def sync_all_reduce(self, t, group):
        self.collectives += 1
        if self.comm is not None and t.is_cuda and group is self.sync_group and self.native_takes(t):
            self.native_all_reduce(t)
            return
        import torch.distributed as dist
        dist.all_reduce(t, group=group)

    @staticmethod
    def native_takes(t):
        import torch
        return t.is_contiguous() and t.dtype in (torch.float32, torch.float64)

    def native_all_reduce(self, t, comm=None):
        import torch
        from .lib import lib, check, ptr, stream
        if not self.native_takes(t):
            raise ValueError('native all-reduce takes contiguous fp32 / fp64 tensors, got %s %s' % (t.dtype, tuple(t.stride())))
        check(lib.pylc_comm_allreduce(comm if comm is not None else self.comm, ptr(t), t.numel(), 0 if t.dtype == torch.float32 else 1, stream()))

    def next_seed(self):
        return (self.seed * 0x9E3779B97F4A7C15 + next(self._counter) * 0xD1B54A32D192ED03) & 0xFFFFFFFFFFFFFFFF

    def manual_seed(self, seed, rank=0):
        self.seed = (int(seed) * 1000003 + rank) & 0xFFFFFFFF
        self._counter = itertools.count(1)


runtime = _Runtime()
```

Measured before the change: 441.0 tiles/s.

## Fuse final bilinear upsample into loss kernels and upsample into decoder concat

Adds loss stats and backward kernels that interpolate the low-resolution logits on the fly, so the full 512x512 upsampled logits and their gradient are never materialised. The backward uses a separable gather over candidate output columns and then a row-axis reduction. It also adds a fused upsample-plus-concat-to-planes kernel for the decoder, which removes the intermediate NHWC buffer. The trade-off is recomputing softmax per contributing output pixel in backward, plus more complex index logic.

New measurement: 444.4 tiles/s, median of 6. Within noise of the previous version (+0.8%).

```diff
diff --git a/include/pylc_hip.h b/include/pylc_hip.h
--- a/include/pylc_hip.h
+++ b/include/pylc_hip.h
@@ -68,6 +68,8 @@
 size_t pylc_planes_colsum_workspace_floats(int C);
 int pylc_upsample2_crop_concat_planes(const float* z, int z_pitch, int B, int h, int w, int C1, const float* bridge, int bridge_pitch, int HH, int WW,
                                       int C2, void* planes, long long plane_stride, int nplanes, const unsigned int* bound, void* stream);
+int pylc_upsample_concat_planes(const float* z, int z_pitch, int B, int h, int w, int C1, const float* bridge, int bridge_pitch, int OH, int OW,
+                                int C2, void* planes, long long plane_stride, int nplanes, const unsigned int* bound, void* stream);
 int pylc_planes_colsum(const void* planes, int p_pitch, long long plane_stride, int nplanes, const unsigned int* amax, long long M, int C,
                        float* sums, float* workspace, void* stream);
 
@@ -357,6 +359,14 @@
 int pylc_multiloss_bwd_ex(const float* logits, int pitch, const void* target, int target_bytes, long long N, int C, int ignore_index,
                           const float* class_weights, const float* stats, float w_ce, float w_dice, float w_focal,
                           const float* grad_scale, float* dlogits, int dpitch, unsigned int* amax_bits, void* stream);
+int pylc_multiloss_stats_up(const float* low, int pitch, int B, int H, int W, int OH, int OW, const void* target, int target_bytes, int C,
+                            int use_ignore, int ignore_index, const float* class_weights, float* stats, float* workspace,
+                            unsigned long long* n_bad, void* stream);
+size_t pylc_multiloss_bwd_up_workspace(int B, int W, int C, int OH);
+int pylc_multiloss_bwd_up(const float* low, int pitch, int B, int H, int W, int OH, int OW, const void* target, int target_bytes, int C,
+                          int use_ignore, int ignore_index, const float* class_weights, const float* stats, double n_global, float w_ce,
+                          float w_dice, float w_focal, const float* grad_scale, float* dlow, int dpitch, float* workspace,
+                          unsigned int* amax_bits, void* stream);
 
 size_t pylc_sqnorm_workspace_floats(long long n);
 int pylc_grad_norm_clip(const float* g, long long n, float max_norm, float* out2, float* workspace, void* stream);
diff --git a/pylc_amd/csrc/common.h b/pylc_amd/csrc/common.h
--- a/pylc_amd/csrc/common.h
+++ b/pylc_amd/csrc/common.h
@@ -94,4 +94,7 @@
     }
 }
 
+int bilinear_bwd_axis1(const float* tmp, int tmp_pitch, float* dx, int dx_pitch, int B, int H, int W, int C, int OH, unsigned int* amax_bits,
+                       void* stream);
+
 }
diff --git a/pylc_amd/csrc/loss.hip b/pylc_amd/csrc/loss.hip
--- a/pylc_amd/csrc/loss.hip
+++ b/pylc_amd/csrc/loss.hip
@@ -20,6 +20,57 @@
 #pragma unroll
     for (int c = 0; c < C; ++c) p[c] *= inv;
     lse = zmax + logf(sum);
+}
+
+template <int C>
+__device__ __forceinline__ void stats_px(const float (&z)[C], int t, const float* __restrict__ cw, float (&acc)[3 + 3 * C]) {
+    float p[C], lse;
+    softmax_px<C>(z, p, lse);
+    float zt = 0.f, pt = 0.f;
+#pragma unroll
+    for (int c = 0; c < C; ++c) {
+        const bool is = (c == t);
+        zt = is ? z[c] : zt;
+        pt = is ? p[c] : pt;
+        acc[3 + c] += is ? p[c] : 0.f;
+        acc[3 + C + c] += p[c];
+        acc[3 + 2 * C + c] += is ? 1.f : 0.f;
+    }
+    const float w = cw != nullptr ? cw[t] : 1.f;
+    acc[0] += w * (lse - zt);
+    acc[1] += w;
+    const float q = pt + kFlEps;
+    const float omq = 1.f - q;
+    acc[2] += -kFlAlpha * omq * omq * logf(q);
+}
+
+struct UpGeom { int H, W, OH, OW; float sh, sw; };
+struct LLerp { int i0, i1; float w0, w1; };
+__device__ __forceinline__ LLerp llerp_of(int dst, float scale, int in_size) {
+    const float src = scale * (float)dst;
+    LLerp l;
+    l.i0 = (int)src;
+    if (l.i0 > in_size - 1) l.i0 = in_size - 1;
+    l.i1 = l.i0 + (l.i0 < in_size - 1 ? 1 : 0);
+    l.w1 = src - (float)l.i0;
+    l.w0 = 1.f - l.w1;
+    return l;
+}
+__device__ __forceinline__ void lcand_range(int i, float scale, int out_size, int& lo, int& hi) {
+    if (scale <= 0.f) { lo = 0; hi = out_size - 1; return; }
+    lo = (int)floorf((float)(i - 1) / scale) - 1;
+    hi = (int)ceilf((float)(i + 1) / scale) + 1;
+    if (lo < 0) lo = 0;
+    if (hi > out_size - 1) hi = out_size - 1;
+}
+template <int C>
+__device__ __forceinline__ void up_row(const float* __restrict__ img, int pitch, int W, const LLerp& lh, const LLerp& lw, float (&z)[C]) {
+    const float* p00 = img + ((size_t)lh.i0 * W + lw.i0) * pitch;
+    const float* p01 = img + ((size_t)lh.i0 * W + lw.i1) * pitch;
+    const float* p10 = img + ((size_t)lh.i1 * W + lw.i0) * pitch;
+    const float* p11 = img + ((size_t)lh.i1 * W + lw.i1) * pitch;
+#pragma unroll
+    for (int c = 0; c < C; ++c) z[c] = lh.w0 * (lw.w0 * p00[c] + lw.w1 * p01[c]) + lh.w1 * (lw.w0 * p10[c] + lw.w1 * p11[c]);
 }
 
 template <int C, typename TT, bool IGN>
@@ -37,28 +88,49 @@
             if (tl == ignore) continue;
             if ((unsigned long long)tl >= (unsigned long long)C) { ++bad; continue; }
         }
-        float z[C], p[C], lse;
+        float z[C];
         const float* src = logits + n * pitch;
 #pragma unroll
         for (int c = 0; c < C; ++c) z[c] = src[c];
-        softmax_px<C>(z, p, lse);
-        const int t = (int)tl;
-        float zt = 0.f, pt = 0.f;
-#pragma unroll
-        for (int c = 0; c < C; ++c) {
-            const bool is = (c == t);
-            zt = is ? z[c] : zt;
-            pt = is ? p[c] : pt;
-            acc[3 + c] += is ? p[c] : 0.f;
-            acc[3 + C + c] += p[c];
-            acc[3 + 2 * C + c] += is ? 1.f : 0.f;
-        }
-        const float w = cw != nullptr ? cw[t] : 1.f;
-        acc[0] += w * (lse - zt);
-        acc[1] += w;
-        const float q = pt + kFlEps;
-        const float omq = 1.f - q;
-        acc[2] += -kFlAlpha * omq * omq * logf(q);
+        stats_px<C>(z, (int)tl, cw, acc);
+    }
+    float* dst = partial + (size_t)blockIdx.x * (3 + 3 * C);
+#pragma unroll
+    for (int k = 0; k < 3 + 3 * C; ++k) {
+        const float s = block_sum_256(acc[k], red);
+        if (threadIdx.x == 0) dst[k] = s;
+    }
+    if constexpr (IGN) {
+        if (n_bad != nullptr) {
+            unsigned long long wave_bad = 0;
+            for (int l = 0; l < 64; ++l) wave_bad += (unsigned)__shfl((int)bad, l, 64);
+            if ((threadIdx.x & 63) == 0 && wave_bad != 0) atomicAdd(n_bad, wave_bad);
+        }
+    }
+}
+
+template <int C, typename TT, bool IGN>
+__global__ __launch_bounds__(256) void multiloss_stats_up_kernel(const float* __restrict__ low, int pitch, UpGeom g, const TT* __restrict__ target,
+                                                                 long long N, const float* __restrict__ cw, float* __restrict__ partial,
+                                                                 long long ignore, unsigned long long* __restrict__ n_bad) {
+    __shared__ float red[4];
+    float acc[3 + 3 * C];
+#pragma unroll
+    for (int k = 0; k < 3 + 3 * C; ++k) acc[k] = 0.f;
+    unsigned int bad = 0;
+    const long long per_img = (long long)g.OH * g.OW;
+    for (long long n = (long long)blockIdx.x * blockDim.x + threadIdx.x; n < N; n += (long long)gridDim.x * blockDim.x) {
+        const long long tl = (long long)target[n];
+        if constexpr (IGN) {
+            if (tl == ignore) continue;
+            if ((unsigned long long)tl >= (unsigned long long)C) { ++bad; continue; }
+        }
+        const int b = (int)(n / per_img);
+        const int r = (int)(n - b * per_img);
+        const int oh = r / g.OW, ow = r - oh * g.OW;
+        float z[C];
+        up_row<C>(low + (size_t)b * g.H * g.W * pitch, pitch, g.W, llerp_of(oh, g.sh, g.H), llerp_of(ow, g.sw, g.W), z);
+        stats_px<C>(z, (int)tl, cw, acc);
     }
     float* dst = partial + (size_t)blockIdx.x * (3 + 3 * C);
 #pragma unroll
@@ -108,29 +180,62 @@
 
 typedef float loss_f4 __attribute__((ext_vector_type(4)));
 
+template <int C>
+struct GradCoef { float dA[C], dB[C], gs, ce_norm, inv_n, w_d, w_f; };
+template <int C, bool IGN>
+__device__ __forceinline__ GradCoef<C> grad_coef(const float* __restrict__ stats, float inv_n, float w_ce, float w_d, float w_f,
+                                                 const float* __restrict__ grad_scale) {
+    GradCoef<C> k;
+#pragma unroll
+    for (int c = 0; c < C; ++c) {
+        const float I = stats[3 + c], K = stats[3 + C + c] + stats[3 + 2 * C + c];
+        const float den = K + kDiceSmooth;
+        k.dA[c] = -2.f / den / (float)C;
+        k.dB[c] = (2.f * I + kDiceSmooth) / (den * den) / (float)C;
+    }
+    k.gs = grad_scale != nullptr ? grad_scale[0] : 1.f;
+    if constexpr (IGN) {
+        const double nv = stats_n_valid(stats, C);
+        inv_n = nv > 0.0 ? (float)(1.0 / nv) : 0.f;
+        k.ce_norm = stats[1] > 0.f ? w_ce / stats[1] : 0.f;
+    } else {
+        k.ce_norm = w_ce / stats[1];
+    }
+    k.inv_n = inv_n;
+    k.w_d = w_d;
+    k.w_f = w_f;
+    return k;
+}
+template <int C>
+__device__ __forceinline__ void grad_px(const float (&z)[C], int t, const float* __restrict__ cw, const GradCoef<C>& k, float (&d)[C]) {
+    float p[C], lse;
+    softmax_px<C>(z, p, lse);
+    float pt = 0.f;
+#pragma unroll
+    for (int c = 0; c < C; ++c) pt = (c == t) ? p[c] : pt;
+    const float w = cw != nullptr ? cw[t] : 1.f;
+    const float q = pt + kFlEps, omq = 1.f - q;
+    const float fprime = kFlAlpha * 2.f * omq * logf(q) - kFlAlpha * omq * omq / q;
+    const float fcoef = k.w_f * k.inv_n * fprime * pt;
+    float gdot = 0.f;
+#pragma unroll
+    for (int c = 0; c < C; ++c) gdot += ((c == t ? k.dA[c] : 0.f) + k.dB[c]) * p[c];
+#pragma unroll
+    for (int c = 0; c < C; ++c) {
+        const float o = (c == t) ? 1.f : 0.f;
+        const float gc = (c == t ? k.dA[c] : 0.f) + k.dB[c];
+        const float dd = k.ce_norm * w * (p[c] - o) + k.w_d * p[c] * (gc - gdot) + fcoef * (o - p[c]);
+        d[c] = k.gs * dd;
+    }
+}
+
 template <int C, typename TT, bool IGN>
 __global__ __launch_bounds__(256) void multiloss_bwd_kernel(const float* __restrict__ logits, int pitch, const TT* __restrict__ target,
                                                             long long N, const float* __restrict__ cw, const float* __restrict__ stats,
                                                             float inv_n, float w_ce, float w_d, float w_f,
                                                             const float* __restrict__ grad_scale, float* __restrict__ dlogits, int dpitch,
                                                             int Cstore, unsigned* __restrict__ amax_out, long long ignore, int zero16) {
-    float dA[C], dB[C];
-#pragma unroll
-    for (int c = 0; c < C; ++c) {
-        const float I = stats[3 + c], K = stats[3 + C + c] + stats[3 + 2 * C + c];
-        const float den = K + kDiceSmooth;
-        dA[c] = -2.f / den / (float)C;
-        dB[c] = (2.f * I + kDiceSmooth) / (den * den) / (float)C;
-    }
-    const float gs = grad_scale != nullptr ? grad_scale[0] : 1.f;
-    float ce_norm;
-    if constexpr (IGN) {
-        const double nv = stats_n_valid(stats, C);
-        inv_n = nv > 0.0 ? (float)(1.0 / nv) : 0.f;
-        ce_norm = stats[1] > 0.f ? w_ce / stats[1] : 0.f;
-    } else {
-        ce_norm = w_ce / stats[1];
-    }
+    const GradCoef<C> k = grad_coef<C, IGN>(stats, inv_n, w_ce, w_d, w_f, grad_scale);
     float gmax = 0.f;
     for (long long n = (long long)blockIdx.x * blockDim.x + threadIdx.x; n < N; n += (long long)gridDim.x * blockDim.x) {
         const long long tl = (long long)target[n];
@@ -145,34 +250,62 @@
                 continue;
             }
         }
-        float z[C], p[C], lse;
+        float z[C], d[C];
         const float* src = logits + n * pitch;
 #pragma unroll
         for (int c = 0; c < C; ++c) z[c] = src[c];
-        softmax_px<C>(z, p, lse);
-        const int t = (int)tl;
-        float pt = 0.f;
-#pragma unroll
-        for (int c = 0; c < C; ++c) pt = (c == t) ? p[c] : pt;
-        const float w = cw != nullptr ? cw[t] : 1.f;
-        const float q = pt + kFlEps, omq = 1.f - q;
-        const float fprime = kFlAlpha * 2.f * omq * logf(q) - kFlAlpha * omq * omq / q;
-        const float fcoef = w_f * inv_n * fprime * pt;
-        float gdot = 0.f;
-#pragma unroll
-        for (int c = 0; c < C; ++c) gdot += ((c == t ? dA[c] : 0.f) + dB[c]) * p[c];
+        grad_px<C>(z, (int)tl, cw, k, d);
         float* dst = dlogits + n * dpitch;
 #pragma unroll
         for (int c = 0; c < C; ++c) {
-            const float o = (c == t) ? 1.f : 0.f;
-            const float gc = (c == t ? dA[c] : 0.f) + dB[c];
-            const float d = ce_norm * w * (p[c] - o) + w_d * p[c] * (gc - gdot) + fcoef * (o - p[c]);
-            dst[c] = gs * d;
-            gmax = fmaxf(gmax, fabsf(gs * d));
+            dst[c] = d[c];
+            gmax = fmaxf(gmax, fabsf(d[c]));
         }
         for (int c = C; c < Cstore; ++c) dst[c] = 0.f;
     }
     if (amax_out != nullptr) amax_commit(gmax, amax_out);
+}
+
+template <int C, typename TT, bool IGN>
+__global__ __launch_bounds__(256) void multiloss_bwd_upx_kernel(const float* __restrict__ low, int pitch, UpGeom g, int B, const TT* __restrict__ target,
+                                                                const float* __restrict__ cw, const float* __restrict__ stats, float inv_n,
+                                                                float w_ce, float w_d, float w_f, const float* __restrict__ grad_scale,
+                                                                float* __restrict__ tmp, int Cstore, long long ignore) {
+    const GradCoef<C> k = grad_coef<C, IGN>(stats, inv_n, w_ce, w_d, w_f, grad_scale);
+    const long long total = (long long)B * g.OH * g.W;
+    for (long long idx = (long long)blockIdx.x * blockDim.x + threadIdx.x; idx < total; idx += (long long)gridDim.x * blockDim.x) {
+        const long long row = idx / g.W;
+        const int i = (int)(idx - row * g.W);
+        const int b = (int)(row / g.OH), oh = (int)(row - (long long)b * g.OH);
+        const LLerp lh = llerp_of(oh, g.sh, g.H);
+        const float* img = low + (size_t)b * g.H * g.W * pitch;
+        const TT* trow = target + row * g.OW;
+        int lo, hi;
+        lcand_range(i, g.sw, g.OW, lo, hi);
+        float acc[C];
+#pragma unroll
+        for (int c = 0; c < C; ++c) acc[c] = 0.f;
+        for (int o = lo; o <= hi; ++o) {
+            const LLerp l = llerp_of(o, g.sw, g.W);
+            if (l.i0 != i && l.i1 != i) continue;
+            float wt = 0.f;
+            if (l.i0 == i) wt += l.w0;
+            if (l.i1 == i) wt += l.w1;
+            const long long tl = (long long)trow[o];
+            if constexpr (IGN) {
+                if (tl == ignore || (unsigned long long)tl >= (unsigned long long)C) continue;
+            }
+            float z[C], d[C];
+            up_row<C>(img, pitch, g.W, lh, l, z);
+            grad_px<C>(z, (int)tl, cw, k, d);
+#pragma unroll
+            for (int c = 0; c < C; ++c) acc[c] += wt * d[c];
+        }
+        float* dst = tmp + idx * Cstore;
+#pragma unroll
+        for (int c = 0; c < C; ++c) dst[c] = acc[c];
+        for (int c = C; c < Cstore; ++c) dst[c] = 0.f;
+    }
 }
 
 #define PYLC_FOR_C(MACRO)                                                                                              \
@@ -309,3 +442,93 @@
     return multiloss_bwd_impl(logits, pitch, target, target_bytes, true, N, C, (long long)ignore_index, cw, stats, 1.0, w_ce, w_dice, w_focal,
                               grad_scale, dlogits, dpitch, amax_bits, stream);
 }
+
+static inline float up_scale(int in, int out) { return out > 1 ? (float)(in - 1) / (float)(out - 1) : 0.f; }
+
+static int check_up_args(const char* what, const float* low, int pitch, int B, int H, int W, int OH, int OW, const void* target, int target_bytes,
+                         int C, int use_ignore) {
+    PYLC_REQUIRE(C >= 2 && C <= MAXC, "%s: n_classes=%d unsupported (2..%d)", what, C, MAXC);
+    PYLC_REQUIRE(target_bytes == 8 || (use_ignore && target_bytes == 1), "%s: target_bytes=%d (8: int64; 1: uint8, with an ignore label only)", what,
+                 target_bytes);
+    PYLC_REQUIRE(low && target, "%s: low or target is NULL", what);
+    PYLC_REQUIRE(B > 0 && H > 0 && W > 0 && OH > 0 && OW > 0, "%s: B=%d, %dx%d -> %dx%d must be positive", what, B, H, W, OH, OW);
+    PYLC_REQUIRE(pitch >= C, "%s: pitch=%d below n_classes=%d", what, pitch, C);
+    PYLC_REQUIRE(target_bytes != 8 || (reinterpret_cast<uintptr_t>(target) & 7) == 0, "%s: an int64 target is not 8-byte aligned", what);
+    return PYLC_OK;
+}
+
+extern "C" int pylc_multiloss_stats_up(const float* low, int pitch, int B, int H, int W, int OH, int OW, const void* target, int target_bytes, int C,
+                                       int use_ignore, int ignore_index, const float* cw, float* stats, float* workspace,
+                                       unsigned long long* n_bad, void* stream) {
+    if (int rc = check_up_args("multiloss_stats_up", low, pitch, B, H, W, OH, OW, target, target_bytes, C, use_ignore)) return rc;
+    PYLC_REQUIRE(stats && workspace && (reinterpret_cast<uintptr_t>(n_bad) & 7) == 0, "multiloss_stats_up: stats or workspace is NULL / n_bad unaligned");
+    hipStream_t st = as_stream(stream);
+    const long long N = (long long)B * OH * OW;
+    const UpGeom g{H, W, OH, OW, up_scale(H, OH), up_scale(W, OW)};
+    const long long ignore = (long long)ignore_index;
+    if (!use_ignore) n_bad = nullptr;
+    const int blocks = (int)(cdiv<long long>(N, 256) < kLossBlocks ? cdiv<long long>(N, 256) : kLossBlocks);
+#define LAUNCH_SUP_T(CC, TT, IGN)                                                                                                              \
+    hipLaunchKernelGGL((multiloss_stats_up_kernel<CC, TT, IGN>), dim3(blocks), dim3(256), 0, st, low, pitch, g, static_cast<const TT*>(target), N, \
+                       cw, workspace, ignore, n_bad)
+    if (!use_ignore) {
+#define LAUNCH_SUP(CC) LAUNCH_SUP_T(CC, long long, false)
+        PYLC_FOR_C(LAUNCH_SUP)
+#undef LAUNCH_SUP
+    } else if (target_bytes == 8) {
+#define LAUNCH_SUP(CC) LAUNCH_SUP_T(CC, long long, true)
+        PYLC_FOR_C(LAUNCH_SUP)
+#undef LAUNCH_SUP
+    } else {
+#define LAUNCH_SUP(CC) LAUNCH_SUP_T(CC, unsigned char, true)
+        PYLC_FOR_C(LAUNCH_SUP)
+#undef LAUNCH_SUP
+    }
+#undef LAUNCH_SUP_T
+    PYLC_LAUNCH_CHECK();
+    const int K = 3 + 3 * C;
+    hipLaunchKernelGGL(column_sum_kernel, dim3(cdiv(K, 8)), dim3(256), 0, st, workspace, blocks, K, stats);
+    PYLC_LAUNCH_CHECK();
+    return PYLC_OK;
+}
+
+extern "C" size_t pylc_multiloss_bwd_up_workspace(int B, int W, int C, int OH) {
+    return (size_t)B * OH * W * (size_t)((C + 3) & ~3) * sizeof(float);
+}
+
+extern "C" int pylc_multiloss_bwd_up(const float* low, int pitch, int B, int H, int W, int OH, int OW, const void* target, int target_bytes, int C,
+                                     int use_ignore, int ignore_index, const float* cw, const float* stats, double n_global, float w_ce, float w_dice,
+                                     float w_focal, const float* grad_scale, float* dlow, int dpitch, float* workspace, unsigned int* amax_bits,
+                                     void* stream) {
+    if (int rc = check_up_args("multiloss_bwd_up", low, pitch, B, H, W, OH, OW, target, target_bytes, C, use_ignore)) return rc;
+    const int C4 = (C + 3) & ~3;
+    PYLC_REQUIRE(stats && dlow && workspace && (use_ignore || n_global > 0), "multiloss_bwd_up: stats, dlow or workspace is NULL / n_global <= 0");
+    PYLC_REQUIRE(OH >= H && OW >= W, "multiloss_bwd_up: %dx%d -> %dx%d is not an up-sampling in both axes", H, W, OH, OW);
+    PYLC_REQUIRE(dpitch >= C4 && dpitch % 4 == 0 && (reinterpret_cast<uintptr_t>(dlow) & 15) == 0 && (reinterpret_cast<uintptr_t>(workspace) & 15) == 0,
+                 "multiloss_bwd_up: dpitch=%d must be a multiple of 4 >= %d; dlow and workspace 16-byte aligned", dpitch, C4);
+    hipStream_t st = as_stream(stream);
+    const UpGeom g{H, W, OH, OW, up_scale(H, OH), up_scale(W, OW)};
+    const long long ignore = (long long)ignore_index;
+    const float inv_n = use_ignore ? 0.f : (float)(1.0 / n_global);
+    const long long total = (long long)B * OH * W;
+    const int blocks = (int)(cdiv<long long>(total, 256) < 8192 ? cdiv<long long>(total, 256) : 8192);
+#define LAUNCH_BUP_T(CC, TT, IGN)                                                                                                              \
+    hipLaunchKernelGGL((multiloss_bwd_upx_kernel<CC, TT, IGN>), dim3(blocks), dim3(256), 0, st, low, pitch, g, B, static_cast<const TT*>(target), cw, \
+                       stats, inv_n, w_ce, w_dice, w_focal, grad_scale, workspace, C4, ignore)
+    if (!use_ignore) {
+#define LAUNCH_BUP(CC) LAUNCH_BUP_T(CC, long long, false)
+        PYLC_FOR_C(LAUNCH_BUP)
+#undef LAUNCH_BUP
+    } else if (target_bytes == 8) {
+#define LAUNCH_BUP(CC) LAUNCH_BUP_T(CC, long long, true)
+        PYLC_FOR_C(LAUNCH_BUP)
+#undef LAUNCH_BUP
+    } else {
+#define LAUNCH_BUP(CC) LAUNCH_BUP_T(CC, unsigned char, true)
+        PYLC_FOR_C(LAUNCH_BUP)
+#undef LAUNCH_BUP
+    }
+#undef LAUNCH_BUP_T
+    PYLC_LAUNCH_CHECK();
+    return bilinear_bwd_axis1(workspace, C4, dlow, dpitch, B, H, W, C4, OH, amax_bits, stream);
+}
diff --git a/pylc_amd/csrc/planes.hip b/pylc_amd/csrc/planes.hip
--- a/pylc_amd/csrc/planes.hip
+++ b/pylc_amd/csrc/planes.hip
@@ -242,3 +242,25 @@
     PYLC_LAUNCH_CHECK();
     return PYLC_OK;
 }
+
+extern "C" int pylc_upsample_concat_planes(const float* z, int z_pitch, int B, int h, int w, int C1, const float* bridge, int bridge_pitch, int OH,
+                                           int OW, int C2, void* planes, long long plane_stride, int nplanes, const unsigned int* bound, void* stream) {
+    PYLC_REQUIRE(z && bridge && planes && bound && B > 0 && h > 0 && w > 0 && OH > 0 && OW > 0 && C1 > 0 && C2 > 0 && C1 % 8 == 0 && C2 % 8 == 0 &&
+                     (nplanes == 1 || nplanes == 2),
+                 "upsample_concat_planes: bad arguments (channel counts must be multiples of 8)");
+    PYLC_REQUIRE(z_pitch >= C1 && bridge_pitch >= C2 && z_pitch % 4 == 0 && bridge_pitch % 4 == 0 && B <= 65535 && OH <= 65535 &&
+                     (long long)B * OH * OW * (C1 + C2) < (1ll << 31) && (reinterpret_cast<uintptr_t>(planes) & 15) == 0 && plane_stride % 8 == 0 &&
+                     (reinterpret_cast<uintptr_t>(z) & 15) == 0 && (reinterpret_cast<uintptr_t>(bridge) & 15) == 0,
+                 "upsample_concat_planes: bad pitch / more than 2^31 elements / unaligned tensors");
+    PYLC_REQUIRE(nplanes == 1 || !planes_il(plane_stride) || (C1 + C2) % 32 == 0, "upsample_concat_planes: chunk-interleaved planes need C1 + C2 %% 32 == 0");
+    const float sh = OH > 1 ? (float)(h - 1) / (float)(OH - 1) : 0.f, sw = OW > 1 ? (float)(w - 1) / (float)(OW - 1) : 0.f;
+    const dim3 grid(cdiv(OW * ((C1 + C2) / 8), 256), OH, B);
+    if (nplanes == 2)
+        hipLaunchKernelGGL(upcat_planes_kernel<2>, grid, dim3(256), 0, as_stream(stream), z, z_pitch, h, w, bridge, bridge_pitch, OH, OW, 0, 0,
+                           static_cast<f16*>(planes), plane_stride, OH, OW, C1, C2, sh, sw, bound);
+    else
+        hipLaunchKernelGGL(upcat_planes_kernel<1>, grid, dim3(256), 0, as_stream(stream), z, z_pitch, h, w, bridge, bridge_pitch, OH, OW, 0, 0,
+                           static_cast<f16*>(planes), plane_stride, OH, OW, C1, C2, sh, sw, bound);
+    PYLC_LAUNCH_CHECK();
+    return PYLC_OK;
+}
diff --git a/pylc_amd/csrc/pool_resize.hip b/pylc_amd/csrc/pool_resize.hip
--- a/pylc_amd/csrc/pool_resize.hip
+++ b/pylc_amd/csrc/pool_resize.hip
@@ -526,6 +526,18 @@
     return PYLC_OK;
 }
 
+int pylc::bilinear_bwd_axis1(const float* tmp, int tmp_pitch, float* dx, int dx_pitch, int B, int H, int W, int C, int OH, unsigned int* amax_bits,
+                             void* stream) {
+    PYLC_REQUIRE(tmp && dx && B > 0 && H > 0 && W > 0 && OH > 0 && C > 0 && C % 4 == 0 && tmp_pitch >= C && dx_pitch >= C && tmp_pitch % 4 == 0 &&
+                     dx_pitch % 4 == 0, "bilinear_bwd_axis1: bad arguments");
+    if (amax_bits != nullptr) PYLC_HIP(hipMemsetAsync(amax_bits, 0, sizeof(unsigned), as_stream(stream)));
+    const long long t1 = (long long)B * H * W * (C / 4);
+    hipLaunchKernelGGL(bilinear_bwd_axis_kernel<1>, dim3(grid_for(t1)), dim3(256), 0, as_stream(stream), tmp, tmp_pitch, dx, dx_pitch, B, H, OH, W, C,
+                       ac_scale(H, OH), amax_bits);
+    PYLC_LAUNCH_CHECK();
+    return PYLC_OK;
+}
+
 extern "C" int pylc_gap_fwd(const float* x, float* y, int B, int HW, int C, void* stream) {
     PYLC_REQUIRE(x && y && B > 0 && HW > 0 && C > 0 && C % 4 == 0, "gap_fwd: bad arguments");
     hipLaunchKernelGGL(gap_fwd_kernel, dim3(cdiv(C / 4, 16), B), dim3(256), 0, as_stream(stream), x, y, HW, C);
diff --git a/pylc_amd/lib.py b/pylc_amd/lib.py
--- a/pylc_amd/lib.py
+++ b/pylc_amd/lib.py
@@ -84,6 +84,7 @@
     'pylc_range_product': (_I, [_P, _P, _F, _P, _P, _P]),
     'pylc_maxpool_fwd_planes': (_I, [_P, _P, _LL, _I, _P, _P, _I, _I, _I, _I, _I, _I, _I, _I, _I, _P]),
     'pylc_upsample2_crop_concat_planes': (_I, [_P, _I, _I, _I, _I, _I, _P, _I, _I, _I, _I, _P, _LL, _I, _P, _P]),
+    'pylc_upsample_concat_planes': (_I, [_P, _I, _I, _I, _I, _I, _P, _I, _I, _I, _I, _P, _LL, _I, _P, _P]),
     'pylc_conv1x1_fold_input_affine': (_I, [_P, _P, _P, _P, _I, _I, _P, _P, _P, _P]),
     'pylc_debug_wgrad_acc1': (_I, [_I]),
     'pylc_debug_wgrad_sets': (_I, [_I]),
@@ -204,6 +205,9 @@
     'pylc_multiloss_stats_ex': (_I, [_P, _I, _P, _I, _LL, _I, _I, _P, _P, _P, _P, _P]),
     'pylc_multiloss_finalize_ex': (_I, [_P, _I, _F, _F, _F, _P, _P]),
     'pylc_multiloss_bwd_ex': (_I, [_P, _I, _P, _I, _LL, _I, _I, _P, _P, _F, _F, _F, _P, _P, _I, _P, _P]),
+    'pylc_multiloss_stats_up': (_I, [_P, _I, _I, _I, _I, _I, _I, _P, _I, _I, _I, _I, _P, _P, _P, _P, _P]),
+    'pylc_multiloss_bwd_up_workspace': (_SZ, [_I, _I, _I, _I]),
+    'pylc_multiloss_bwd_up': (_I, [_P, _I, _I, _I, _I, _I, _I, _P, _I, _I, _I, _I, _P, _P, _D, _F, _F, _F, _P, _P, _I, _P, _P, _P]),
     'pylc_sqnorm_workspace_floats': (_SZ, [_LL]),
     'pylc_grad_norm_clip': (_I, [_P, _LL, _F, _P, _P, _P]),
     'pylc_adamw_step': (_I, [_P, _P, _P, _P, _LL, _P, _F, _F, _F, _F, _F, _I, _P]),
diff --git a/pylc_amd/loss.py b/pylc_amd/loss.py
--- a/pylc_amd/loss.py
+++ b/pylc_amd/loss.py
@@ -27,27 +27,31 @@
         self.eps = 1e-8
         self.ce = self.dsc = self.fl = 0.
 
-    def _check(self, pred, target):
+    def _check(self, pred, target, up_to=None):
         if not torch.is_tensor(pred):
             raise TypeError('Input type is not a torch.Tensor. Got {}'.format(type(pred)))
         if pred.dim() != 4 or pred.size(1) != self.n_classes:
             raise ValueError('Invalid input shape, we expect Bx{}xHxW. Got: {}'.format(self.n_classes, tuple(pred.shape)))
-        if pred.size(0) != target.size(0) or pred.size(2) != target.size(1) or pred.size(3) != target.size(2):
-            raise ValueError('Expected prediction {} to match target {}.'.format(tuple(pred.shape), tuple(target.shape)))
+        h, w = (pred.size(2), pred.size(3)) if up_to is None else up_to
+        if pred.size(0) != target.size(0) or h != target.size(1) or w != target.size(2):
+            raise ValueError('Expected prediction {} to match target {}.'.format((pred.size(0), pred.size(1), h, w), tuple(target.shape)))
         if pred.device != target.device:
             raise ValueError('input and target must be in the same device. Got: {} and {}'.format(pred.device, target.device))
 
-    def _all(self, pred, target, w_ce, w_d, w_f):
-        self._check(pred, target)
+    def _all(self, pred, target, w_ce, w_d, w_f, up_to=None):
+        self._check(pred, target, up_to)
         cw = self.weights if self.weighted else None
-        if self.ignore_index is None:
-            return ops.multiloss(pred, target, cw, w_ce, w_d, w_f, runtime.sync_group)
-        if self.bad_targets is None or self.bad_targets.device != pred.device:
-            self.bad_targets = torch.zeros(1, dtype=torch.int64, device=pred.device)
-        return ops.multiloss(pred, target, cw, w_ce, w_d, w_f, runtime.sync_group, self.ignore_index, self.bad_targets)
+        bad = None
+        if self.ignore_index is not None:
+            if self.bad_targets is None or self.bad_targets.device != pred.device:
+                self.bad_targets = torch.zeros(1, dtype=torch.int64, device=pred.device)
+            bad = self.bad_targets
+        if up_to is not None:
+            return ops.multiloss_up(pred, up_to, target, cw, w_ce, w_d, w_f, runtime.sync_group, self.ignore_index, bad)
+        return ops.multiloss(pred, target, cw, w_ce, w_d, w_f, runtime.sync_group, self.ignore_index, bad)
 
-    def forward(self, pred, target):
-        losses = self._all(pred, target, self.ce_weight, self.dsc_weight, self.fl_weight)
+    def forward(self, pred, target, up_to=None):
+        losses = self._all(pred, target, self.ce_weight, self.dsc_weight, self.fl_weight, up_to)
         self.ce, self.dsc, self.fl = losses[1].detach(), losses[2].detach(), losses[3].detach()
         return losses[0]
 
diff --git a/pylc_amd/model.py b/pylc_amd/model.py
--- a/pylc_amd/model.py
+++ b/pylc_amd/model.py
@@ -214,6 +214,12 @@
             y = y[:, p:y.shape[1] - p, p:y.shape[2] - p]
         return y.contiguous()
 
+    def _loss_takes_low_logits(self):
+        net, crit = self.net, self.crit
+        return bool(runtime.loss_on_low_logits and type(crit) is MultiLoss and callable(getattr(net, 'logits_low', None))
+                    and 'forward' not in vars(crit) and 'forward' not in vars(net)
+                    and not (net._forward_hooks or net._forward_pre_hooks or crit._forward_hooks or crit._forward_pre_hooks))
+
     def train(self, x, y):
         self.net.train()
         if getattr(self.net, 'freeze_bn', False) and ops.nplanes() == 1:
@@ -222,8 +228,11 @@
         self._ranges_checked = False
         x4 = self.pack_input(x)
         y = self._target(y)
-        y_hat = self.net(x4)
-        loss = self.crit(y_hat, y)
+        if self._loss_takes_low_logits():
+            low, size = self.net.logits_low(x4)
+            loss = self.crit(low, y, up_to=size)
+        else:
+            loss = self.crit(self.net(x4), y)
         self.loss.push(torch.stack((self.crit.ce, self.crit.dsc, self.crit.fl)))
         self.optim.zero_grad()
         if runtime.sync_group is not None:
diff --git a/pylc_amd/nets/deeplabv3p.py b/pylc_amd/nets/deeplabv3p.py
--- a/pylc_amd/nets/deeplabv3p.py
+++ b/pylc_amd/nets/deeplabv3p.py
@@ -68,10 +68,16 @@
     def forward(self, x, low):
         b, _, lh, lw = low.shape
         cx, cl = x.shape[1], self.conv1.cout
-        buf = [ops.empty_nhwc(b, cx + cl, lh, lw, x.device)]
-        up = ops.bilinear(x, lh, lw, into=(buf, 0))
-        low = conv_bn(self.conv1, self.bn1, low, relu=True, conv_link=ops.grad_link(low), into=(buf, cx))
-        x = ops.concat_slices(buf, (up, low))
+        if (self.training and torch.is_grad_enabled() and ops.upsample_concat_ok(x, cl, lh, lw)
+                and ops.conv_takes_planes(self.last_conv.child(0).weight, b * lh * lw, 0)):
+            low = conv_bn(self.conv1, self.bn1, low, relu=True, conv_link=ops.grad_link(low))
+            cat = ops.upsample_concat(x, low, lh, lw)
+        else:
+            buf = [ops.empty_nhwc(b, cx + cl, lh, lw, x.device)]
+            up = ops.bilinear(x, lh, lw, into=(buf, 0))
+            low = conv_bn(self.conv1, self.bn1, low, relu=True, conv_link=ops.grad_link(low), into=(buf, cx))
+            cat = ops.concat_slices(buf, (up, low))
+        x = cat
         lc = self.last_conv
         x = conv_bn(lc.child(0), lc.child(1), x, relu=True, out_planes=lc.child(4).takes_planes(), drop=self.drop3, sole=True)
         x = conv_bn(lc.child(4), lc.child(5), x, relu=True, drop=self.drop7)
@@ -127,8 +133,11 @@
         return sorted(picked)
 
     def forward(self, x):
+        y, (h, w) = self.logits_low(x)
+        return ops.bilinear(y, h, w)
+
+    def logits_low(self, x):
         h, w = x.shape[2:]
         x4 = x if x.shape[1] == 4 else ops.pack_nchw(x, 4)
         f, low = self.backbone(x4, keep_planes=True)
-        y = self.decoder(self.aspp(f), low)
-        return ops.bilinear(y, h, w)
+        return self.decoder(self.aspp(f), low), (int(h), int(w))
diff --git a/pylc_amd/ops/misc.py b/pylc_amd/ops/misc.py
--- a/pylc_amd/ops/misc.py
+++ b/pylc_amd/ops/misc.py
@@ -200,6 +200,55 @@
         return None
     bound = torch.maximum(amax_of(z), amax_of(bridge))
     out = UpCatPlanesFn.apply(z, bridge, bound, link)
+    return mark_planes(out, bound)
+
+
+class UpCatFn(torch.autograd.Function):
+
+    @staticmethod
+    def forward(ctx, z, bridge, bound):
+        L.init()
+        z, bridge = as_nhwc(z), as_nhwc(bridge)
+        b, c1, h, w = z.shape
+        c2, oh, ow = bridge.shape[1:]
+        out = empty_nhwc(b, c1 + c2, oh, ow, z.device)
+        check(lib.pylc_upsample_concat_planes(ptr(z), pitch_of(z), b, h, w, c1, ptr(bridge), pitch_of(bridge), oh, ow, c2, ptr(out),
+                                              pstride(b * oh * ow, c1 + c2), nplanes(), ptr(bound), stream()))
+        ctx.geom = (b, c1, h, w, c2, oh, ow)
+        return out
+
+    @staticmethod
+    def backward(ctx, dy):
+        b, c1, h, w, c2, oh, ow = ctx.geom
+        dy = as_nhwc(dy)
+        dz = None
+        if ctx.needs_input_grad[0]:
+            dz = empty_nhwc(b, c1, h, w, dy.device)
+            if oh >= 2 * h and ow >= 2 * w:
+                tmp = torch.empty(lib.pylc_bilinear_bwd_workspace(b, w, c1, oh) // 4, device=dy.device, dtype=torch.float32)
+                amax = torch.empty(1, dtype=torch.int32, device=dy.device) if ranges_needed() and _runtime.fused_grad_ranges else None
+                check(lib.pylc_bilinear_bwd_separable(ptr(dy), pitch_of(dy), ptr(dz), c1, b, h, w, c1, oh, ow, ptr(tmp), ptr(amax), stream()))
+                if amax is not None:
+                    tag_amax(dz, amax)
+            else:
+                check(lib.pylc_bilinear_bwd(ptr(dy), pitch_of(dy), ptr(dz), c1, b, h, w, c1, oh, ow, stream()))
+        return dz, (dy[:, c1:] if ctx.needs_input_grad[1] else None), None
+
+
+def upsample_concat_ok(z, c2, oh, ow):
+    c1 = z.shape[1]
+    pixels = z.shape[0] * oh * ow
+    return bool((torch.is_grad_enabled() or _runtime.eval_planes) and ranges_needed() and not _runtime.no_planes and c1 % 8 == 0 and c2 % 8 == 0
+                and planes_ok(c1 + c2, pixels) and pixels >= _core.PLANES_MIN_PIXELS and not is_planes(z) and _runtime.decoder_upcat)
+
+
+def upsample_concat(z, bridge, oh, ow):
+    if tuple(bridge.shape[2:]) != (oh, ow) or bridge.shape[0] != z.shape[0]:
+        raise L.PylcError('upsample_concat: the bridge %s is not [%d, C, %d, %d]' % (tuple(bridge.shape), z.shape[0], oh, ow))
+    if is_planes(bridge) or not upsample_concat_ok(z, bridge.shape[1], oh, ow):
+        return None
+    bound = torch.maximum(amax_of(z), amax_of(bridge))
+    out = UpCatFn.apply(z, bridge, bound)
     return mark_planes(out, bound)
 
 
@@ -485,4 +534,67 @@
     return MultiLossFn.apply(logits, target, class_weights, w_ce, w_dice, w_focal, group, ignore_index, bad)
 
 
+class MultiLossUpFn(torch.autograd.Function):
+
+    @staticmethod
+    def forward(ctx, low, oh, ow, target, class_weights, w_ce, w_dice, w_focal, group, ignore_index=None, bad=None):
+        L.init()
+        low = as_nhwc(low)
+        b, c, h, w = low.shape
+        if pitch_of(low) < _r4(c):
+            raise L.PylcError('multiloss_up: channel count %d needs a pitch >= %d' % (c, _r4(c)))
+        target = target.contiguous()
+        ign = ignore_index is not None
+        if tuple(target.shape) != (b, oh, ow) or target.dtype not in ((torch.uint8, torch.int64) if ign else (torch.int64,)):
+            raise L.PylcError('target must be %sint64 [B,H,W] matching the up-sampled logits' % ('uint8 or ' if ign else ''))
+        if bad is not None and (bad.dtype != torch.int64 or bad.numel() != 1 or bad.device != low.device):
+            raise L.PylcError('bad must be an int64 [1] tensor on the device of the logits')
+        dev = low.device
+        st = stream()
+        n = b * oh * ow
+        k = 3 + 3 * c
+        stats = torch.empty(k + (2 if group is not None else 0), device=dev)
+        ws = torch.empty(lib.pylc_multiloss_workspace_floats(n, c), device=dev)
+        check(lib.pylc_multiloss_stats_up(ptr(low), pitch_of(low), b, h, w, oh, ow, ptr(target), target.element_size(), c, int(ign),
+                                          int(ignore_index) if ign else 0, ptr(class_weights), ptr(stats), ptr(ws), ptr(bad) if ign else None, st))
+        n_global = float(n)
+        if group is not None:
+            stats[k:].copy_(_shard_pair(b, dev), non_blocking=True)
+            _runtime.sync_all_reduce(stats, group)
+            n_global = float(n) * dist.get_world_size(group)
+            note_shard_pair(stats[k:], dist.get_world_size(group))
+        losses = torch.empty(4, device=dev)
+        if ign:
+            check(lib.pylc_multiloss_finalize_ex(ptr(stats), c, w_ce, w_dice, w_focal, ptr(losses), st))
+        else:
+            check(lib.pylc_multiloss_finalize(ptr(stats), n_global, c, w_ce, w_dice, w_focal, ptr(losses), st))
+        ctx.save_for_backward(low, target, stats, class_weights)
+        ctx.cfg = (oh, ow, n_global, w_ce, w_dice, w_focal, int(ignore_index) if ign else None)
+        return losses
+
+    @staticmethod
+    def backward(ctx, dlosses):
+        low, target, stats, cw = ctx.saved_tensors
+        oh, ow, n_global, w_ce, w_dice, w_focal, ignore = ctx.cfg
+        b, c, h, w = low.shape
+        gs = dlosses[0:1].contiguous().float()
+        cp = _r4(c)
+        dl = empty_nhwc(b, c, h, w, low.device, cp)
+        tmp = torch.empty(lib.pylc_multiloss_bwd_up_workspace(b, w, c, oh) // 4, device=low.device, dtype=torch.float32)
+        amax = torch.empty(1, dtype=torch.int32, device=low.device) if ranges_needed() and _runtime.fused_grad_ranges else None
+        check(lib.pylc_multiloss_bwd_up(ptr(low), pitch_of(low), b, h, w, oh, ow, ptr(target), target.element_size(), c, int(ignore is not None),
+                                        ignore if ignore is not None else 0, ptr(cw), ptr(stats), n_global, w_ce, w_dice, w_focal, ptr(gs),
+                                        ptr(dl), cp, ptr(tmp), ptr(amax), stream()))
+        if amax is not None:
+            tag_amax(dl, amax)
+        return (dl,) + (None,) * 10
+
+
+def multiloss_up(low, size, target, class_weights, w_ce, w_dice, w_focal, group=None, ignore_index=None, bad=None):
+    oh, ow = int(size[0]), int(size[1])
+    if oh >= 2 * low.shape[2] and ow >= 2 * low.shape[3]:
+        return MultiLossUpFn.apply(low, oh, ow, target, class_weights, w_ce, w_dice, w_focal, group, ignore_index, bad)
+    return multiloss(bilinear(low, oh, ow), target, class_weights, w_ce, w_dice, w_focal, group, ignore_index, bad)
+
+
 __all__ = [n for n in dir() if not n.startswith('__')]
diff --git a/pylc_amd/runtime.py b/pylc_amd/runtime.py
--- a/pylc_amd/runtime.py
+++ b/pylc_amd/runtime.py
@@ -25,6 +25,8 @@
         self.skip_zero_bias_grad = True
         self.defer_bn_apply = True
         self.upcat_planes = True
+        self.decoder_upcat = True
+        self.loss_on_low_logits = True
         self.fused_grad_ranges = True
         self.gap_planes = True
         self.batch_slab_sums = True
```
